# gssales/gaussian-splatting-reflection

Measured on AMD Instinct MI355X. Metric: train_step_views_per_s (fwd+bwd, 1e6 Gaussians @1080p, surfel rasterizer + reflection path), higher is better.
Workload: dtype f32

## Files before the change

gaussian-splatting-reflection_amd/csrc/gsr_cubemap.hip:

```cpp
#include <algorithm>
#include <cstring>
#include "gsr_internal.hpp"
#include <mutex>
#include <memory>
#include "gsr_sort.hpp"
#include <rocprim/iterator/counting_iterator.hpp>
#include "gsr_refl.hpp"

namespace gsr {



struct Plain {
	int f, ux0, ux1, uy0, uy1;
	float kx, ky;
};
__device__ __forceinline__ void plain_index(float vx, float vy, float vz, int L, Plain& p, bool nearest) {
	float u, v;
	cube_uv(vx, vy, vz, u, v, p.f);
	v = -v;
	u = (u * 0.5f + 0.5f) * (float)L;
	v = (v * 0.5f + 0.5f) * (float)L;
	if (nearest) {
		p.ux0 = min(max((int)u, 0), L - 1);
		p.uy0 = min(max((int)v, 0), L - 1);
		p.ux1 = p.ux0; p.uy1 = p.uy0; p.kx = 0; p.ky = 0;
		return;
	}
	const int ux_0 = (int)floorf(u - 0.5f), uy_0 = (int)floorf(v - 0.5f);
	p.kx = u - (float)ux_0 - 0.5f;
	p.ky = v - (float)uy_0 - 0.5f;
	p.ux0 = min(max(ux_0, 0), L - 1); p.ux1 = min(max(ux_0 + 1, 0), L - 1);
	p.uy0 = min(max(uy_0, 0), L - 1); p.uy1 = min(max(uy_0 + 1, 0), L - 1);
}

__global__ void __launch_bounds__(256)
cubemap_fwd_kernel(const float* __restrict__ inputs, const float* __restrict__ cubemap, const float* __restrict__ fail_value,
                   float* __restrict__ outputs, int interp, int seamless, uint32_t B, int C, int L) {
	const uint32_t n = blockIdx.x * 256 + threadIdx.x;
	if (n >= B) return;
	const float vx = inputs[(size_t)n * 3], vy = inputs[(size_t)n * 3 + 1], vz = inputs[(size_t)n * 3 + 2];
	if (vx == 0.f && vy == 0.f && vz == 0.f) {
		for (int c = 0; c < C; c++) outputs[(size_t)c * B + n] = fail_value[c];
		return;
	}
	if (interp == 0 || seamless == 0) {
		Plain p;
		plain_index(vx, vy, vz, L, p, interp == 0);
		for (int c = 0; c < C; c++) {
			if (interp == 0) {
				outputs[(size_t)c * B + n] = cubemap[texel(p.f, c, p.uy0, p.ux0, C, L)];
			} else {
				const float v00 = cubemap[texel(p.f, c, p.uy0, p.ux0, C, L)], v01 = cubemap[texel(p.f, c, p.uy0, p.ux1, C, L)];
				const float v10 = cubemap[texel(p.f, c, p.uy1, p.ux0, C, L)], v11 = cubemap[texel(p.f, c, p.uy1, p.ux1, C, L)];
				outputs[(size_t)c * B + n] = (1 - p.ky) * ((1 - p.kx) * v00 + p.kx * v01) + p.ky * ((1 - p.kx) * v10 + p.kx * v11);
			}
		}
		return;
	}
	float u, v;
	int face;
	cube_uv(vx, vy, vz, u, v, face);
	Seamless s;
	seamless_index(face, L, u, v, s);
	for (int c = 0; c < C; c++) {
		const float v00 = cubemap[texel(s.f[0], c, s.y[0], s.x[0], C, L)];
		const float v01 = cubemap[texel(s.f[1], c, s.y[1], s.x[1], C, L)];
		const float v10 = cubemap[texel(s.f[2], c, s.y[2], s.x[2], C, L)];
		const float v11 = s.is_vertex ? (v00 + v01 + v10) / 3.f : cubemap[texel(s.f[3], c, s.y[3], s.x[3], C, L)];
		outputs[(size_t)c * B + n] = (1 - s.ky) * ((1 - s.kx) * v00 + s.kx * v01) + s.ky * ((1 - s.kx) * v10 + s.kx * v11);
	}
}

__device__ __forceinline__ void seamless_bwd_channel(const Seamless& s, int c, int C, int L, const float* __restrict__ cubemap,
                                                     float* __restrict__ grad_cubemap, float g, float& gu, float& gv) {
	const size_t i00 = texel(s.f[0], c, s.y[0], s.x[0], C, L), i01 = texel(s.f[1], c, s.y[1], s.x[1], C, L);
	const size_t i10 = texel(s.f[2], c, s.y[2], s.x[2], C, L);
	const float v00 = cubemap[i00], v01 = cubemap[i01], v10 = cubemap[i10];
	float v11;
	if (s.is_vertex) {
		v11 = (v00 + v01 + v10) / 3.f;
		const float extra_g = s.ky * s.kx / 3.f;
		atomicAdd(grad_cubemap + i00, ((1 - s.ky) * (1 - s.kx) + extra_g) * g);
		atomicAdd(grad_cubemap + i01, ((1 - s.ky) * s.kx + extra_g) * g);
		atomicAdd(grad_cubemap + i10, ((s.ky * (1 - s.kx)) + extra_g) * g);
	} else {
		const size_t i11 = texel(s.f[3], c, s.y[3], s.x[3], C, L);
		v11 = cubemap[i11];
		atomicAdd(grad_cubemap + i00, (1 - s.ky) * (1 - s.kx) * g);
		atomicAdd(grad_cubemap + i01, (1 - s.ky) * s.kx * g);
		atomicAdd(grad_cubemap + i10, s.ky * (1 - s.kx) * g);
		atomicAdd(grad_cubemap + i11, s.ky * s.kx * g);
	}
	float lg0 = (1 - s.ky) * (v01 - v00) + s.ky * (v11 - v10);
	float lg1 = (1 - s.kx) * (v10 - v00) + s.kx * (v11 - v01);
	lg0 *= 0.5f * (float)L * g;
	lg1 *= 0.5f * (float)L * g;
	if (s.flag & 1) lg0 = -lg0;
	if (s.flag & 4) lg1 = -lg1;
	lg1 = -lg1;
	gu = lg0;
	gv = lg1;
}

__global__ void __launch_bounds__(256)
cubemap_bwd_kernel(const float* __restrict__ grad_outputs, const float* __restrict__ inputs, const float* __restrict__ cubemap,
                   float* __restrict__ grad_cubemap, float* __restrict__ grad_inputs, float* __restrict__ grad_fail, int interp, int seamless,
                   uint32_t B, int C, int L) {
	const uint32_t n = blockIdx.x * 256 + threadIdx.x;
	if (n >= B) return;
	const float vx = inputs[(size_t)n * 3], vy = inputs[(size_t)n * 3 + 1], vz = inputs[(size_t)n * 3 + 2];
	float gx = 0.f, gy = 0.f, gz = 0.f;
	if (vx == 0.f && vy == 0.f && vz == 0.f) {
		for (int c = 0; c < C; c++) atomicAdd(grad_fail + c, grad_outputs[(size_t)c * B + n]);
	} else if (interp == 0) {
		Plain p;
		plain_index(vx, vy, vz, L, p, true);
		for (int c = 0; c < C; c++) atomicAdd(grad_cubemap + texel(p.f, c, p.uy0, p.ux0, C, L), grad_outputs[(size_t)c * B + n]);
	} else if (seamless == 0) {
		Plain p;
		plain_index(vx, vy, vz, L, p, false);
		for (int c = 0; c < C; c++) {
			const size_t i00 = texel(p.f, c, p.uy0, p.ux0, C, L), i01 = texel(p.f, c, p.uy0, p.ux1, C, L);
			const size_t i10 = texel(p.f, c, p.uy1, p.ux0, C, L), i11 = texel(p.f, c, p.uy1, p.ux1, C, L);
			const float v00 = cubemap[i00], v01 = cubemap[i01], v10 = cubemap[i10], v11 = cubemap[i11];
			const float g = grad_outputs[(size_t)c * B + n];
			atomicAdd(grad_cubemap + i00, (1 - p.ky) * (1 - p.kx) * g);
			atomicAdd(grad_cubemap + i01, (1 - p.ky) * p.kx * g);
			atomicAdd(grad_cubemap + i10, p.ky * (1 - p.kx) * g);
			atomicAdd(grad_cubemap + i11, p.ky * p.kx * g);
			float lg0 = (1 - p.ky) * (v01 - v00) + p.ky * (v11 - v10);
			float lg1 = (1 - p.kx) * (v10 - v00) + p.kx * (v11 - v01);
			lg0 *= 0.5f * (float)L * g;
			lg1 *= 0.5f * (float)L * g;
			lg1 = -lg1;
			float a, b, cc;
			cube_uv_backward(p.f, vx, vy, vz, lg0, lg1, a, b, cc);
			gx += a; gy += b; gz += cc;
		}
	} else {
		float u, v;
		int face;
		cube_uv(vx, vy, vz, u, v, face);
		Seamless s;
		seamless_index(face, L, u, v, s);
		for (int c = 0; c < C; c++) {
			float gu, gv, a, b, cc;
			seamless_bwd_channel(s, c, C, L, cubemap, grad_cubemap, grad_outputs[(size_t)c * B + n], gu, gv);
			cube_uv_backward(face, vx, vy, vz, gu, gv, a, b, cc);
			gx += a; gy += b; gz += cc;
		}
	}
	grad_inputs[(size_t)n * 3] = gx;
	grad_inputs[(size_t)n * 3 + 1] = gy;
	grad_inputs[(size_t)n * 3 + 2] = gz;
}

__global__ void __launch_bounds__(256) cubemap_interleave_kernel(const float* __restrict__ cubemap, float4* __restrict__ rgba, int L) {
	const size_t LL = (size_t)L * L;
	const size_t t = (size_t)blockIdx.x * 256 + threadIdx.x;
	if (t >= 6 * LL) return;
	const size_t f = t / LL, r = t - f * LL;
	rgba[t] = make_float4(cubemap[(f * 3 + 0) * LL + r], cubemap[(f * 3 + 1) * LL + r], cubemap[(f * 3 + 2) * LL + r], 0.f);
}
template <bool RGBA>
__global__ void __launch_bounds__(256)
deferred_refl_fwd_kernel(const float* __restrict__ normal_view, const float* __restrict__ base, const float* __restrict__ strength,
                         const float* __restrict__ cam, const float* __restrict__ cubemap, const float4* __restrict__ rgba,
                         const float* __restrict__ fail_value, int L, int W, int H, float* __restrict__ out_final, float* __restrict__ out_refl,
                         float* __restrict__ out_nworld, uint32_t* __restrict__ sort_keys, uint32_t no_key) {
	const size_t HW = (size_t)W * H;
	const size_t pix = (size_t)blockIdx.x * 256 + threadIdx.x;
	if (pix >= HW) return;
	const int py = (int)(pix / W), px = (int)(pix - (size_t)py * W);
	const float nvx = normal_view[pix], nvy = normal_view[HW + pix], nvz = normal_view[2 * HW + pix];
	const float sv = strength[pix];
	const float b0 = base[pix], b1 = base[HW + pix], b2 = base[2 * HW + pix];
	ReflFwdOut o;
	refl_forward_pixel<RGBA>(cam, cubemap, rgba, fail_value, L, nvx, nvy, nvz, px, py, sv, b0, b1, b2, no_key, o);
	if (sort_keys) sort_keys[pix] = o.key;
#pragma unroll
	for (int ch = 0; ch < 3; ch++) {
		out_refl[ch * HW + pix] = o.refl_c[ch];
		out_final[ch * HW + pix] = o.final_c[ch];
	}
	out_nworld[pix] = o.nx;
	out_nworld[HW + pix] = o.ny;
	out_nworld[2 * HW + pix] = o.nz;
}

__device__ __forceinline__ float quad_sum(float v) {
	v += __int_as_float(__builtin_amdgcn_mov_dpp(__float_as_int(v), 0xB1, 0xF, 0xF, true));
	v += __int_as_float(__builtin_amdgcn_mov_dpp(__float_as_int(v), 0x4E, 0xF, 0xF, true));
	return v;
}
__global__ void __launch_bounds__(256)
deferred_refl_bwd_kernel(const float* __restrict__ normal_view, const float* __restrict__ base, const float* __restrict__ strength,
                         const float* __restrict__ cam, const float* __restrict__ cubemap, const float* __restrict__ fail_value, int L, int W,
                         int H, const float* __restrict__ g_final, const float* __restrict__ g_refl_color, const float* __restrict__ g_nworld,
                         float* __restrict__ g_normal_view, float* __restrict__ g_base, float* __restrict__ g_strength,
                         float* __restrict__ g_scratch, float* __restrict__ g_fail) {
	const size_t HW = (size_t)W * H;
	const size_t gid = (size_t)blockIdx.x * 256 + threadIdx.x;
	const size_t pix = gid >> 2;
	const int ch = (int)(gid & 3);
	const bool live = pix < HW;
	const size_t p = live ? pix : 0;
	const int py = (int)(p / W), px = (int)(p - (size_t)py * W);
	ReflPixel o;
	refl_pixel(cam, normal_view[p], normal_view[HW + p], normal_view[2 * HW + p], px, py, o);
	const bool fail = (o.rx == 0.f && o.ry == 0.f && o.rz == 0.f);
	const bool chan = live && ch < 3;
	const int c = ch < 3 ? ch : 0;
	Seamless s;
	int face = 0;
	float cval;
	size_t i00 = 0, i01 = 0, i10 = 0, i11 = 0;
	float v00 = 0, v01 = 0, v10 = 0, v11 = 0;
	if (fail) {
		cval = fail_value[c];
		s.kx = 0; s.ky = 0; s.flag = 0; s.is_vertex = false;
	} else {
		float u, v;
		cube_uv(o.rx, o.ry, o.rz, u, v, face);
		seamless_index(face, L, u, v, s);
		i00 = texel(s.f[0], c, s.y[0], s.x[0], 3, L); i01 = texel(s.f[1], c, s.y[1], s.x[1], 3, L);
		i10 = texel(s.f[2], c, s.y[2], s.x[2], 3, L);
		v00 = cubemap[i00]; v01 = cubemap[i01]; v10 = cubemap[i10];
		if (s.is_vertex) v11 = (v00 + v01 + v10) / 3.f;
		else { i11 = texel(s.f[3], c, s.y[3], s.x[3], 3, L); v11 = cubemap[i11]; }
		cval = (1 - s.ky) * ((1 - s.kx) * v00 + s.kx * v01) + s.ky * ((1 - s.kx) * v10 + s.kx * v11);
	}
	const float sv = strength[p];
	const float rc = sigmoidf_(cval);
	float gs = 0.f, grx = 0.f, gry = 0.f, grz = 0.f;
	int tix[4] = {-1, -1, -1, -1};
	float twg[4] = {0.f, 0.f, 0.f, 0.f};
	if (chan) {
		const float gf = g_final[c * HW + p];
		const float b = base[c * HW + p];
		g_base[c * HW + p] = (1 - sv) * gf;
		gs = gf * (rc - b);
		float gc = sv * gf;
		if (g_refl_color) gc += g_refl_color[c * HW + p];
		const float graw = gc * rc * (1 - rc);
		if (fail) {
			atomicAdd(g_fail + c, graw);
		} else {
			auto sidx = [&](int k) -> int { return (int)((((((size_t)s.f[k] * L + s.y[k]) * L + s.x[k]) << 2)) + c); };
			if (s.is_vertex) {
				const float extra_g = s.ky * s.kx / 3.f;
				tix[0] = sidx(0); twg[0] = ((1 - s.ky) * (1 - s.kx) + extra_g) * graw;
				tix[1] = sidx(1); twg[1] = ((1 - s.ky) * s.kx + extra_g) * graw;
				tix[2] = sidx(2); twg[2] = ((s.ky * (1 - s.kx)) + extra_g) * graw;
			} else {
				tix[0] = sidx(0); twg[0] = (1 - s.ky) * (1 - s.kx) * graw;
				tix[1] = sidx(1); twg[1] = (1 - s.ky) * s.kx * graw;
				tix[2] = sidx(2); twg[2] = s.ky * (1 - s.kx) * graw;
				tix[3] = sidx(3); twg[3] = s.ky * s.kx * graw;
			}
			float lg0 = (1 - s.ky) * (v01 - v00) + s.ky * (v11 - v10);
			float lg1 = (1 - s.kx) * (v10 - v00) + s.kx * (v11 - v01);
			lg0 *= 0.5f * (float)L * graw;
			lg1 *= 0.5f * (float)L * graw;
			if (s.flag & 1) lg0 = -lg0;
			if (s.flag & 4) lg1 = -lg1;
			lg1 = -lg1;
			cube_uv_backward(face, o.rx, o.ry, o.rz, lg0, lg1, grx, gry, grz);
		}
	}
	{
		const bool inA = ((threadIdx.x >> 2) & 1) == 0;
		const int XOR4 = 0x101F;
		const int s_i0 = inA ? tix[1] : tix[0], s_i1 = inA ? tix[3] : tix[2];
		const float s_w0 = inA ? twg[1] : twg[0], s_w1 = inA ? twg[3] : twg[2];
		const int r_i0 = __builtin_amdgcn_ds_swizzle(s_i0, XOR4), r_i1 = __builtin_amdgcn_ds_swizzle(s_i1, XOR4);
		const float r_w0 = __int_as_float(__builtin_amdgcn_ds_swizzle(__float_as_int(s_w0), XOR4));
		const float r_w1 = __int_as_float(__builtin_amdgcn_ds_swizzle(__float_as_int(s_w1), XOR4));
		const int i0 = inA ? tix[0] : r_i0, i1 = inA ? tix[2] : r_i1, i2 = inA ? r_i0 : tix[1], i3 = inA ? r_i1 : tix[3];
		const float w0 = inA ? twg[0] : r_w0, w1 = inA ? twg[2] : r_w1, w2 = inA ? r_w0 : twg[1], w3 = inA ? r_w1 : twg[3];
		if (i0 >= 0) atomicAdd(g_scratch + i0, w0);
		if (i1 >= 0) atomicAdd(g_scratch + i1, w1);
		if (i2 >= 0) atomicAdd(g_scratch + i2, w2);
		if (i3 >= 0) atomicAdd(g_scratch + i3, w3);
	}
	gs = quad_sum(gs); grx = quad_sum(grx); gry = quad_sum(gry); grz = quad_sum(grz);
	if (live && ch == 3) g_strength[p] = gs;
	const float grn = grx * o.nx + gry * o.ny + grz * o.nz;
	float gnx = -2.f * (o.dn * grx + grn * o.dx);
	float gny = -2.f * (o.dn * gry + grn * o.dy);
	float gnz = -2.f * (o.dn * grz + grn * o.dz);
	if (g_nworld) { gnx += g_nworld[p]; gny += g_nworld[HW + p]; gnz += g_nworld[2 * HW + p]; }
	const float inv = refl_rcp(o.len + 1e-6f);
	float gwx = gnx * inv, gwy = gny * inv, gwz = gnz * inv;
	if (o.len > 0.f) {
		const float k = (o.nwx * gnx + o.nwy * gny + o.nwz * gnz) * inv * inv * refl_rcp(o.len);
		gwx -= o.nwx * k; gwy -= o.nwy * k; gwz -= o.nwz * k;
	}
	if (chan) g_normal_view[c * HW + p] = gwx * cam[c] + gwy * cam[3 + c] + gwz * cam[6 + c];
}

#ifndef ENTRIES_BS
#define ENTRIES_BS 512
#endif
template <bool RGBA>
__global__ void __launch_bounds__(ENTRIES_BS)
deferred_refl_bwd_entries_kernel(const float* __restrict__ normal_view, const float* __restrict__ base, const float* __restrict__ strength,
                                 const float* __restrict__ cam, const float* __restrict__ cubemap, const float4* __restrict__ rgba,
                                 const float* __restrict__ fail_value, int L,
                                 int W, int H, const float* __restrict__ g_final, const float* __restrict__ g_refl_color,
                                 const float* __restrict__ g_nworld, float* __restrict__ g_normal_view, float* __restrict__ g_base,
                                 float* __restrict__ g_strength, float* __restrict__ g_fail, float* __restrict__ g_scratch,
                                 ReflFootprint* __restrict__ footprints, uint32_t* __restrict__ keys, const uint32_t* __restrict__ keys_fwd, uint32_t no_key,
                                 void* sort_clear, size_t sort_clear_bytes) {
	const size_t HW = (size_t)W * H;
	const size_t pix = (size_t)blockIdx.x * ENTRIES_BS + threadIdx.x;
	sort_clear_region(sort_clear, sort_clear_bytes, pix, (size_t)gridDim.x * ENTRIES_BS);
	const bool live = pix < HW;
	const size_t p = live ? pix : 0;
	const int py = (int)(p / W), px = (int)(p - (size_t)py * W);
	ReflBwdIn in;
	in.nvx = normal_view[p]; in.nvy = normal_view[HW + p]; in.nvz = normal_view[2 * HW + p];
	in.sv = strength[p];
	in.has_grc = g_refl_color != nullptr;
	in.has_gnw = g_nworld != nullptr;
#pragma unroll
	for (int c = 0; c < 3; c++) {
		in.gfin[c] = g_final[c * HW + p];
		in.bas[c] = base[c * HW + p];
		in.grc[c] = g_refl_color ? g_refl_color[c * HW + p] : 0.f;
		in.gnw[c] = g_nworld ? g_nworld[c * HW + p] : 0.f;
	}
	const uint32_t kf = keys_fwd ? keys_fwd[p] : no_key;
	ReflBwdOut o;
	refl_backward_pixel<RGBA>(cam, cubemap, rgba, fail_value, L, px, py, live, in, g_fail, g_scratch, footprints + p, keys_fwd != nullptr, kf,
	                          keys ? keys + p : nullptr, no_key, (int)(threadIdx.x & 63), o);
	if (!live) return;
	g_strength[p] = o.g_strength;
#pragma unroll
	for (int c = 0; c < 3; c++) {
		g_base[c * HW + p] = o.g_base[c];
		g_normal_view[c * HW + p] = o.g_nv[c];
	}
}

template <bool ACC>
__global__ void __launch_bounds__(256) unpack_cubemap_grad_kernel(const float4* __restrict__ scratch, float* __restrict__ g_cubemap,
                                                                  float* __restrict__ g_fail, int L) {
	const size_t n = (size_t)6 * L * L;
	const size_t t = (size_t)blockIdx.x * 256 + threadIdx.x;
	if (t == 0) {
		const float4 gf = scratch[n];
		g_fail[0] = (ACC ? g_fail[0] : 0.f) + gf.x; g_fail[1] = (ACC ? g_fail[1] : 0.f) + gf.y; g_fail[2] = (ACC ? g_fail[2] : 0.f) + gf.z;
	}
	if (t >= n) return;
	const size_t LL = (size_t)L * L;
	const size_t f = t / LL, r = t - f * LL;
	const float4 g = scratch[t];
	float* o = g_cubemap + f * 3 * LL + r;
	o[0] = (ACC ? o[0] : 0.f) + g.x;
	o[LL] = (ACC ? o[LL] : 0.f) + g.y;
	o[2 * LL] = (ACC ? o[2 * LL] : 0.f) + g.z;
}

#define REFL_CHUNK 8
#ifndef REFL_WIN
#define REFL_WIN 1024u
#endif
__global__ void __launch_bounds__(256) refl_run_combine_kernel(const uint32_t* __restrict__ keys_sorted, const uint32_t* __restrict__ pix_sorted,
                                                               const ReflFootprint* __restrict__ footprints, size_t n, uint32_t L, uint32_t no_key,
                                                               float* __restrict__ g_scratch) {
	__shared__ float win[3][REFL_WIN];
	__shared__ uint32_t s_hi;
	const size_t wg0 = (size_t)blockIdx.x * 256 * REFL_CHUNK;
	const uint32_t t_lo = keys_sorted[wg0];
	if (t_lo == no_key) return;
	const size_t wg_last = min(n, wg0 + (size_t)256 * REFL_CHUNK) - 1;
	const uint32_t t_hi = keys_sorted[wg_last];
	const uint32_t reach = t_hi == no_key ? REFL_WIN : min(REFL_WIN, t_hi - t_lo + L + 2u);
	for (uint32_t i = threadIdx.x; i < reach; i += 256) { win[0][i] = 0.f; win[1][i] = 0.f; win[2][i] = 0.f; }
	if (threadIdx.x == 0) s_hi = 0u;
	__syncthreads();

	const size_t i0 = wg0 + (size_t)threadIdx.x * REFL_CHUNK;
	uint32_t key[REFL_CHUNK];
	float4 ga[REFL_CHUNK];
	float gky[REFL_CHUNK];
#pragma unroll
	for (int j = 0; j < REFL_CHUNK; j++) key[j] = i0 + j < n ? keys_sorted[i0 + j] : no_key;
#pragma unroll
	for (int j = 0; j < REFL_CHUNK; j++) {
		ga[j] = make_float4(0.f, 0.f, 0.f, 0.f);
		gky[j] = 0.f;
		if (key[j] != no_key) {
			const float* f = reinterpret_cast<const float*>(footprints + pix_sorted[i0 + j]);
			ga[j] = *reinterpret_cast<const float4*>(f);
			gky[j] = f[4];
		}
	}
	float acc[4][3];
	uint32_t cur = no_key, hi = 0u;
	auto flush = [&]() {
		if (cur == no_key) return;
#pragma unroll
		for (int k = 0; k < 4; k++) {
			const uint32_t rel = cur - t_lo + (uint32_t)(k & 1) + (uint32_t)(k >> 1) * L;
			if (rel < REFL_WIN) {
				hi = max(hi, rel);
#pragma unroll
				for (int c = 0; c < 3; c++)
					if (acc[k][c] != 0.f) atomicAdd(&win[c][rel], acc[k][c]);
			} else {
				float* dst = g_scratch + (((size_t)t_lo + rel) << 2);
#pragma unroll
				for (int c = 0; c < 3; c++)
					if (acc[k][c] != 0.f) atomicAdd(dst + c, acc[k][c]);
			}
		}
	};
#pragma unroll
	for (int j = 0; j < REFL_CHUNK; j++) {
		if (key[j] != no_key) {
			if (key[j] != cur) {
				flush();
				cur = key[j];
#pragma unroll
				for (int k = 0; k < 4; k++) { acc[k][0] = 0.f; acc[k][1] = 0.f; acc[k][2] = 0.f; }
			}
			const float kx = ga[j].w, ky = gky[j];
			const float w4[4] = {(1 - ky) * (1 - kx), (1 - ky) * kx, ky * (1 - kx), ky * kx};
#pragma unroll
			for (int k = 0; k < 4; k++) {
				acc[k][0] += w4[k] * ga[j].x; acc[k][1] += w4[k] * ga[j].y; acc[k][2] += w4[k] * ga[j].z;
			}
		}
	}
	flush();
	if (hi != 0u) atomicMax(&s_hi, hi);
	__syncthreads();
	const uint32_t top = s_hi;
	for (uint32_t i = threadIdx.x; i <= top; i += 256) {
		float* dst = g_scratch + (((size_t)t_lo + i) << 2);
#pragma unroll
		for (int c = 0; c < 3; c++) {
			const float v = win[c][i];
			if (v != 0.f) atomicAdd(dst + c, v);
		}
	}
}

}

using namespace gsr;

extern "C" int gsr_cubemap_forward(const float* inputs, const float* cubemap, const float* fail_value, float* outputs, uint32_t interp,
                                   uint32_t seamless, uint32_t B, uint32_t C, uint32_t L, void* stream_) {
	hipStream_t stream = (hipStream_t)stream_;
	if (B == 0) return 0;
	if (!inputs || !cubemap || !fail_value || !outputs || C == 0 || L == 0) { set_error("gsr_cubemap_forward: invalid argument"); return GSR_E_INVALID; }
{ StageTimer st_(GSR_STAGE_CUBEMAP_FWD, stream); 	cubemap_fwd_kernel<<<(B + 255) / 256, 256, 0, stream>>>(inputs, cubemap, fail_value, outputs, (int)interp, (int)seamless, B, (int)C, (int)L); }
	GSR_LAUNCH_CHECK(0, stream);
	return 0;
}

extern "C" int gsr_cubemap_backward(const float* grad_outputs, const float* inputs, const float* cubemap, float* grad_cubemap,
                                    float* grad_inputs, float* grad_fail, uint32_t interp, uint32_t seamless, uint32_t B, uint32_t C, uint32_t L,
                                    void* stream_) {
	hipStream_t stream = (hipStream_t)stream_;
	if (B == 0) return 0;
	if (!grad_outputs || !inputs || !cubemap || !grad_cubemap || !grad_inputs || !grad_fail || C == 0 || L == 0) {
		set_error("gsr_cubemap_backward: invalid argument");
		return GSR_E_INVALID;
	}
{ StageTimer st_(GSR_STAGE_CUBEMAP_BWD, stream); 	cubemap_bwd_kernel<<<(B + 255) / 256, 256, 0, stream>>>(grad_outputs, inputs, cubemap, grad_cubemap, grad_inputs, grad_fail, (int)interp,
	                                                        (int)seamless, B, (int)C, (int)L); }
	GSR_LAUNCH_CHECK(0, stream);
	return 0;
}

extern "C" int gsr_deferred_reflection_forward_keys(const float* normal_view, const float* base_color, const float* refl_strength, const float* cam,
                                                  const float* cubemap, const float* fail_value, uint32_t L, int width, int height,
                                                  float* out_final, float* out_refl_color, float* out_normal_world, float* cubemap_rgba,
                                                  uint32_t* sort_keys, void* stream_) {
	hipStream_t stream = (hipStream_t)stream_;
	if (width <= 0 || height <= 0 || !normal_view || !base_color || !refl_strength || !cam || !cubemap || !fail_value || !out_final ||
	    !out_refl_color || !out_normal_world || L == 0 || ((uintptr_t)cubemap_rgba & 15) != 0) {
		set_error("gsr_deferred_reflection_forward: invalid argument");
		return GSR_E_INVALID;
	}
	if ((size_t)6 * L * L >= 0xFFFFFFFFull) { set_error("gsr_deferred_reflection_forward: cubemap too large"); return GSR_E_INVALID; }
	const size_t HW = (size_t)width * height;
	StageTimer st_(GSR_STAGE_REFL_FWD, stream);
	const unsigned grid = (unsigned)((HW + 255) / 256);
	if (cubemap_rgba) {
		float4* rgba = reinterpret_cast<float4*>(cubemap_rgba);
		cubemap_interleave_kernel<<<(unsigned)((6 * (size_t)L * L + 255) / 256), 256, 0, stream>>>(cubemap, rgba, (int)L);
		deferred_refl_fwd_kernel<true><<<grid, 256, 0, stream>>>(normal_view, base_color, refl_strength, cam, cubemap, rgba, fail_value, (int)L, width, height,
		                                                        out_final, out_refl_color, out_normal_world, sort_keys, (uint32_t)(6 * (size_t)L * L));
	} else {
		deferred_refl_fwd_kernel<false><<<grid, 256, 0, stream>>>(normal_view, base_color, refl_strength, cam, cubemap, nullptr, fail_value, (int)L, width, height,
		                                                         out_final, out_refl_color, out_normal_world, sort_keys, (uint32_t)(6 * (size_t)L * L));
	}
	GSR_LAUNCH_CHECK(0, stream);
	return 0;
}
extern "C" int gsr_deferred_reflection_forward_ex(const float* normal_view, const float* base_color, const float* refl_strength, const float* cam,
                                                  const float* cubemap, const float* fail_value, uint32_t L, int width, int height,
                                                  float* out_final, float* out_refl_color, float* out_normal_world, float* cubemap_rgba, void* stream_) {
	return gsr_deferred_reflection_forward_keys(normal_view, base_color, refl_strength, cam, cubemap, fail_value, L, width, height, out_final, out_refl_color,
	                                            out_normal_world, cubemap_rgba, nullptr, stream_);
}
extern "C" int gsr_deferred_reflection_forward(const float* normal_view, const float* base_color, const float* refl_strength, const float* cam,
                                               const float* cubemap, const float* fail_value, uint32_t L, int width, int height,
                                               float* out_final, float* out_refl_color, float* out_normal_world, void* stream_) {
	return gsr_deferred_reflection_forward_keys(normal_view, base_color, refl_strength, cam, cubemap, fail_value, L, width, height, out_final, out_refl_color,
	                                          out_normal_world, nullptr, nullptr, stream_);
}

struct ReflScratch {
	size_t ntex, n, sort_bytes, total_floats;
	int key_bits;
};
#ifndef REFL_SORT_BS
#define REFL_SORT_BS 512
#endif
#ifndef REFL_SORT_IPT
#define REFL_SORT_IPT 16
#endif
template <class F>
static auto with_refl_sort(int key_bits, bool small, F&& f) {
	if (small) return f(RadixSort<256, 8, 8>{});
	if (key_bits > 16 && key_bits <= 18) return f(RadixSort<REFL_SORT_BS, REFL_SORT_IPT, 9>{});
	if (key_bits > 18 && key_bits <= 20) return f(RadixSort<1024, 8, 10>{});
	return f(RadixSort<1024, 8, 8>{});
}
static ReflScratch refl_scratch(uint32_t L, int width, int height) {
	thread_local uint32_t last_L = 0;
	thread_local int last_w = 0, last_h = 0;
	thread_local ReflScratch last;
	if (last_L != 0 && L == last_L && width == last_w && height == last_h) return last;
	ReflScratch r;
	r.ntex = (size_t)6 * L * L;
	r.n = (size_t)width * height;
	r.key_bits = 1;
	while (((size_t)1 << r.key_bits) <= r.ntex) r.key_bits++;
	auto need = [&](bool small) {
		return with_refl_sort(r.key_bits, small, [&](auto sort) {
			return sort.temp_bytes((const uint32_t*)nullptr, rocprim::counting_iterator<uint32_t>(0), (uint32_t*)nullptr, r.n, (unsigned)r.key_bits);
		});
	};
	r.sort_bytes = std::max(need(false), need(true));
	r.total_floats = (r.ntex + 2) * 4 + 8 * r.n + 3 * r.n + (r.sort_bytes + 3) / 4 + 128;
	last = r; last_L = L; last_w = width; last_h = height;
	return r;
}
extern "C" size_t gsr_deferred_reflection_scratch_floats(uint32_t L, int width, int height, int binned) {
	if (L == 0 || width <= 0 || height <= 0) return 0;
	if (!binned) return ((size_t)6 * L * L + 1) * 4;
	return refl_scratch(L, width, height).total_floats;
}

namespace {
struct SideStream {
	hipStream_t stream = nullptr;
	hipEvent_t fork = nullptr, fork2 = nullptr, done = nullptr, gate = nullptr;
	bool recorded = false;
	bool gate_pending = false;
};
std::mutex g_side_mu;
SideStream g_side[64];
SideStream* side_stream(bool create) {
	int dev = 0;
	if (hipGetDevice(&dev) != hipSuccess || dev < 0 || dev >= 64) return nullptr;
	SideStream& s = g_side[dev];
	if (!s.stream && create) {
		int least = 0, greatest = 0;
		(void)hipDeviceGetStreamPriorityRange(&least, &greatest);
		if (hipStreamCreateWithPriority(&s.stream, hipStreamNonBlocking, greatest) != hipSuccess) { s.stream = nullptr; return nullptr; }
		if (hipEventCreateWithFlags(&s.fork, hipEventDisableTiming) != hipSuccess || hipEventCreateWithFlags(&s.fork2, hipEventDisableTiming) != hipSuccess ||
		    hipEventCreateWithFlags(&s.done, hipEventDisableTiming) != hipSuccess || hipEventCreateWithFlags(&s.gate, hipEventDisableTiming) != hipSuccess) {
			(void)hipStreamDestroy(s.stream);
			s.stream = nullptr;
		}
	}
	return s.stream ? &s : nullptr;
}

struct ReflTail {
	ReflScratch rs;
	float* staging = nullptr;
	float* fail_acc = nullptr;
	ReflFootprint* footprints = nullptr;
	uint32_t *keys_in = nullptr, *keys_out = nullptr, *pix_out = nullptr;
	void* sort_temp = nullptr;
	hipStream_t stream, tail;
	SideStream* side = nullptr;
	std::unique_lock<std::mutex> lock;

	ReflTail(uint32_t L, int width, int height, hipStream_t s) : rs(refl_scratch(L, width, height)), stream(s), tail(s) {}
	bool carve(float* scratch, size_t scratch_floats) {
		staging = scratch;
		fail_acc = scratch + rs.ntex * 4;
		if (scratch_floats < rs.total_floats || rs.n >= ((size_t)1 << 30) || rs.ntex >= 0xFFFFFFFFull || ((uintptr_t)scratch & 31) != 0) return false;
		footprints = reinterpret_cast<ReflFootprint*>(scratch + (rs.ntex + 1) * 4 + 4);
		keys_in = reinterpret_cast<uint32_t*>(footprints + rs.n);
		keys_out = keys_in + rs.n;
		pix_out = keys_out + rs.n;
		sort_temp = reinterpret_cast<void*>(((uintptr_t)(pix_out + rs.n) + 255) & ~(uintptr_t)255);
		return true;
	}
	void lock_side() { lock = std::unique_lock<std::mutex>(g_side_mu); }
	void use_side_stream() {
		lock_side();
		side = side_stream(true);
		if (side) tail = side->stream;
	}
	size_t sort_cleared_bytes(bool small) const {
		return with_refl_sort(rs.key_bits, small, [&](auto sort) { return sort.cleared_bytes(rs.n, (unsigned)rs.key_bits); });
	}
	hipError_t fork(hipEvent_t ev) {
		hipError_t e = hipEventRecord(ev, stream);
		return e == hipSuccess ? hipStreamWaitEvent(side->stream, ev, 0) : e;
	}
	hipError_t sort(const uint32_t* keys, bool small, bool gated) {
		hipError_t e = with_refl_sort(rs.key_bits, small, [&](auto sort) {
			return sort.pairs(sort_temp, rs.sort_bytes, keys, keys_out, rocprim::counting_iterator<uint32_t>(0), pix_out, rs.n, (unsigned)rs.key_bits, tail, true, nullptr,
			                  gated && side ? side->gate : nullptr);
		});
		if (e == hipSuccess && gated && side) side->gate_pending = true;
		return e;
	}
	hipError_t mark_done() {
		hipError_t e = hipEventRecord(side->done, side->stream);
		if (e == hipSuccess) side->recorded = true;
		return e;
	}
};
}

namespace gsr {
int side_gate_wait(hipStream_t stream) {
	std::lock_guard<std::mutex> lk(g_side_mu);
	SideStream* s = side_stream(false);
	if (s && s->gate_pending) {
		s->gate_pending = false;
		GSR_HIP_CHECK(hipStreamWaitEvent(stream, s->gate, 0));
	}
	return 0;
}

int refl_scratch_check(const char* entry, uint32_t L, int width, int height, const float* scratch, size_t scratch_floats) {
	ReflTail t(L, width, height, nullptr);
	if (!scratch || !t.carve(const_cast<float*>(scratch), scratch_floats)) {
		set_error("%s: reflection backward (sorted footprints): scratch of %zu floats, 32-byte aligned, needed (gsr_deferred_reflection_scratch_floats(L, W, H, 1))",
		          entry, t.rs.total_floats);
		return GSR_E_INVALID;
	}
	return 0;
}
int refl_sort_keys_early(uint32_t L, int width, int height, float* scratch, size_t scratch_floats, const uint32_t* sort_keys, int async, bool gated,
                         hipStream_t stream) {
	if (const int rc = refl_scratch_check("gsr_surfel_forward_refl", L, width, height, scratch, scratch_floats); rc < 0) return rc;
	ReflTail t(L, width, height, stream);
	t.carve(scratch, scratch_floats);
	if (async) t.use_side_stream();
	if (t.side) GSR_HIP_CHECK(t.fork(t.side->fork));
	{
		StageTimer tt(GSR_STAGE_REFL_BWD_TAIL, t.tail);
		GSR_HIP_CHECK(hipMemsetAsync(t.sort_temp, 0, t.sort_cleared_bytes(false), t.tail));
		GSR_HIP_CHECK(t.sort(sort_keys, false, gated));
	}
	if (t.side) GSR_HIP_CHECK(t.mark_done());
	return 0;
}
}

extern "C" int gsr_side_join(void* stream_) {
	std::lock_guard<std::mutex> lk(g_side_mu);
	const SideStream* s = side_stream(false);
	if (s && s->recorded) GSR_HIP_CHECK(hipStreamWaitEvent((hipStream_t)stream_, s->done, 0));
	return 0;
}

extern "C" int gsr_deferred_reflection_backward_keys(const float* normal_view, const float* base_color, const float* refl_strength, const float* cam,
                                                   const float* cubemap, const float* fail_value, uint32_t L, int width, int height,
                                                   const float* g_final, const float* g_refl_color, const float* g_normal_world,
                                                   float* g_normal_view, float* g_base, float* g_strength, float* g_cubemap, float* g_fail,
                                                   float* scratch, size_t scratch_floats, int accumulate, int async_tail, const float* cubemap_rgba,
                                                   const uint32_t* sort_keys, int keys_sorted, void* stream_) {
	hipStream_t stream = (hipStream_t)stream_;
	if (width <= 0 || height <= 0 || !normal_view || !base_color || !refl_strength || !cam || !cubemap || !fail_value || !g_final ||
	    !g_normal_view || !g_base || !g_strength || !g_cubemap || !g_fail || !scratch || L == 0 || (keys_sorted && !sort_keys)) {
		set_error("gsr_deferred_reflection_backward: invalid argument");
		return GSR_E_INVALID;
	}
	if ((size_t)6 * L * L >= 0xFFFFFFFFull) { set_error("gsr_deferred_reflection_backward: cubemap too large"); return GSR_E_INVALID; }
	GSR_REQUIRE_ALIGNED16_IN("gsr_deferred_reflection_backward", scratch, "scratch");
	GSR_REQUIRE_ALIGNED16_IN("gsr_deferred_reflection_backward", cubemap_rgba, "cubemap_rgba");
	const size_t HW = (size_t)width * height;
	ReflTail t(L, width, height, stream);
	const size_t ntex = t.rs.ntex;
	if (scratch_floats < (ntex + 1) * 4) { set_error("gsr_deferred_reflection_backward: scratch smaller than (6*L*L+1)*4 floats"); return GSR_E_INVALID; }
	const bool binned = t.carve(scratch, scratch_floats);
	if (keys_sorted && !binned) { set_error("gsr_deferred_reflection_backward: keys_sorted needs the scratch the forward sorted into"); return GSR_E_INVALID; }
	auto unpack = accumulate ? unpack_cubemap_grad_kernel<true> : unpack_cubemap_grad_kernel<false>;
	GSR_HIP_CHECK(hipMemsetAsync(scratch, 0, (ntex + 1) * 4 * sizeof(float), stream));
	if (!binned) {
		{
			StageTimer st_(GSR_STAGE_REFL_BWD, stream);
			const unsigned grid = (unsigned)((HW * 4 + 255) / 256);
			deferred_refl_bwd_kernel<<<grid, 256, 0, stream>>>(normal_view, base_color, refl_strength, cam, cubemap, fail_value, (int)L, width, height, g_final,
			                                                  g_refl_color, g_normal_world, g_normal_view, g_base, g_strength, t.staging, t.fail_acc);
		}
		unpack<<<(unsigned)((ntex + 255) / 256), 256, 0, stream>>>((const float4*)t.staging, g_cubemap, g_fail, (int)L);
		GSR_LAUNCH_CHECK(0, stream);
		return 0;
	}
	const bool small_sort = async_tail && !sort_keys;
	const size_t sort_cleared = t.sort_cleared_bytes(small_sort);
	if (async_tail) t.use_side_stream();
	else if (keys_sorted) t.lock_side();
	if (keys_sorted) {
		const SideStream* s = side_stream(false);
		if (s && s->recorded && t.tail != s->stream) GSR_HIP_CHECK(hipStreamWaitEvent(t.tail, s->done, 0));
	} else if (sort_keys) {
		GSR_HIP_CHECK(hipMemsetAsync(t.sort_temp, 0, sort_cleared, stream));
		if (t.side) GSR_HIP_CHECK(t.fork(t.side->fork));
		StageTimer tt(GSR_STAGE_REFL_BWD_TAIL, t.tail);
		GSR_HIP_CHECK(t.sort(sort_keys, false, true));
	}
	{
		StageTimer st_(GSR_STAGE_REFL_BWD, stream);
		const unsigned egrid = (unsigned)((HW + ENTRIES_BS - 1) / ENTRIES_BS);
		if (cubemap_rgba)
			deferred_refl_bwd_entries_kernel<true><<<egrid, ENTRIES_BS, 0, stream>>>(normal_view, base_color, refl_strength, cam, cubemap,
			                                                                 reinterpret_cast<const float4*>(cubemap_rgba), fail_value, (int)L, width, height, g_final,
			                                                                 g_refl_color, g_normal_world, g_normal_view, g_base, g_strength, t.fail_acc, t.staging,
			                                                                 t.footprints, t.keys_in, sort_keys, (uint32_t)ntex, sort_keys ? nullptr : t.sort_temp,
			                                                                 sort_keys ? 0 : sort_cleared);
		else
			deferred_refl_bwd_entries_kernel<false><<<egrid, ENTRIES_BS, 0, stream>>>(normal_view, base_color, refl_strength, cam, cubemap, nullptr, fail_value, (int)L, width,
			                                                                  height, g_final, g_refl_color, g_normal_world, g_normal_view, g_base, g_strength, t.fail_acc,
			                                                                  t.staging, t.footprints, t.keys_in, sort_keys, (uint32_t)ntex, sort_keys ? nullptr : t.sort_temp,
			                                                                  sort_keys ? 0 : sort_cleared);
	}
	if (t.side) GSR_HIP_CHECK(t.fork(sort_keys ? t.side->fork2 : t.side->fork));
	{
		StageTimer tt(GSR_STAGE_REFL_BWD_TAIL, t.tail);
		const size_t per_wg = (size_t)256 * REFL_CHUNK;
		const unsigned cgrid = (unsigned)((t.rs.n + per_wg - 1) / per_wg);
		if (!sort_keys) GSR_HIP_CHECK(t.sort(t.keys_in, small_sort, false));
		refl_run_combine_kernel<<<cgrid, 256, 0, t.tail>>>(t.keys_out, t.pix_out, t.footprints, t.rs.n, L, (uint32_t)ntex, t.staging);
		unpack<<<(unsigned)((ntex + 255) / 256), 256, 0, t.tail>>>((const float4*)t.staging, g_cubemap, g_fail, (int)L);
	}
	if (t.side) GSR_HIP_CHECK(t.mark_done());
	GSR_HIP_CHECK(hipGetLastError());
	return 0;
}

extern "C" int gsr_deferred_reflection_backward_ex(const float* normal_view, const float* base_color, const float* refl_strength, const float* cam,
                                                   const float* cubemap, const float* fail_value, uint32_t L, int width, int height,
                                                   const float* g_final, const float* g_refl_color, const float* g_normal_world,
                                                   float* g_normal_view, float* g_base, float* g_strength, float* g_cubemap, float* g_fail,
                                                   float* scratch, size_t scratch_floats, int accumulate, int async_tail, const float* cubemap_rgba,
                                                   void* stream_) {
	return gsr_deferred_reflection_backward_keys(normal_view, base_color, refl_strength, cam, cubemap, fail_value, L, width, height, g_final, g_refl_color,
	                                             g_normal_world, g_normal_view, g_base, g_strength, g_cubemap, g_fail, scratch, scratch_floats, accumulate,
	                                             async_tail, cubemap_rgba, nullptr, 0, stream_);
}

extern "C" int gsr_deferred_reflection_backward_accum(const float* normal_view, const float* base_color, const float* refl_strength, const float* cam,
                                                const float* cubemap, const float* fail_value, uint32_t L, int width, int height,
                                                const float* g_final, const float* g_refl_color, const float* g_normal_world,
                                                float* g_normal_view, float* g_base, float* g_strength, float* g_cubemap, float* g_fail,
                                                float* scratch, size_t scratch_floats, int accumulate, void* stream_) {
	return gsr_deferred_reflection_backward_keys(normal_view, base_color, refl_strength, cam, cubemap, fail_value, L, width, height, g_final, g_refl_color,
	                                             g_normal_world, g_normal_view, g_base, g_strength, g_cubemap, g_fail, scratch, scratch_floats, accumulate, 0, nullptr,
	                                             nullptr, 0, stream_);
}

extern "C" int gsr_deferred_reflection_backward(const float* normal_view, const float* base_color, const float* refl_strength, const float* cam,
                                                const float* cubemap, const float* fail_value, uint32_t L, int width, int height,
                                                const float* g_final, const float* g_refl_color, const float* g_normal_world,
                                                float* g_normal_view, float* g_base, float* g_strength, float* g_cubemap, float* g_fail,
                                                float* scratch, size_t scratch_floats, void* stream_) {
	return gsr_deferred_reflection_backward_accum(normal_view, base_color, refl_strength, cam, cubemap, fail_value, L, width, height, g_final, g_refl_color,
	                                              g_normal_world, g_normal_view, g_base, g_strength, g_cubemap, g_fail, scratch, scratch_floats, 0, stream_);
}

__global__ void __launch_bounds__(256) normal_world_fwd_kernel(const float* __restrict__ normal_view, const float* __restrict__ cam, size_t HW,
                                                               float* __restrict__ out) {
	const size_t pix = (size_t)blockIdx.x * 256 + threadIdx.x;
	if (pix >= HW) return;
	const float vx = normal_view[pix], vy = normal_view[HW + pix], vz = normal_view[2 * HW + pix];
	const float wx = vx * cam[0] + vy * cam[1] + vz * cam[2], wy = vx * cam[3] + vy * cam[4] + vz * cam[5], wz = vx * cam[6] + vy * cam[7] + vz * cam[8];
	const float inv = 1.0f / (sqrtf(wx * wx + wy * wy + wz * wz) + 1e-6f);
	out[pix] = wx * inv; out[HW + pix] = wy * inv; out[2 * HW + pix] = wz * inv;
}
__global__ void __launch_bounds__(256) normal_world_bwd_kernel(const float* __restrict__ normal_view, const float* __restrict__ cam, size_t HW,
                                                               const float* __restrict__ g_out, float* __restrict__ g_normal_view) {
	const size_t pix = (size_t)blockIdx.x * 256 + threadIdx.x;
	if (pix >= HW) return;
	const float vx = normal_view[pix], vy = normal_view[HW + pix], vz = normal_view[2 * HW + pix];
	const float wx = vx * cam[0] + vy * cam[1] + vz * cam[2], wy = vx * cam[3] + vy * cam[4] + vz * cam[5], wz = vx * cam[6] + vy * cam[7] + vz * cam[8];
	const float len = sqrtf(wx * wx + wy * wy + wz * wz);
	const float inv = 1.0f / (len + 1e-6f);
	const float gx = g_out[pix], gy = g_out[HW + pix], gz = g_out[2 * HW + pix];
	float ax = gx * inv, ay = gy * inv, az = gz * inv;
	if (len > 0.f) {
		const float k = (wx * gx + wy * gy + wz * gz) * inv * inv / len;
		ax -= wx * k; ay -= wy * k; az -= wz * k;
	}
#pragma unroll
	for (int c = 0; c < 3; c++) g_normal_view[c * HW + pix] = ax * cam[c] + ay * cam[3 + c] + az * cam[6 + c];
}
extern "C" int gsr_normal_world_forward(const float* normal_view, const float* cam, int width, int height, float* out_normal_world, void* stream_) {
	if (width <= 0 || height <= 0 || !normal_view || !cam || !out_normal_world) { set_error("gsr_normal_world_forward: invalid argument"); return GSR_E_INVALID; }
	const size_t HW = (size_t)width * height;
	normal_world_fwd_kernel<<<(unsigned)((HW + 255) / 256), 256, 0, (hipStream_t)stream_>>>(normal_view, cam, HW, out_normal_world);
	GSR_LAUNCH_CHECK(0, (hipStream_t)stream_);
	return 0;
}
extern "C" int gsr_normal_world_backward(const float* normal_view, const float* cam, int width, int height, const float* g_normal_world,
                                         float* g_normal_view, void* stream_) {
	if (width <= 0 || height <= 0 || !normal_view || !cam || !g_normal_world || !g_normal_view) { set_error("gsr_normal_world_backward: invalid argument"); return GSR_E_INVALID; }
	const size_t HW = (size_t)width * height;
	normal_world_bwd_kernel<<<(unsigned)((HW + 255) / 256), 256, 0, (hipStream_t)stream_>>>(normal_view, cam, HW, g_normal_world, g_normal_view);
	GSR_LAUNCH_CHECK(0, (hipStream_t)stream_);
	return 0;
}
```

gaussian-splatting-reflection_amd/csrc/gsr_internal.hpp:

```cpp
#pragma once
#include <cstring>
#include <cstdint>
#include <cstdio>
#include <hip/hip_runtime.h>
#include "../../include/gsr_hip.h"

#define GSR_TILE 16
#define GSR_TILE_PIX 256

namespace gsr {

void set_error(const char* fmt, ...);
#define GSR_HIP_CHECK(expr)                                                                       \
	do {                                                                                          \
		hipError_t _e = (expr);                                                                   \
		if (_e != hipSuccess) {                                                                   \
			gsr::set_error("%s failed: %s (%s:%d)", #expr, hipGetErrorString(_e), __FILE__, __LINE__); \
			return GSR_E_HIP;                                                                     \
		}                                                                                         \
	} while (0)
#define GSR_LAUNCH_CHECK(debug, stream)                                  \
	do {                                                                 \
		GSR_HIP_CHECK(hipGetLastError());                                \
		if (debug) GSR_HIP_CHECK(hipStreamSynchronize(stream));          \
	} while (0)

static inline bool misaligned16(const void* p) { return (reinterpret_cast<uintptr_t>(p) & 15u) != 0; }
#define GSR_REQUIRE_ALIGNED16_IN(func, ptr, what)                                                             \
	do {                                                                                                      \
		if ((ptr) && gsr::misaligned16(ptr)) {                                                                \
			gsr::set_error("%s: %s must be 16-byte aligned (float4 accesses); got %p", func, what, (const void*)(ptr)); \
			return GSR_E_INVALID;                                                                             \
		}                                                                                                     \
	} while (0)
#define GSR_REQUIRE_ALIGNED16(ptr, what) GSR_REQUIRE_ALIGNED16_IN(__func__, ptr, what)

struct StageTimer {
	int stage;
	hipStream_t stream;
	void* rec;
	StageTimer(int stage, hipStream_t stream);
	~StageTimer();
};

struct Carver {
	char* base;
	size_t off;
	explicit Carver(void* b) : base((char*)b), off(0) {}
	template <class T> T* take(size_t count) {
		off = (off + 255) & ~(size_t)255;
		T* p = base ? (T*)(base + off) : nullptr;
		off += count * sizeof(T);
		return p;
	}
	size_t size() const { return (off + 255) & ~(size_t)255; }
};

struct GeomState {
	float* depths;
	uint32_t* rect;
	uint32_t* tiles_touched;
	uint32_t* point_offsets;
	uint8_t* clamped;
	float4* rec;
	float4* bbox;
	float* aux;
	float* acc;
	int* flags;
	uint32_t* depth_sorted;
	unsigned long long* order;
	unsigned long long* emit_state;
	size_t emit_state_bytes;
	void* scan_temp;
	size_t scan_temp_bytes;
	void* depth_sort_temp;
	size_t depth_sort_bytes, depth_sort_clear;
};
struct ImageState {
	uint2* ranges;
	float* final_T;
	uint32_t* n_contrib;
	uint32_t* tile_order;
};
struct BinningState {
	uint32_t* point_list;
	unsigned long long* blend_mask;
	size_t mask_stride;
	uint32_t* tile_keys;
	uint32_t* tile_keys_unsorted;
	uint32_t* vals_unsorted;
	void* sort_temp;
	size_t sort_temp_bytes;
};

#define S_REC_F4 5
#define S_ACC_F 20
#define G_REC_F4 4
#define G_ACC_F 16
struct WorkspaceLayout {
	int rec_f4, aux_floats, acc_floats;
	int planes_T, planes_n;
	constexpr WorkspaceLayout inference() const { return {rec_f4, aux_floats, 0, 0, 0}; }
};
constexpr WorkspaceLayout SURFEL_LAYOUT{S_REC_F4, 0, S_ACC_F, 3, 2};
constexpr WorkspaceLayout GAUSS_LAYOUT{G_REC_F4, 0, G_ACC_F, 1, 1};

GeomState carve_geom(void* buf, size_t P, const WorkspaceLayout& layout, size_t* total);
ImageState carve_image(void* buf, size_t HW, size_t tiles, const WorkspaceLayout& layout, size_t* total);
BinningState carve_binning(void* buf, size_t R, size_t tiles, size_t sort_temp_bytes, size_t* total, bool blend_masks = true);
int forward_workspace(gsr_alloc_fn alloc, void* alloc_user, const WorkspaceLayout& layout, size_t P, size_t HW, size_t tiles, GeomState* geom,
                      ImageState* img);

static inline int check_sh_input(const char* entry, int D, int M, const float* shs) {
	if (D < 0 || D > 3 || (shs && (D + 1) * (D + 1) > M)) { set_error("%s: SH degree %d not supported with M=%d", entry, D, M); return GSR_E_INVALID; }
	if (shs && ((M * 3) & 3) == 0 && misaligned16(shs)) {
		set_error("%s: shs (rows of a multiple of 16 bytes) must be 16-byte aligned (float4 accesses); got %p", entry, (const void*)shs);
		return GSR_E_INVALID;
	}
	return 0;
}

struct RasterCam {
	const float* view;
	const float* proj;
	const float* campos;
	int W, H;
	float tan_fovx, tan_fovy, focal_x, focal_y;
};
static inline RasterCam make_cam(const float* view, const float* proj, const float* campos, int W, int H, float tan_fovx, float tan_fovy) {
	RasterCam c;
	c.view = view; c.proj = proj; c.campos = campos; c.W = W; c.H = H;
	c.tan_fovx = tan_fovx; c.tan_fovy = tan_fovy;
	c.focal_y = H / (2.0f * tan_fovy);
	c.focal_x = W / (2.0f * tan_fovx);
	return c;
}

struct BackwardWorkspace { GeomState geom; ImageState img; BinningState bin; int tiles_x, ntiles; };
static inline int backward_prologue(const char* entry, const char* func, const WorkspaceLayout& layout, int P, int M, int R, int width, int height,
                                    bool missing_pointer, const float* shs, const float* dL_dsh, const float* dL_drot, const float* also_aligned,
                                    const char* also_what, void* geom_buffer, void* binning_buffer, void* image_buffer, hipStream_t stream,
                                    BackwardWorkspace* w) {
	if (P < 0 || R < 0 || width <= 0 || height <= 0) { set_error("%s: invalid size", entry); return GSR_E_INVALID; }
	if (P == 0) return 0;
	if (missing_pointer) { set_error("%s: missing required pointer", entry); return GSR_E_INVALID; }
	if (shs && ((M * 3) & 3) == 0) GSR_REQUIRE_ALIGNED16_IN(func, dL_dsh, "dL_dsh");
	GSR_REQUIRE_ALIGNED16_IN(func, dL_drot, "dL_drot");
	GSR_REQUIRE_ALIGNED16_IN(func, also_aligned, also_what);
	w->tiles_x = (width + 15) / 16;
	w->ntiles = w->tiles_x * ((height + 15) / 16);
	w->geom = carve_geom(geom_buffer, P, layout, nullptr);
	w->img = carve_image(image_buffer, (size_t)width * height, w->ntiles, layout, nullptr);
	w->bin = carve_binning(binning_buffer, R, w->ntiles, 0, nullptr);
	GSR_HIP_CHECK(hipMemsetAsync(w->geom.acc, 0, (size_t)P * layout.acc_floats * sizeof(float), stream));
	return 1;
}

int option_cull();
int option_dev();
unsigned long long* dev_pair_counter();
size_t sort_temp_bytes(size_t R, int end_bit);
int run_tile_order(const ImageState& img, size_t tiles, hipStream_t stream);
uint32_t higher_msb(uint32_t n);

int run_binning(gsr_alloc_fn alloc, void* alloc_user, int P, int tiles_x, int tiles_y, const GeomState& geom,
                const ImageState& img, BinningState* out_binning, int prefiltered, int debug, hipStream_t stream, bool blend_masks = true);

int side_gate_wait(hipStream_t stream);
int refl_scratch_check(const char* entry, uint32_t L, int width, int height, const float* scratch, size_t scratch_floats);
int refl_sort_keys_early(uint32_t L, int width, int height, float* scratch, size_t scratch_floats, const uint32_t* sort_keys, int async, bool gated,
                         hipStream_t stream);

}

#ifdef __HIPCC__
namespace gsr {

__device__ __forceinline__ int f2i(float v) { return (int)v; }

__device__ __forceinline__ void get_rect(float px, float py, int max_radius, int gx, int gy, uint32_t& x0, uint32_t& y0,
                                         uint32_t& x1, uint32_t& y1) {
	const float r = (float)max_radius;
	x0 = (uint32_t)min(gx, max(0, f2i((px - r) / 16.0f)));
	y0 = (uint32_t)min(gy, max(0, f2i((py - r) / 16.0f)));
	x1 = (uint32_t)min(gx, max(0, f2i((px + r + 15.0f) / 16.0f)));
	y1 = (uint32_t)min(gy, max(0, f2i((py + r + 15.0f) / 16.0f)));
}

#define GSR_DPP1(CTRL, i) "v_add_f32_dpp %" #i ", %" #i ", %" #i " " CTRL "\n\t"
#define GSR_DPP4(CTRL) GSR_DPP1(CTRL, 0) GSR_DPP1(CTRL, 1) GSR_DPP1(CTRL, 2) GSR_DPP1(CTRL, 3)
#define GSR_SHR1 "row_shr:1 row_mask:0xf bank_mask:0xf bound_ctrl:0"
#define GSR_SHR2 "row_shr:2 row_mask:0xf bank_mask:0xf bound_ctrl:0"
#define GSR_SHR4 "row_shr:4 row_mask:0xf bank_mask:0xf bound_ctrl:0"
#define GSR_SHR8 "row_shr:8 row_mask:0xf bank_mask:0xf bound_ctrl:0"
#define GSR_BC15 "row_bcast:15 row_mask:0xa bank_mask:0xf"
#define GSR_BC31 "row_bcast:31 row_mask:0xc bank_mask:0xf"
__device__ __forceinline__ void wave_sum4(float* v) {
	asm volatile("s_nop 1\n\t" GSR_DPP4(GSR_SHR1) GSR_DPP4(GSR_SHR2) GSR_DPP4(GSR_SHR4) GSR_DPP4(GSR_SHR8) GSR_DPP4(GSR_BC15) GSR_DPP4(GSR_BC31)
	             : "+v"(v[0]), "+v"(v[1]), "+v"(v[2]), "+v"(v[3]));
}

#define GSR_Q1(CTRL, i) "v_add_f32_dpp %" #i ", %" #i ", %" #i " " CTRL " row_mask:0xf bank_mask:0xf\n\t"
#define GSR_DPPB(CTRL, BANK, dst, src) "v_add_f32_dpp %" #dst ", %" #src ", %" #src " " CTRL " row_mask:0xf bank_mask:" BANK "\n\t"
#define GSR_L1(CTRL, d, a, b) GSR_DPPB(CTRL, "0x3", d, a) GSR_DPPB(CTRL, "0xc", d, b)
__device__ __forceinline__ void row_reduce20(const float* v, float* z) {
	float p0, q0, p1, q1, p2, q2, p3, q3, p4, q4;
	asm volatile("s_nop 1\n\t" GSR_L1("row_mirror", 0, 6, 7) GSR_L1("row_mirror", 1, 8, 9) GSR_L1("row_mirror", 2, 10, 11)
	             GSR_L1("row_mirror", 3, 12, 13) GSR_L1("row_mirror", 4, 14, 15) GSR_L1("row_mirror", 5, 16, 17)
	             : "=&v"(p0), "=&v"(q0), "=&v"(p1), "=&v"(q1), "=&v"(p2), "=&v"(q2)
	             : "v"(v[0]), "v"(v[1]), "v"(v[2]), "v"(v[3]), "v"(v[4]), "v"(v[5]), "v"(v[6]), "v"(v[7]), "v"(v[8]), "v"(v[9]), "v"(v[10]), "v"(v[11]));
	asm volatile("s_nop 1\n\t" GSR_L1("row_mirror", 0, 4, 5) GSR_L1("row_mirror", 1, 6, 7) GSR_L1("row_mirror", 2, 8, 9) GSR_L1("row_mirror", 3, 10, 11)
	             : "=&v"(p3), "=&v"(q3), "=&v"(p4), "=&v"(q4)
	             : "v"(v[12]), "v"(v[13]), "v"(v[14]), "v"(v[15]), "v"(v[16]), "v"(v[17]), "v"(v[18]), "v"(v[19]));
#define GSR_L2(d, a, b) GSR_DPPB("row_half_mirror", "0x5", d, a) GSR_DPPB("row_half_mirror", "0xa", d, b)
#define GSR_QA(CTRL) GSR_Q1(CTRL, 0) GSR_Q1(CTRL, 1) GSR_Q1(CTRL, 2) GSR_Q1(CTRL, 3) GSR_Q1(CTRL, 4)
	asm volatile("s_nop 1\n\t" GSR_L2(0, 5, 6) GSR_L2(1, 7, 8) GSR_L2(2, 9, 10) GSR_L2(3, 11, 12) GSR_L2(4, 13, 14)
	             GSR_QA("quad_perm:[2,3,0,1]") GSR_QA("quad_perm:[1,0,3,2]")
	             : "=&v"(z[0]), "=&v"(z[1]), "=&v"(z[2]), "=&v"(z[3]), "=&v"(z[4])
	             : "v"(p0), "v"(q0), "v"(p1), "v"(q1), "v"(p2), "v"(q2), "v"(p3), "v"(q3), "v"(p4), "v"(q4));
}
__device__ __forceinline__ void row_reduce16(const float* v, float* z) {
	float p0, q0, p1, q1, p2, q2, p3, q3;
	asm volatile("s_nop 1\n\t" GSR_L1("row_mirror", 0, 8, 9) GSR_L1("row_mirror", 1, 10, 11) GSR_L1("row_mirror", 2, 12, 13) GSR_L1("row_mirror", 3, 14, 15)
	             GSR_L1("row_mirror", 4, 16, 17) GSR_L1("row_mirror", 5, 18, 19) GSR_L1("row_mirror", 6, 20, 21) GSR_L1("row_mirror", 7, 22, 23)
	             : "=&v"(p0), "=&v"(q0), "=&v"(p1), "=&v"(q1), "=&v"(p2), "=&v"(q2), "=&v"(p3), "=&v"(q3)
	             : "v"(v[0]), "v"(v[1]), "v"(v[2]), "v"(v[3]), "v"(v[4]), "v"(v[5]), "v"(v[6]), "v"(v[7]), "v"(v[8]), "v"(v[9]), "v"(v[10]), "v"(v[11]),
	               "v"(v[12]), "v"(v[13]), "v"(v[14]), "v"(v[15]));
#define GSR_QB(CTRL) GSR_Q1(CTRL, 0) GSR_Q1(CTRL, 1) GSR_Q1(CTRL, 2) GSR_Q1(CTRL, 3)
	asm volatile("s_nop 1\n\t" GSR_L2(0, 4, 5) GSR_L2(1, 6, 7) GSR_L2(2, 8, 9) GSR_L2(3, 10, 11)
	             GSR_QB("quad_perm:[2,3,0,1]") GSR_QB("quad_perm:[1,0,3,2]")
	             : "=&v"(z[0]), "=&v"(z[1]), "=&v"(z[2]), "=&v"(z[3])
	             : "v"(p0), "v"(q0), "v"(p1), "v"(q1), "v"(p2), "v"(q2), "v"(p3), "v"(q3));
}
__device__ __forceinline__ int sub_px(int lane) { return ((lane >> 4) & 1) * 4 + (lane & 3); }
__device__ __forceinline__ int sub_py(int lane) { return (lane >> 5) * 4 + ((lane >> 2) & 3); }
__device__ __forceinline__ void wave_lds_sync() {
	__builtin_amdgcn_fence(__ATOMIC_RELEASE, "wavefront");
	__builtin_amdgcn_wave_barrier();
	__builtin_amdgcn_fence(__ATOMIC_ACQUIRE, "wavefront");
}
template <int N, bool ACC>
__device__ __forceinline__ void wave_store_rows(float* lds, const float* v, float* __restrict__ out, int nrows, int lane) {
#pragma unroll
	for (int k = 0; k < N; k++) lds[k * 65 + lane] = v[k];
	wave_lds_sync();
#pragma unroll
	for (int j = 0; j < N; j++) {
		const int e = lane + 64 * j, r = e / N, k = e - r * N;
		if (r < nrows) {
			const float x = lds[k * 65 + r];
			if (ACC) {
				if (x != 0.f) out[e] += x;
			} else {
				out[e] = x;
			}
		}
	}
	wave_lds_sync();
}
template <int N, bool ACC>
__device__ __forceinline__ void wave_store_rows4(float4* lds, const float4* v, float4* __restrict__ out, int pitch, int col0, int nrows, int lane) {
#pragma unroll
	for (int k = 0; k < N; k++) lds[k * 65 + lane] = v[k];
	wave_lds_sync();
#pragma unroll
	for (int j = 0; j < N; j++) {
		const int e = lane + 64 * j, r = e / N, k = e - r * N;
		if (r < nrows) {
			const float4 x = lds[k * 65 + r];
			float4* o = out + (size_t)r * pitch + col0 + k;
			if (ACC) {
				if (x.x != 0.f || x.y != 0.f || x.z != 0.f || x.w != 0.f) {
					const float4 y = *o;
					*o = make_float4(y.x + x.x, y.y + x.y, y.z + x.z, y.w + x.w);
				}
			} else {
				*o = x;
			}
		}
	}
	wave_lds_sync();
}
template <bool ACC> __device__ __forceinline__ void put(float* p, float v) {
	if (ACC) { if (v != 0.f) *p += v; }
	else *p = v;
}
template <bool ACC> __device__ __forceinline__ void put4(float4* p, float a, float b, float c, float d) {
	if (ACC) {
		if (a != 0.f || b != 0.f || c != 0.f || d != 0.f) {
			const float4 r = *p;
			*p = make_float4(r.x + a, r.y + b, r.z + c, r.w + d);
		}
	} else {
		*p = make_float4(a, b, c, d);
	}
}
__device__ __forceinline__ uint32_t ffbl_raw(uint32_t x) {
	uint32_t r;
	asm("v_ffbl_b32 %0, %1" : "=v"(r) : "v"(x));
	return r;
}
__device__ __forceinline__ int row_reduce_slot(int lane) {
	const int q = (lane >> 2) & 3;
	return ((q & 1) << 1) | (q >> 1);
}

typedef unsigned long long lmask;
#define LMASK(cond) __builtin_amdgcn_ballot_w64(cond)
__device__ __forceinline__ float selm(lmask m, float a, float b) {
	float r;
	asm("v_cndmask_b32 %0, %1, %2, %3" : "=v"(r) : "v"(b), "v"(a), "s"(m));
	return r;
}
__device__ __forceinline__ float selm0(lmask m, float a) {
	float r;
	asm("v_cndmask_b32 %0, 0, %1, %2" : "=v"(r) : "v"(a), "s"(m));
	return r;
}
__device__ __forceinline__ uint32_t selmu(lmask m, uint32_t a, uint32_t b) {
	uint32_t r;
	asm("v_cndmask_b32 %0, %1, %2, %3" : "=v"(r) : "v"(b), "v"(a), "s"(m));
	return r;
}

__device__ __forceinline__ float min_raw(float a, float b) {
	float r;
	asm("v_min_f32 %0, %1, %2" : "=v"(r) : "v"(a), "v"(b));
	return r;
}

__device__ __forceinline__ float row_max4(float a, float b, float c, float d) {
	float p, q, z;
	asm volatile("s_nop 1\n\t"
	             "v_max_f32_dpp %0, %2, %2 row_mirror row_mask:0xf bank_mask:0x3\n\t"
	             "v_max_f32_dpp %0, %3, %3 row_mirror row_mask:0xf bank_mask:0xc\n\t"
	             "v_max_f32_dpp %1, %4, %4 row_mirror row_mask:0xf bank_mask:0x3\n\t"
	             "v_max_f32_dpp %1, %5, %5 row_mirror row_mask:0xf bank_mask:0xc\n\t"
	             : "=&v"(p), "=&v"(q) : "v"(a), "v"(b), "v"(c), "v"(d));
	asm volatile("s_nop 1\n\t"
	             "v_max_f32_dpp %0, %1, %1 row_half_mirror row_mask:0xf bank_mask:0x5\n\t"
	             "v_max_f32_dpp %0, %2, %2 row_half_mirror row_mask:0xf bank_mask:0xa\n\t"
	             "s_nop 1\n\t"
	             "v_max_f32_dpp %0, %0, %0 quad_perm:[2,3,0,1] row_mask:0xf bank_mask:0xf\n\t"
	             "s_nop 1\n\t"
	             "v_max_f32_dpp %0, %0, %0 quad_perm:[1,0,3,2] row_mask:0xf bank_mask:0xf\n\t"
	             : "=&v"(z) : "v"(p), "v"(q));
	return z;
}

__device__ __forceinline__ float exp_neg(float x) {
	const float hi = x * 1.44269504f;
	const float lo = fmaf(x, 1.44269504f, -hi) + x * 1.92596299e-8f;
	const float e = __builtin_amdgcn_exp2f(hi);
	return fmaf(e, 0.693147181f * lo, e);
}

__device__ __forceinline__ float div_nr(float a, float b) {
	const float r = __builtin_amdgcn_rcpf(b);
	const float q = a * r;
	const float e = fmaf(-b, q, a);
	return fmaf(e, r, q);
}


#ifndef GSR_CULL_RCP
#define GSR_CULL_RCP 1
#endif
__device__ __forceinline__ bool cull_hit(const float4 c0, const float4 c1, float x0, float x1, float y0, float y1) {
	if (c1.w == -2.0f) return false;
	const float a = c0.z, b = c0.w, c = c1.x;
	if (!(a > 0.0f)) return true;
	const float ex = c0.x, ey = c0.y;
	bool hit = ex >= x0 && ex <= x1 && ey >= y0 && ey <= y1;
	if (!hit) {
		float best = __int_as_float(0x7f800000);
#if GSR_CULL_RCP
		const float boc = b * __builtin_amdgcn_rcpf(c), boa = b * __builtin_amdgcn_rcpf(a);
#else
		const float boc = b / c, boa = b / a;
#endif
#pragma unroll
		for (int e = 0; e < 2; e++) {
			const float dx = (e ? x1 : x0) - ex;
			const float dy = fminf(fmaxf(-boc * dx, y0 - ey), y1 - ey);
			best = fminf(best, a * dx * dx + 2.0f * b * dx * dy + c * dy * dy);
			const float dy2 = (e ? y1 : y0) - ey;
			const float dx2 = fminf(fmaxf(-boa * dy2, x0 - ex), x1 - ex);
			best = fminf(best, a * dx2 * dx2 + 2.0f * b * dx2 * dy2 + c * dy2 * dy2);
		}
		hit = !(best > 1.0f);
	}
	if (!hit && c1.w >= 0.0f) {
		const float dx = fminf(fmaxf(c1.y, x0), x1) - c1.y;
		const float dy = fminf(fmaxf(c1.z, y0), y1) - c1.z;
		hit = !(dx * dx + dy * dy > c1.w);
	}
	return hit;
}

#define XCD_CHUNK 4
__device__ __forceinline__ uint32_t xcd_slot(uint32_t bid) {
	const uint32_t xcd = bid & 7u, j = bid >> 3;
	return ((j / XCD_CHUNK) * 8u + xcd) * XCD_CHUNK + (j % XCD_CHUNK);
}
__host__ __device__ __forceinline__ uint32_t xcd_grid(uint32_t nunits) {
	const uint32_t g = 8u * XCD_CHUNK;
	return (nunits + g - 1) / g * g;
}

}
#endif
```

gaussian-splatting-reflection_amd/csrc/gsr_refl.hpp:

```cpp
#pragma once
#include "gsr_internal.hpp"

namespace gsr {

#ifndef GSR_REFL_FAST
#define GSR_REFL_FAST 1
#endif
__device__ __forceinline__ float refl_rcp(float x) {
#if GSR_REFL_FAST
	return __builtin_amdgcn_rcpf(x);
#else
	return 1.0f / x;
#endif
}
__device__ __forceinline__ float refl_sqrt(float x) {
#if GSR_REFL_FAST
	return __builtin_amdgcn_sqrtf(x);
#else
	return sqrtf(x);
#endif
}

__device__ __forceinline__ void cube_uv(float x, float y, float z, float& u, float& v, int& index) {
	int max_dim = 0;
	const float x_ = fabsf(x), y_ = fabsf(y), z_ = fabsf(z);
	float max_v = x_;
	if (y_ > max_v) { max_v = y_; max_dim = 1; }
	if (z_ > max_v) { max_v = z_; max_dim = 2; }
#if GSR_REFL_FAST
	const float m = max_dim == 0 ? x : (max_dim == 1 ? y : z);
	const float a = max_dim == 0 ? z : x, b = max_dim == 1 ? z : y;
	const float r = refl_rcp(m);
	index = 2 * max_dim + (m >= 0.f ? 0 : 1);
	u = a * r; v = b * r;
	if (index == 0 || index == 1 || index == 3) u = -u;
	if (index == 0 || index == 3 || index == 4) v = -v;
#else
	if (max_dim == 0) {
		u = z / x; v = y / x;
		if (x >= 0.f) { index = 0; u = -u; v = -v; }
		else { index = 1; u = -u; }
	} else if (max_dim == 1) {
		u = x / y; v = z / y;
		if (y >= 0.f) { index = 2; }
		else { index = 3; u = -u; v = -v; }
	} else {
		u = x / z; v = y / z;
		if (z >= 0.f) { index = 4; v = -v; }
		else { index = 5; }
	}
#endif
}

__device__ __forceinline__ void edge_table(int L, int flag, int& face, int& x, int& y) {
	const unsigned short tbl[24] = {
	    4 | (1 << 4) | (3 << 8), 5 | (0 << 4) | (3 << 8), 3 | (1 << 4) | (2 << 8), 2 | (1 << 4) | (2 << 8),
	    5 | (1 << 4) | (3 << 8), 4 | (0 << 4) | (3 << 8), 3 | (0 << 4) | (4 << 8), 2 | (0 << 4) | (4 << 8),
	    1 | (5 << 4) | (1 << 8), 0 | (3 << 4) | (1 << 8), 4 | (2 << 4) | (1 << 8), 5 | (4 << 4) | (1 << 8),
	    1 | (5 << 4) | (0 << 8), 0 | (3 << 4) | (0 << 8), 4 | (2 << 4) | (0 << 8), 5 | (4 << 4) | (0 << 8),
	    1 | (1 << 4) | (3 << 8), 0 | (0 << 4) | (3 << 8), 3 | (2 << 4) | (0 << 8), 2 | (2 << 4) | (0 << 8),
	    0 | (1 << 4) | (3 << 8), 1 | (0 << 4) | (3 << 8), 3 | (4 << 4) | (1 << 8), 2 | (4 << 4) | (1 << 8)};
	const int fi = flag == 1 ? 0 : (flag == 2 ? 1 : (flag == 4 ? 2 : 3));
	const unsigned e = tbl[face * 4 + fi];
	const int ix = x, iy = y, Lm = L - 1;
	auto sel = [&](unsigned s) -> int {
		int r = 0;
		r = s == 1u ? Lm : r;
		r = s == 2u ? ix : r;
		r = s == 3u ? iy : r;
		r = s == 4u ? Lm - ix : r;
		r = s == 5u ? Lm - iy : r;
		return r;
	};
	face = e & 15;
	x = sel((e >> 4) & 15);
	y = sel((e >> 8) & 15);
}

struct Seamless {
	int f[4], x[4], y[4];
	float kx, ky;
	int flag;
	bool is_vertex;
};
__device__ __forceinline__ void seamless_index(int index, int L, float u, float v, Seamless& s) {
	float lu = u, lv = -v;
	lu = (lu * 0.5f + 0.5f) * (float)L;
	lv = (lv * 0.5f + 0.5f) * (float)L;
	int ux_0 = (int)floorf(lu - 0.5f), uy_0 = (int)floorf(lv - 0.5f);
	int ux_1 = ux_0 + 1, uy_1 = uy_0 + 1;
	float kx = lu - (float)ux_0 - 0.5f;
	float ky = lv - (float)uy_0 - 0.5f;
	ux_0 = min(max(ux_0, 0), L - 1); ux_1 = min(max(ux_1, 0), L - 1);
	uy_0 = min(max(uy_0, 0), L - 1); uy_1 = min(max(uy_1, 0), L - 1);
	int flag = 0;
	if (lu < 0.5f) { flag |= 1; kx = 0.5f - lu; }
	else if (lu >= (float)L - 0.5f) flag |= 2;
	if (lv < 0.5f) { flag |= 4; ky = 0.5f - lv; }
	else if (lv >= (float)L - 0.5f) flag |= 8;
	s.is_vertex = false;
#pragma unroll
	for (int i = 0; i < 4; i++) s.f[i] = index;
	s.x[0] = ux_0; s.y[0] = uy_0;
	s.x[1] = ux_1; s.y[1] = uy_0;
	s.x[2] = ux_0; s.y[2] = uy_1;
	s.x[3] = ux_1; s.y[3] = uy_1;
	if (flag != 0) {
		const int fu = flag & 3, fv = flag & 12;
		const bool hu = fu != 0, hv = fv != 0;
		s.is_vertex = hu && hv;
		int f1 = index, x1 = ux_0, y1 = uy_0;
		edge_table(L, hu ? fu : 1, f1, x1, y1);
		int f2 = index, x2 = ux_0, y2 = uy_0;
		edge_table(L, hv ? fv : 4, f2, x2, y2);
		int f3 = index, x3 = hu ? ux_0 : ux_1, y3 = hu ? uy_1 : uy_0;
		edge_table(L, hu ? fu : fv, f3, x3, y3);
		if (hu) { s.f[1] = f1; s.x[1] = x1; s.y[1] = y1; }
		if (hv) { s.f[2] = f2; s.x[2] = x2; s.y[2] = y2; }
		if (s.is_vertex) { s.f[3] = index; s.x[3] = ux_0; s.y[3] = uy_0; }
		else { s.f[3] = f3; s.x[3] = x3; s.y[3] = y3; }
	}
	s.kx = kx; s.ky = ky; s.flag = flag;
}

__device__ __forceinline__ void cube_uv_backward(int index, float x, float y, float z, float gu, float gv, float& gx, float& gy, float& gz) {
	const int face = index / 2;
#if GSR_REFL_FAST
	if (index == 0 || index == 1 || index == 3) gu = -gu;
	if (index == 0 || index == 3 || index == 4) gv = -gv;
	const float m = face == 0 ? x : (face == 1 ? y : z);
	const float a = face == 0 ? z : x, b = face == 1 ? z : y;
	const float r = refl_rcp(m);
	const float ga = r * gu, gb = r * gv, gm = -(a * gu + b * gv) * (r * r);
	gx = face == 0 ? gm : ga;
	gy = face == 1 ? gm : gb;
	gz = face == 2 ? gm : (face == 0 ? ga : gb);
#else
	if (face == 0) {
		if (index == 0) { gu = -gu; gv = -gv; }
		else { gu = -gu; }
		gx = -(z * gu + y * gv) / (x * x);
		gy = 1.f / x * gv;
		gz = 1.f / x * gu;
	} else if (face == 1) {
		if (index != 2) { gu = -gu; gv = -gv; }
		gx = 1.f / y * gu;
		gy = -(x * gu + z * gv) / (y * y);
		gz = 1.f / y * gv;
	} else {
		if (index == 4) { gv = -gv; }
		gx = 1.f / z * gu;
		gy = 1.f / z * gv;
		gz = -(x * gu + y * gv) / (z * z);
	}
#endif
}

__device__ __forceinline__ size_t texel(int f, int c, int y, int x, int C, int L) { return (((size_t)f * C + c) * L + y) * L + x; }

struct ReflPixel {
	float nwx, nwy, nwz, len;
	float nx, ny, nz;
	float dx, dy, dz;
	float dn;
	float rx, ry, rz;
};
__device__ __forceinline__ void refl_pixel(const float* __restrict__ cam, float nvx, float nvy, float nvz, int px, int py, ReflPixel& o) {
	o.nwx = nvx * cam[0] + nvy * cam[1] + nvz * cam[2];
	o.nwy = nvx * cam[3] + nvy * cam[4] + nvz * cam[5];
	o.nwz = nvx * cam[6] + nvy * cam[7] + nvz * cam[8];
	o.len = refl_sqrt(o.nwx * o.nwx + o.nwy * o.nwy + o.nwz * o.nwz);
	const float inv = refl_rcp(o.len + 1e-6f);
	o.nx = o.nwx * inv; o.ny = o.nwy * inv; o.nz = o.nwz * inv;
	const float x = (float)px, y = (float)py;
	const float pcx = cam[9] * x + cam[10] * y + cam[11] - cam[27];
	const float pcy = cam[12] * x + cam[13] * y + cam[14] - cam[28];
	const float pcz = cam[15] * x + cam[16] * y + cam[17] - cam[29];
	float wx = pcx * cam[18] + pcy * cam[21] + pcz * cam[24] - cam[30];
	float wy = pcx * cam[19] + pcy * cam[22] + pcz * cam[25] - cam[31];
	float wz = pcx * cam[20] + pcy * cam[23] + pcz * cam[26] - cam[32];
#if GSR_REFL_FAST
	const float idl = __builtin_amdgcn_rsqf(wx * wx + wy * wy + wz * wz);
	o.dx = wx * idl; o.dy = wy * idl; o.dz = wz * idl;
#else
	const float dl = sqrtf(wx * wx + wy * wy + wz * wz);
	o.dx = wx / dl; o.dy = wy / dl; o.dz = wz / dl;
#endif
	o.dn = o.dx * o.nx + o.dy * o.ny + o.dz * o.nz;
	o.rx = o.dx - 2 * o.nx * o.dn;
	o.ry = o.dy - 2 * o.ny * o.dn;
	o.rz = o.dz - 2 * o.nz * o.dn;
}
__device__ __forceinline__ float sigmoidf_(float x) { return refl_rcp(1.0f + __expf(-x)); }

template <bool RGBA>
__device__ __forceinline__ void fetch_corners(const Seamless& s, int L, const float* __restrict__ cubemap, const float4* __restrict__ rgba, float (&v)[4][3]) {
#pragma unroll
	for (int k = 0; k < 4; k++) {
		{
			if (RGBA) {
				const float4 t = rgba[(uint32_t)((s.f[k] * L + s.y[k]) * L + s.x[k])];
				v[k][0] = t.x; v[k][1] = t.y; v[k][2] = t.z;
			} else {
#pragma unroll
				for (int c = 0; c < 3; c++) v[k][c] = cubemap[texel(s.f[k], c, s.y[k], s.x[k], 3, L)];
			}
		}
	}
	if (s.is_vertex) {
#pragma unroll
		for (int c = 0; c < 3; c++) v[3][c] = GSR_REFL_FAST ? (v[0][c] + v[1][c] + v[2][c]) * 0.33333334f : (v[0][c] + v[1][c] + v[2][c]) / 3.f;
	}
}


struct alignas(32) ReflFootprint {
	float g[3], kx, ky;
	float pad[3];
};

struct ReflFwdOut {
	float final_c[3], refl_c[3], nx, ny, nz;
	uint32_t key;
};
template <bool RGBA>
__device__ __forceinline__ void refl_forward_pixel(const float* __restrict__ cam, const float* __restrict__ cubemap, const float4* __restrict__ rgba,
                                                   const float* __restrict__ fail_value, int L, float nvx, float nvy, float nvz, int px, int py, float sv,
                                                   float b0, float b1, float b2, uint32_t no_key, ReflFwdOut& out) {
	out.key = no_key;
	ReflPixel o;
	refl_pixel(cam, nvx, nvy, nvz, px, py, o);
	float c[3];
	if (o.rx == 0.f && o.ry == 0.f && o.rz == 0.f) {
		c[0] = fail_value[0]; c[1] = fail_value[1]; c[2] = fail_value[2];
	} else {
		float u, v;
		int face;
		cube_uv(o.rx, o.ry, o.rz, u, v, face);
		Seamless s;
		seamless_index(face, L, u, v, s);
		float cv[4][3];
		fetch_corners<RGBA>(s, L, cubemap, rgba, cv);
#pragma unroll
		for (int ch = 0; ch < 3; ch++)
			c[ch] = (1 - s.ky) * ((1 - s.kx) * cv[0][ch] + s.kx * cv[1][ch]) + s.ky * ((1 - s.kx) * cv[2][ch] + s.kx * cv[3][ch]);
		if (s.flag == 0 && s.x[3] == s.x[0] + 1 && s.y[3] == s.y[0] + 1) out.key = (uint32_t)(((size_t)s.f[0] * L + s.y[0]) * L + s.x[0]);
	}
	const float bs[3] = {b0, b1, b2};
#pragma unroll
	for (int ch = 0; ch < 3; ch++) {
		const float rc = sigmoidf_(c[ch]);
		out.refl_c[ch] = rc;
		out.final_c[ch] = (1 - sv) * bs[ch] + sv * rc;
	}
	out.nx = o.nx; out.ny = o.ny; out.nz = o.nz;
}

struct ReflBwdIn {
	float nvx, nvy, nvz, sv;
	float gfin[3], bas[3], grc[3], gnw[3];
	bool has_grc, has_gnw;
};
struct ReflBwdOut {
	float g_base[3], g_strength, g_nv[3];
};
template <bool RGBA>
__device__ __forceinline__ void refl_backward_pixel(const float* __restrict__ cam, const float* __restrict__ cubemap, const float4* __restrict__ rgba,
                                                    const float* __restrict__ fail_value, int L, int px, int py, bool live, const ReflBwdIn& in,
                                                    float* __restrict__ g_fail, float* __restrict__ g_scratch, ReflFootprint* __restrict__ footprint,
                                                    bool keys_fwd_valid, uint32_t kf, uint32_t* __restrict__ key_out, uint32_t no_key, int lane,
                                                    ReflBwdOut& out) {
	const float sv = in.sv;
	ReflPixel o;
	refl_pixel(cam, in.nvx, in.nvy, in.nvz, px, py, o);
	const bool fail = (o.rx == 0.f && o.ry == 0.f && o.rz == 0.f);
	Seamless s;
	int face = 0;
	s.kx = 0; s.ky = 0; s.flag = 0; s.is_vertex = false;
#pragma unroll
	for (int k = 0; k < 4; k++) { s.f[k] = 0; s.x[k] = 0; s.y[k] = 0; }
	if (!fail) {
		float u, v;
		cube_uv(o.rx, o.ry, o.rz, u, v, face);
		seamless_index(face, L, u, v, s);
	}
	float graw[3] = {0.f, 0.f, 0.f};
	float gs = 0.f, grx = 0.f, gry = 0.f, grz = 0.f;
	float cv[4][3] = {{0.f, 0.f, 0.f}, {0.f, 0.f, 0.f}, {0.f, 0.f, 0.f}, {0.f, 0.f, 0.f}};
	if (!fail) fetch_corners<RGBA>(s, L, cubemap, rgba, cv);
#pragma unroll
	for (int c = 0; c < 3; c++) {
		float cval;
		const float v00 = cv[0][c], v01 = cv[1][c], v10 = cv[2][c], v11 = cv[3][c];
		if (fail) cval = fail_value[c];
		else cval = (1 - s.ky) * ((1 - s.kx) * v00 + s.kx * v01) + s.ky * ((1 - s.kx) * v10 + s.kx * v11);
		const float rc = sigmoidf_(cval);
		const float gf = in.gfin[c];
		const float b = in.bas[c];
		out.g_base[c] = (1 - sv) * gf;
		gs += gf * (rc - b);
		float gc = sv * gf;
		if (in.has_grc) gc += in.grc[c];
		graw[c] = gc * rc * (1 - rc);
		if (fail) {
			if (live) atomicAdd(g_fail + c, graw[c]);
		} else {
			float lg0 = (1 - s.ky) * (v01 - v00) + s.ky * (v11 - v10);
			float lg1 = (1 - s.kx) * (v10 - v00) + s.kx * (v11 - v01);
			lg0 *= 0.5f * (float)L * graw[c];
			lg1 *= 0.5f * (float)L * graw[c];
			if (s.flag & 1) lg0 = -lg0;
			if (s.flag & 4) lg1 = -lg1;
			lg1 = -lg1;
			float a, bb, cc;
			cube_uv_backward(face, o.rx, o.ry, o.rz, lg0, lg1, a, bb, cc);
			grx += a; gry += bb; grz += cc;
		}
	}
	bool interior = !fail && s.flag == 0 && s.x[3] == s.x[0] + 1 && s.y[3] == s.y[0] + 1;
	const uint32_t t00 = (uint32_t)(((size_t)s.f[0] * L + s.y[0]) * L + s.x[0]);
	if (keys_fwd_valid) interior = interior && kf == t00;
	{
		const int k_of_lane = lane / 3, c_of_lane = lane - 3 * k_of_lane;
		const float extra_g = s.is_vertex ? s.ky * s.kx * 0.33333334f : 0.f;
		const float w4[4] = {(1 - s.ky) * (1 - s.kx) + extra_g, (1 - s.ky) * s.kx + extra_g, s.ky * (1 - s.kx) + extra_g, s.ky * s.kx};
		unsigned long long todo = __ballot(live && !fail && !interior);
		while (todo) {
			const int src = __ffsll((long long)todo) - 1;
			todo &= todo - 1;
			uint32_t tk[4];
			float wk[4], gk[3];
#pragma unroll
			for (int k = 0; k < 4; k++) {
				const int f = __builtin_amdgcn_readlane(s.f[k], src), y = __builtin_amdgcn_readlane(s.y[k], src), x = __builtin_amdgcn_readlane(s.x[k], src);
				tk[k] = (uint32_t)(((size_t)f * L + y) * L + x);
				wk[k] = __int_as_float(__builtin_amdgcn_readlane(__float_as_int(w4[k]), src));
			}
#pragma unroll
			for (int c = 0; c < 3; c++) gk[c] = __int_as_float(__builtin_amdgcn_readlane(__float_as_int(graw[c]), src));
			const int corners = __builtin_amdgcn_readlane((int)s.is_vertex, src) ? 3 : 4;
			if (k_of_lane < corners) {
				const uint32_t t = k_of_lane == 0 ? tk[0] : k_of_lane == 1 ? tk[1] : k_of_lane == 2 ? tk[2] : tk[3];
				const float w = k_of_lane == 0 ? wk[0] : k_of_lane == 1 ? wk[1] : k_of_lane == 2 ? wk[2] : wk[3];
				const float g = c_of_lane == 0 ? gk[0] : c_of_lane == 1 ? gk[1] : gk[2];
				atomicAdd(g_scratch + ((size_t)t << 2) + c_of_lane, w * g);
			}
		}
	}
	if (live) {
		if (interior || kf != no_key) {
			float* f = reinterpret_cast<float*>(footprint);
			*reinterpret_cast<float4*>(f) = interior ? make_float4(graw[0], graw[1], graw[2], s.kx) : make_float4(0.f, 0.f, 0.f, 0.f);
			f[4] = interior ? s.ky : 0.f;
		}
		if (!keys_fwd_valid) *key_out = interior ? t00 : no_key;
	}
	out.g_strength = gs;
	const float grn = grx * o.nx + gry * o.ny + grz * o.nz;
	float gnx = -2.f * (o.dn * grx + grn * o.dx);
	float gny = -2.f * (o.dn * gry + grn * o.dy);
	float gnz = -2.f * (o.dn * grz + grn * o.dz);
	if (in.has_gnw) { gnx += in.gnw[0]; gny += in.gnw[1]; gnz += in.gnw[2]; }
	const float inv = refl_rcp(o.len + 1e-6f);
	float gwx = gnx * inv, gwy = gny * inv, gwz = gnz * inv;
	if (o.len > 0.f) {
		const float k = (o.nwx * gnx + o.nwy * gny + o.nwz * gnz) * inv * inv * refl_rcp(o.len);
		gwx -= o.nwx * k; gwy -= o.nwy * k; gwz -= o.nwz * k;
	}
#pragma unroll
	for (int c = 0; c < 3; c++) out.g_nv[c] = gwx * cam[c] + gwy * cam[3 + c] + gwz * cam[6 + c];
}

}
```

gaussian-splatting-reflection_amd/csrc/gsr_surfel.hip:

```cpp
#include <type_traits>
#include "gsr_internal.hpp"
#include "gsr_tile_walk.hpp"
#include "gsr_sort.hpp"
#include "gsr_math.hpp"
#include "gsr_refl.hpp"

namespace gsr {

#define SA_COLOR 0
#define SA_REFL 3
#define SA_NORMAL 4
#define SA_OPAC 7
#define SA_T 8
#define SA_MEAN2D 17

#define S_NEAR 0.2f
#define S_FAR 100.0f
#define S_FILTER_INV_SQ 2.0f

__device__ __forceinline__ M3 quat_to_rotmat(const float* __restrict__ q, float& w, float& x, float& y, float& z) {
#pragma clang fp contract(off)
	const float s = 1.0f / sqrtf(q[3] * q[3] + q[0] * q[0] + q[1] * q[1] + q[2] * q[2]);
	w = q[0] * s; x = q[1] * s; y = q[2] * s; z = q[3] * s;
	return m3_make(1.f - 2.f * (y * y + z * z), 2.f * (x * y + w * z), 2.f * (x * z - w * y), 2.f * (x * y - w * z),
// ... 210 lines not shown
	__device__ __forceinline__ float refl() const { return f[3].w; }
	__device__ __forceinline__ v2f rg() const { return mk2(f[4].x, f[4].y); }
	__device__ __forceinline__ float b() const { return f[4].z; }
	__device__ __forceinline__ float mask() const { return f[4].w; }
};

#ifndef GSR_BWD_WPE
#define GSR_BWD_WPE 4
#endif
#ifndef GSR_BWD_LIST
#define GSR_BWD_LIST 1
#endif
#ifndef GSR_BWD_UNROLL
#define GSR_BWD_UNROLL 1
#endif
#ifdef GSR_FWD_WPE
#define GSR_FWD_ATTR __attribute__((amdgpu_waves_per_eu(GSR_FWD_WPE, GSR_FWD_WPE)))
#else
#define GSR_FWD_ATTR
#endif

struct SurfelFwdPix {
	float T, C2, M2, distortion, median_depth, median_contributor, maskacc;
	v2f Crg, Nxy, NzR, DM;
	uint32_t last_contributor;
};

template <bool TRAIN>
__device__ __forceinline__ lmask surfel_fwd_pair(const SurfelRec& R, const v2f pix, uint32_t contributor, bool med_live, SurfelFwdPix& st,
                                                 lmask& done, float& wq, bool& grazed) {
	float sx, sy, rho3d, depth, alpha, rho2d;
	{
#pragma clang fp contract(off)
		const v2f Tw = R.Twxy();
		const v2f X = pix * Tw.x - R.TuvX();
		const v2f Y = pix * Tw.y - R.TuvY();
		const v2f Z = pix * R.Twz() - R.TuvZ();
		const v2f a = Y * Z.yx;
		const v2f b = Z * X.yx;
		const v2f c = X * Y.yx;
		const float ppx = a.x - a.y, ppy = b.x - b.y, pz = c.x - c.y;
		const lmask unstable = LMASK(fabsf(pz) < 1e-4f);
		if (__builtin_expect(unstable == 0ull, 1)) {
			const float inv = div_nr(1.0f, pz);
			sx = ppx * inv; sy = ppy * inv;
			rho3d = sx * sx + sy * sy;
		} else {
			if constexpr (TRAIN) grazed = true;
			const float inv = div_nr(1.0f, selm(unstable, 1.0f, pz));
			sx = selm(unstable, 0.f, ppx * inv); sy = selm(unstable, 0.f, ppy * inv);
			rho3d = selm(unstable, 1e8f, sx * sx + sy * sy);
		}
		const v2f d = R.xy() - pix;
		const v2f d2 = d * d;
		rho2d = S_FILTER_INV_SQ * (d2.x + d2.y);
		const v2f st2 = mk2(sx, sy) * Tw;
		depth = (st2.x + st2.y) + R.Twz();
	}
	const float power = -0.5f * min_raw(rho3d, rho2d);
	alpha = fminf(0.99f, R.opac() * exp_neg(power));
	const lmask live = LMASK(!(depth < S_NEAR)) & LMASK(!(alpha < 1.0f / 255.0f)) & ~done;
	const float test_T = st.T * (1 - alpha);
	const lmask sat = LMASK(test_T < 0.0001f) & live;
	const lmask ok = live & ~sat;
	done |= sat;
	if constexpr (TRAIN) wq = 0.f;
	if (ok != 0ull) {
		const float w = selm0(ok, alpha * st.T);
		const v2f w2 = mk2(w, w);
		if constexpr (TRAIN) {
			const float dep = selm(ok, depth, 1.0f);
			const float A = 1 - st.T;
			const float m = S_FAR / (S_FAR - S_NEAR) * (1 - S_NEAR * __builtin_amdgcn_rcpf(dep));
			st.distortion += (m * m * A + st.M2 - 2 * m * st.DM.y) * w;
			st.M2 += m * (m * w);
			st.DM = __builtin_elementwise_fma(mk2(dep, m), w2, st.DM);
			if (med_live) {
				const lmask med = ok & LMASK(st.T > 0.5f);
				st.median_depth = selm(med, dep, st.median_depth);
				st.median_contributor = selm(med, (float)contributor, st.median_contributor);
			}
		}
		st.Nxy = __builtin_elementwise_fma(R.nxy(), w2, st.Nxy);
		st.NzR = __builtin_elementwise_fma(mk2(R.nz(), R.refl()), w2, st.NzR);
		st.Crg = __builtin_elementwise_fma(R.rg(), w2, st.Crg);
		st.C2 = fmaf(R.b(), w, st.C2);
		if constexpr (TRAIN) st.maskacc = fmaf(R.mask(), w, st.maskacc);
		st.T = selm(ok, test_T, st.T);
		if constexpr (TRAIN) {
			st.last_contributor = selmu(ok, contributor, st.last_contributor);
			wq = w;
		}
	}
	return ok;
}

struct SurfelReflFwd {
	const float* cam;
	const float* cubemap;
	const float4* rgba;
	const float* fail_value;
	int L;
	uint32_t no_key;
	float* out_final;
	float* out_refl_color;
	float* out_nworld;
	uint32_t* sort_keys;
};
struct SurfelEvalFwd {
	SurfelReflFwd refl;
	float* out_alpha;
	float* out_normal;
};
__device__ __forceinline__ const SurfelReflFwd& refl_args(const SurfelReflFwd& a) { return a; }
__device__ __forceinline__ const SurfelReflFwd& refl_args(const SurfelEvalFwd& a) { return a.refl; }
template <bool REFL, bool TRAIN, bool COUNT = false>
__global__ void __launch_bounds__(64) GSR_FWD_ATTR
surfel_render_fwd_wave_kernel(const uint2* __restrict__ ranges, const uint32_t* __restrict__ tile_order, const uint32_t* __restrict__ point_list, int W, int H, int tiles_x, int ntiles,
                              const float4* __restrict__ rec, const float4* __restrict__ bbox, int cull, const float* __restrict__ bg,
                              float* __restrict__ final_T, uint32_t* __restrict__ n_contrib, float* __restrict__ out_color,
                              float* __restrict__ out_others, float* __restrict__ out_refl, float* __restrict__ gaussian_weights,
                              unsigned long long* __restrict__ blend_mask, size_t mask_stride,
                              std::conditional_t<TRAIN, SurfelReflFwd, SurfelEvalFwd> args, PairCount<COUNT> pairs) {
	const SurfelReflFwd& rf = refl_args(args);
	const uint32_t slot = xcd_slot(blockIdx.x);
	if (slot >= (uint32_t)ntiles * 4u) return;
	const TileBlock blk = tile_block(tile_order, slot, tiles_x);
	if (blk.bx0 >= W || blk.by0 >= H) return;
	const uint32_t tile = blk.tile, quad = blk.quad;
	const int lane = threadIdx.x, bx0 = blk.bx0, by0 = blk.by0;
	const int px = bx0 + sub_px(lane), py = by0 + sub_py(lane);
	const bool inside = px < W && py < H;
	const v2f pix = mk2((float)px, (float)py);
	const uint2 range = ranges[tile];
	const int count = (int)(range.y - range.x);
	const float qx0 = (float)bx0, qy0 = (float)by0;

	__shared__ uint32_t s_hid[WBATCH];
	__shared__ uint32_t s_hc[TRAIN ? WBATCH : 1];
	__shared__ float4 s_wmax[TRAIN ? WBATCH : 1];

	lmask done = ~LMASK(px < W) | ~LMASK(py < H);
	LiveBox<true> box(qx0, qy0);
	uint32_t npairs = 0;
	SurfelFwdPix st;
	st.T = 1.0f;
	st.C2 = st.M2 = st.distortion = st.median_depth = st.maskacc = 0.f;
	st.median_contributor = -1.0f;
	st.Crg = st.Nxy = st.NzR = st.DM = mk2(0.f, 0.f);
	st.last_contributor = 0;
	bool med_live = true;
	const size_t batch0 = (size_t)(range.x / WBATCH) + tile;
	const uint32_t wmax_off = (uint32_t)row_reduce_slot(lane) * 16u + (uint32_t)(lane >> 4) * 4u;

	for (int base = 0; base < count; base += WBATCH) {
		if (done == ~0ull) break;
		const int nb = min(WBATCH, count - base);
		bool hit = lane < nb;
		uint32_t id = 0;
		if (!pairs.whole_block()) box.refresh(done, qx0, qy0);
		if (hit) {
			id = point_list[range.x + (uint32_t)(base + lane)];
			if (cull) {
				hit = cull_hit(bbox[2 * id], bbox[2 * id + 1], box.x0, box.x1, box.y0, box.y1);
			}
		}
		const unsigned long long mm = __ballot(hit);
		const int nh = __popcll(mm);
		if (nh == 0) continue;
		if constexpr (TRAIN) s_wmax[lane] = make_float4(0.f, 0.f, 0.f, 0.f);
		const int kown = __popcll(mm & ((1ull << lane) - 1ull));
		if (hit) {
			s_hid[kown] = id;
			if constexpr (TRAIN) s_hc[kown] = (uint32_t)(base + lane + 1);
		}
		__syncthreads();
		const uint32_t hid = lane < nh ? s_hid[lane] : 0u;
		const uint32_t hc = TRAIN && lane < nh ? s_hc[lane] : 0u;
		using Rec = SurfelRec;
		auto fetch = [&](int k) { return Rec{fetch_rec<S_REC_F4>(rec, hid, k)}; };
		Rec A = fetch(0), B = A;
		unsigned long long force = 0ull;
		for (int k = 0; k < nh; k += 4) {
			float w0 = 0.f, w1 = 0.f, w2 = 0.f, w3 = 0.f;
			lmask any = 0ull;
			bool stop, grazed = false;
			{
				const uint32_t c = __builtin_amdgcn_readlane(hc, k);
				if (k + 1 < nh) B = fetch(k + 1);
				any |= surfel_fwd_pair<TRAIN>(A, pix, c, med_live, st, done, w0, grazed);
				if constexpr (COUNT) npairs++;
				stop = done == ~0ull || k + 1 >= nh;
			}
			if (!stop) {
				const uint32_t c = __builtin_amdgcn_readlane(hc, k + 1);
				if (k + 2 < nh) A = fetch(k + 2);
				any |= surfel_fwd_pair<TRAIN>(B, pix, c, med_live, st, done, w1, grazed);
				if constexpr (COUNT) npairs++;
				stop = done == ~0ull || k + 2 >= nh;
			}
			if (!stop) {
				const uint32_t c = __builtin_amdgcn_readlane(hc, k + 2);
				if (k + 3 < nh) B = fetch(k + 3);
				any |= surfel_fwd_pair<TRAIN>(A, pix, c, med_live, st, done, w2, grazed);
				if constexpr (COUNT) npairs++;
				stop = done == ~0ull || k + 3 >= nh;
			}
			if (!stop) {
				const uint32_t c = __builtin_amdgcn_readlane(hc, k + 3);
				if (k + 4 < nh) A = fetch(k + 4);
				any |= surfel_fwd_pair<TRAIN>(B, pix, c, med_live, st, done, w3, grazed);
				if constexpr (COUNT) npairs++;
				stop = done == ~0ull;
			}
			if constexpr (TRAIN) {
				if (grazed) force |= 0xFull << k;
				if (any != 0ull) {
					const float z = row_max4(w0, w1, w2, w3);
					reinterpret_cast<float*>(s_wmax)[(k * 16 + wmax_off) >> 2] = z;
					med_live = med_live && LMASK(st.T > 0.5f) != 0ull;
				}
			}
			if (stop) break;
		}
		__syncthreads();
		if constexpr (!TRAIN) continue;
		float4 r = make_float4(0.f, 0.f, 0.f, 0.f);
		if (hit) {
			r = s_wmax[kown];
			const float m = fmaxf(fmaxf(r.x, r.y), fmaxf(r.z, r.w));
			if (m > 0.f) atomicMax(reinterpret_cast<int*>(gaussian_weights) + id, __float_as_int(m));
		}
		const lmask forced = __ballot(hit && ((force >> kown) & 1ull) != 0ull);
		const lmask b0 = LMASK(r.x > 0.f) | forced, b1 = LMASK(r.y > 0.f) | forced, b2 = LMASK(r.z > 0.f) | forced, b3 = LMASK(r.w > 0.f) | forced;
		if (lane < 4) {
			const lmask mine = lane == 0 ? b0 : (lane == 1 ? b1 : (lane == 2 ? b2 : b3));
			blend_mask[(batch0 + (size_t)(base / WBATCH)) * 16u + quad * 4u + (uint32_t)lane] = mine;
		}
		__syncthreads();
	}
	if constexpr (COUNT) {
		if (lane == 0) atomicAdd(pairs.word, (unsigned long long)npairs);
	}
	if (inside) {
		const size_t HW = (size_t)H * W;
		const size_t p = (size_t)W * py + px;
		const float T = st.T;
		if constexpr (TRAIN) {
			final_T[p] = T;
			final_T[HW + p] = st.DM.y;
			final_T[2 * HW + p] = st.M2;
			n_contrib[p] = st.last_contributor;
			n_contrib[HW + p] = (uint32_t)fmaxf(st.median_contributor, 0.0f);
		}
		const float c0 = st.Crg.x + T * bg[0], c1 = st.Crg.y + T * bg[1], c2 = st.C2 + T * bg[2];
		out_color[p] = c0;
		out_color[HW + p] = c1;
		out_color[2 * HW + p] = c2;
		out_refl[p] = st.NzR.y;
		if (REFL) {
			ReflFwdOut ro;
			refl_forward_pixel<true>(rf.cam, rf.cubemap, rf.rgba, rf.fail_value, rf.L, st.Nxy.x, st.Nxy.y, st.NzR.x, px, py, st.NzR.y, c0, c1, c2, rf.no_key, ro);
			if constexpr (TRAIN) {
				if (rf.sort_keys) rf.sort_keys[p] = ro.key;
			}
#pragma unroll
			for (int ch = 0; ch < 3; ch++) {
				rf.out_final[ch * HW + p] = ro.final_c[ch];
				rf.out_refl_color[ch * HW + p] = ro.refl_c[ch];
			}
			rf.out_nworld[p] = ro.nx;
			rf.out_nworld[HW + p] = ro.ny;
			rf.out_nworld[2 * HW + p] = ro.nz;
		}
		if constexpr (TRAIN) {
			out_others[0 * HW + p] = st.DM.x;
			out_others[1 * HW + p] = 1 - T;
			out_others[2 * HW + p] = st.Nxy.x;
			out_others[3 * HW + p] = st.Nxy.y;
			out_others[4 * HW + p] = st.NzR.x;
			out_others[5 * HW + p] = st.median_depth;
			out_others[6 * HW + p] = st.distortion;
			out_others[7 * HW + p] = st.maskacc > 0.f ? 1.0f : 0.f;
		} else {
			args.out_alpha[p] = 1 - T;
			if (args.out_normal) {
				args.out_normal[p] = st.Nxy.x;
				args.out_normal[HW + p] = st.Nxy.y;
				args.out_normal[2 * HW + p] = st.NzR.x;
			}
		}
	}
}

struct SurfelBwdPix {
	float T, T_final, last_dL_dT, bg_dot_dpixel;
	int last_contributor, median_contributor;
	v2f dp01, dn01, dnzr;
	v2f pixs;
	float dp2, dL_ddepth, dL_daccum, dL_dmedian_depth;
	float FD2r, FAr, FDr;
	float A, Dprev, last_alpha;
};
__device__ __forceinline__ void surfel_bwd_init(SurfelBwdPix& s, bool inside, size_t pix, size_t HW, const float* __restrict__ bg,
                                                const float* __restrict__ final_Ts, const uint32_t* __restrict__ n_contrib,
                                                const float* __restrict__ dL_dpixels, const float* __restrict__ dL_depths,
                                                const float* __restrict__ dL_drefl_map, const float* __restrict__ dL_dnormal_extra) {
	s.T_final = inside ? final_Ts[pix] : 0.f;
	s.T = s.T_final;
	s.last_contributor = inside ? (int)n_contrib[pix] : 0;
	s.median_contributor = inside ? (int)n_contrib[HW + pix] : 0;
	s.dp01 = s.dn01 = s.dnzr = mk2(0.f, 0.f);
	s.dp2 = s.dL_ddepth = s.dL_daccum = s.dL_dmedian_depth = 0.f;
	float dL_dreg = 0.f;
	if (inside) {
		s.dp01 = mk2(dL_dpixels[pix], dL_dpixels[HW + pix]);
		s.dp2 = dL_dpixels[2 * HW + pix];
		s.dL_ddepth = dL_depths[0 * HW + pix];
		s.dL_daccum = dL_depths[1 * HW + pix];
		s.dn01 = mk2(dL_depths[2 * HW + pix], dL_depths[3 * HW + pix]);
		s.dnzr = mk2(dL_depths[4 * HW + pix], dL_drefl_map[pix]);
		s.dL_dmedian_depth = dL_depths[5 * HW + pix];
		dL_dreg = dL_depths[6 * HW + pix];
		if (dL_dnormal_extra) {
			s.dn01 += mk2(dL_dnormal_extra[pix], dL_dnormal_extra[HW + pix]);
			s.dnzr.x += dL_dnormal_extra[2 * HW + pix];
		}
	}
	s.FDr = (inside ? final_Ts[HW + pix] : 0.f) * dL_dreg;
	s.FD2r = (inside ? final_Ts[2 * HW + pix] : 0.f) * dL_dreg;
	s.FAr = (1 - s.T_final) * dL_dreg;
	s.last_dL_dT = 0;
	s.A = s.Dprev = s.last_alpha = 0.f;
	s.bg_dot_dpixel = bg[0] * s.dp01.x + bg[1] * s.dp01.y + bg[2] * s.dp2;
}
__device__ __forceinline__ lmask surfel_bwd_pair(SurfelBwdPix& s, const SurfelRec& R, const v2f pix, int contributor, lmask inside_m, float* v) {
	v2f X, Y, Z, d;
	float sx, sy, rho3d, rho2d, depth, inv_pz;
	{
#pragma clang fp contract(off)
		const v2f Tw = R.Twxy();
		X = pix * Tw.x - R.TuvX();
		Y = pix * Tw.y - R.TuvY();
		Z = pix * R.Twz() - R.TuvZ();
		const v2f a = Y * Z.yx;
		const v2f b = Z * X.yx;
		const v2f c = X * Y.yx;
		const float ppx = a.x - a.y, ppy = b.x - b.y, pz = c.x - c.y;
		const lmask unstable = LMASK(fabsf(pz) < 1e-6f);
		if (__builtin_expect(unstable == 0ull, 1)) {
			inv_pz = div_nr(1.0f, pz);
			sx = ppx * inv_pz; sy = ppy * inv_pz;
			rho3d = sx * sx + sy * sy;
		} else {
			inv_pz = div_nr(1.0f, selm(unstable, 1.0f, pz));
			sx = selm(unstable, 0.f, ppx * inv_pz); sy = selm(unstable, 0.f, ppy * inv_pz);
			rho3d = selm(unstable, 1e8f, sx * sx + sy * sy);
		}
		d = R.xy() - pix;
		const v2f d2 = d * d;
		rho2d = S_FILTER_INV_SQ * (d2.x + d2.y);
		const v2f st2 = mk2(sx, sy) * Tw;
		depth = (st2.x + st2.y) + R.Twz();
	}
	const float power = -0.5f * min_raw(rho3d, rho2d);
	const float G = exp_neg(power);
	const float alpha_raw = fminf(0.99f, R.opac() * G);
	const lmask ok = LMASK(!(depth < S_NEAR)) & LMASK(!(alpha_raw < 1.0f / 255.0f)) & LMASK(contributor < s.last_contributor) & inside_m;
	const float alpha = selm0(ok, alpha_raw);
	const float c_d = selm(ok, depth, 1.0f);
	const v2f sxy = mk2(selm0(ok, sx), selm0(ok, sy));
	const float inv_1ma = div_nr(1.0f, 1.f - alpha);
	s.T *= inv_1ma;
	const float T = s.T;
	const float w = alpha * T;
	const v2f w2 = mk2(w, w);
	v2f Dv = R.rg() * s.dp01;
	Dv = __builtin_elementwise_fma(R.nxy(), s.dn01, Dv);
	Dv = __builtin_elementwise_fma(mk2(R.nz(), R.refl()), s.dnzr, Dv);
	const float D = (Dv.x + Dv.y) + R.b() * s.dp2 + c_d * s.dL_ddepth + s.dL_daccum;
	s.A = s.last_alpha * s.Dprev + (1.f - s.last_alpha) * s.A;
	s.Dprev = D;
	s.last_alpha = alpha;
	float dL_dalpha = D - s.A;
	const v2f vc = w2 * s.dp01, vn = w2 * s.dn01, vz = w2 * s.dnzr;
	v[SA_COLOR + 0] = vc.x;
	v[SA_COLOR + 1] = vc.y;
	v[SA_COLOR + 2] = w * s.dp2;
	v[SA_REFL] = vz.y;
	v[SA_NORMAL + 0] = vn.x;
	v[SA_NORMAL + 1] = vn.y;
	v[SA_NORMAL + 2] = vz.x;
	const float rc = div_nr(1.0f, c_d);
	const float m_d = S_FAR / (S_FAR - S_NEAR) * (1 - S_NEAR * rc);
	const float dmd_dd = (S_FAR * S_NEAR / (S_FAR - S_NEAR)) * rc * rc;
	const float dL_dweight = s.FD2r + m_d * (m_d * s.FAr - 2 * s.FDr);
	dL_dalpha += dL_dweight - s.last_dL_dT;
	s.last_dL_dT = dL_dweight * alpha + (1 - alpha) * s.last_dL_dT;
	const float dL_dmd = 2.0f * w * (m_d * s.FAr - s.FDr);
	float dL_dz = dL_dmd * dmd_dd + w * s.dL_ddepth;
	dL_dz += (contributor == s.median_contributor - 1) ? s.dL_dmedian_depth : 0.f;
	dL_dalpha *= T;
	dL_dalpha -= s.T_final * inv_1ma * s.bg_dot_dpixel;
	dL_dalpha = selm0(ok, dL_dalpha);
	dL_dz = selm0(ok, dL_dz);
	const float nG = -G * (R.opac() * dL_dalpha);
	const lmask use3d = LMASK(rho3d <= rho2d);
	const v2f dL_ds = __builtin_elementwise_fma(mk2(nG, nG), sxy, mk2(dL_dz, dL_dz) * R.Twxy());
	const v2f dp = mk2(selm0(use3d, dL_ds.x), selm0(use3d, dL_ds.y)) * inv_pz;
	const v2f dps = dp * sxy;
	const float dpz = -(dps.x + dps.y);
	const v2f dpx2 = mk2(dp.x, dp.x), dpy2 = mk2(dp.y, dp.y), dpz2 = mk2(dpz, dpz);
	const v2f N1 = __builtin_elementwise_fma(Z, dpy2, -(Y * dpz2));
	const v2f N2 = __builtin_elementwise_fma(X, dpz2, -(Z * dpx2));
	const v2f N3 = __builtin_elementwise_fma(Y, dpx2, -(X * dpy2));
	v[SA_T + 0] = N1.y; v[SA_T + 1] = N2.y; v[SA_T + 2] = N3.y;
	v[SA_T + 3] = N1.x; v[SA_T + 4] = N2.x; v[SA_T + 5] = N3.x;
	const v2f t1 = N1 * s.pixs, t2 = N2 * s.pixs, t3 = N3 * s.pixs;
	v[SA_T + 6] = dL_dz * sxy.x - (t1.y + t1.x);
	v[SA_T + 7] = dL_dz * sxy.y - (t2.y + t2.x);
	v[SA_T + 8] = dL_dz - (t3.y + t3.x);
	const v2f gm = d * selm(use3d, 0.f, nG * S_FILTER_INV_SQ);
	v[SA_MEAN2D + 0] = gm.x;
	v[SA_MEAN2D + 1] = gm.y;
	v[SA_OPAC] = G * dL_dalpha;
	return ok;
}

#ifndef S_CAP
#define S_CAP 48
#endif
__device__ __forceinline__ void
surfel_render_bwd_rows_body(const uint2* __restrict__ ranges, const uint32_t* __restrict__ tile_order, const uint32_t* __restrict__ point_list, int W, int H, int tiles_x, int ntiles,
                            const float* __restrict__ bg, const float4* __restrict__ rec, int dev_flags, const float* __restrict__ final_Ts,
                            const uint32_t* __restrict__ n_contrib, const float* __restrict__ dL_dpixels, const float* __restrict__ dL_depths,
                            const float* __restrict__ dL_drefl_map, const float* __restrict__ dL_dnormal_extra, float* __restrict__ acc,
                            const unsigned long long* __restrict__ blend_mask) {
	const uint32_t slot = xcd_slot(blockIdx.x);
	if (slot >= (uint32_t)ntiles * 4u) return;
	const TileBlock blk = tile_block(tile_order, slot, tiles_x);
	if (blk.bx0 >= W || blk.by0 >= H) return;
	const uint32_t tile = blk.tile, quad = blk.quad;
	const int lane = threadIdx.x, row = lane >> 4, bx0 = blk.bx0, by0 = blk.by0;
	const int px = bx0 + sub_px(lane), py = by0 + sub_py(lane);
	const bool inside = px < W && py < H;
	const lmask inside_m = LMASK(px < W) & LMASK(py < H);
	const v2f pixv = mk2((float)px, (float)py);
	const uint2 range = ranges[tile];
	const int count = (int)(range.y - range.x);
	const size_t HW = (size_t)H * W;
	const size_t pix = (size_t)W * py + px;

	__shared__ float s_slab[(S_CAP + 2) * S_ACC_F];
	__shared__ float4 s_rec[WBATCH * S_REC_F4];
	__shared__ uint32_t s_cw[WBATCH];
#if GSR_BWD_LIST
	__shared__ uint8_t s_list[64];
#endif
	static_assert(S_CAP + 1 < 64, "slab slots are packed into 6 bits");
	static_assert(S_CAP >= 32, "a chunk always takes the first 8-position group of its batch, up to 4 rows x 8 = 32 pairs");

	SurfelBwdPix st;
	surfel_bwd_init(st, inside, pix, HW, bg, final_Ts, n_contrib, dL_dpixels, dL_depths, dL_drefl_map, dL_dnormal_extra);
	st.pixs = mk2(-pixv.y, pixv.x);
	int wave_last = st.last_contributor;
#pragma unroll
	for (int off = 32; off > 0; off >>= 1) wave_last = max(wave_last, __shfl_xor(wave_last, off));
	wave_last = __builtin_amdgcn_readfirstlane(wave_last);
	if (wave_last == 0) return;
	if (lane < S_ACC_F) s_slab[(S_CAP + 1) * S_ACC_F + lane] = 0.f;
	const uint32_t slab_lane = (uint32_t)row_reduce_slot(lane) * 4u;
	const unsigned long long lt = (1ull << lane) - 1ull, gt = ~((2ull << lane) - 1ull);
	const uint32_t fl_k = (uint32_t)lane / S_ACC_F, fl_d = (uint32_t)lane - fl_k * S_ACC_F;
	const bool fl_on = lane < 3 * S_ACC_F && fl_d < S_ACC_F - 1;
	float* const fl_acc = acc + fl_d;
	const char* const slab_b = reinterpret_cast<const char*>(s_slab);

	const size_t batch0 = (size_t)(range.x / WBATCH) + tile;
	for (int b = (min(wave_last, count) - 1) / WBATCH; b >= 0; b--) {
		const unsigned long long* mp = blend_mask + ((batch0 + (size_t)b) * 16u + quad * 4u);
		const lmask m0 = mp[0], m1 = mp[1], m2 = mp[2], m3 = mp[3];
		const lmask any = (m0 | m1) | (m2 | m3);
		if (any == 0ull) continue;
		uint32_t id = 0u;
		if ((any >> lane) & 1ull) {
			id = point_list[range.x + (uint32_t)(b * WBATCH + lane)];
			const float4* q = rec + (size_t)id * S_REC_F4;
			const float4 r0 = q[0], r1 = q[1], r2 = q[2], r3 = q[3];
			float4 r4 = q[4];
			r4.w = __uint_as_float(id);
			float4* d = s_rec + lane * S_REC_F4;
			d[0] = r0; d[1] = r1; d[2] = r2; d[3] = r3; d[4] = r4;
		}
		const uint32_t jany = 63u - (uint32_t)__builtin_clzll(any);
		lmask todo = any;
		while (todo != 0ull) {
			lmask c = ~0ull;
			if (__popcll(m0 & todo) + __popcll(m1 & todo) + __popcll(m2 & todo) + __popcll(m3 & todo) > S_CAP) {
				c = 0ull;
#pragma unroll 1
				for (int e = 7; e >= 0; e--) {
					const lmask em = (0xFFull << (8 * e)) & todo;
					if (em == 0ull) continue;
					const lmask cc = c | em;
					if (c != 0ull && __popcll(m0 & cc) + __popcll(m1 & cc) + __popcll(m2 & cc) + __popcll(m3 & cc) > S_CAP) break;
					c = cc;
				}
			}
			const lmask c0 = m0 & todo & c, c1 = m1 & todo & c, c2 = m2 & todo & c, c3 = m3 & todo & c, call = any & todo & c;
			todo &= ~c;
			const int n0 = __popcll(c0), n1 = __popcll(c1), n2 = __popcll(c2), n3 = __popcll(c3);
			const int nmax = __builtin_amdgcn_readfirstlane(max(max(n0, n1), max(n2, n3)));
			const int nent = __popcll(call);
			if ((call >> lane) & 1ull) {
				const uint32_t s0 = ((c0 >> lane) & 1ull) ? (uint32_t)__popcll(c0 & gt) : (uint32_t)(S_CAP + 1);
				const uint32_t s1 = ((c1 >> lane) & 1ull) ? (uint32_t)(n0 + __popcll(c1 & gt)) : (uint32_t)(S_CAP + 1);
				const uint32_t s2 = ((c2 >> lane) & 1ull) ? (uint32_t)(n0 + n1 + __popcll(c2 & gt)) : (uint32_t)(S_CAP + 1);
				const uint32_t s3 = ((c3 >> lane) & 1ull) ? (uint32_t)(n0 + n1 + n2 + __popcll(c3 & gt)) : (uint32_t)(S_CAP + 1);
				const int k = __popcll(call & lt);
				s_cw[k] = s0 | (s1 << 6) | (s2 << 12) | (s3 << 18) | ((uint32_t)lane << 24);
#if GSR_BWD_LIST
				if ((c0 >> lane) & 1ull) s_list[s0] = (uint8_t)lane;
				if ((c1 >> lane) & 1ull) s_list[s1] = (uint8_t)lane;
				if ((c2 >> lane) & 1ull) s_list[s2] = (uint8_t)lane;
				if ((c3 >> lane) & 1ull) s_list[s3] = (uint8_t)lane;
#endif
			}
			__syncthreads();
#if !GSR_BWD_LIST
			unsigned long long left = __builtin_bitreverse64(row == 0 ? c0 : (row == 1 ? c1 : (row == 2 ? c2 : c3)));
#else
			const int nrow = row == 0 ? n0 : (row == 1 ? n1 : (row == 2 ? n2 : n3));
#endif
			const uint32_t rowbase = (uint32_t)(row == 0 ? 0 : (row == 1 ? n0 : (row == 2 ? n0 + n1 : n0 + n1 + n2)));
			uint32_t myslot = rowbase * (S_ACC_F * 4u) + slab_lane;
#pragma unroll GSR_BWD_UNROLL
			for (int t = 0; t < nmax; t++) {
#if !GSR_BWD_LIST
				const uint32_t lo = (uint32_t)left, hi = (uint32_t)(left >> 32);
				const lmask valid = LMASK((lo | hi) != 0u);
				const uint32_t tz = min(ffbl_raw(lo), ffbl_raw(hi) | 32u);
				const uint32_t j = selmu(valid, 63u - tz, jany);
				left &= left - 1ull;
#else
				const lmask valid = LMASK(t < nrow);
				const uint32_t j = selmu(valid, (uint32_t)s_list[min(rowbase + (uint32_t)t, 63u)], jany);
#endif
				const float4* q = reinterpret_cast<const float4*>(reinterpret_cast<const char*>(s_rec) + __umul24(j, S_REC_F4 * 16u));
				const SurfelRec R{q[0], q[1], q[2], q[3], q[4]};
				float v[S_ACC_F];
				v[S_ACC_F - 1] = 0.f;
				surfel_bwd_pair(st, R, pixv, b * WBATCH + (int)j, inside_m & valid, v);
				float z[5];
				row_reduce20(v, z);
				float* slab = reinterpret_cast<float*>(reinterpret_cast<char*>(s_slab) + selmu(valid, myslot, (uint32_t)(S_CAP * S_ACC_F * 4) + slab_lane));
				myslot += S_ACC_F * 4u;
#pragma unroll
				for (int g = 0; g < 5; g++) slab[4 * g] = z[g];
			}
			__syncthreads();
#pragma unroll 1
			for (int k0 = 0; k0 < nent; k0 += 3) {
				const uint32_t k = (uint32_t)k0 + fl_k;
				if (fl_on && k < (uint32_t)nent) {
					const uint32_t w = s_cw[k];
					const uint32_t eid = __float_as_uint(s_rec[(w >> 24) * S_REC_F4 + 4].w);
					const char* base = slab_b + fl_d * 4u;
					const float a0 = *reinterpret_cast<const float*>(base + (w & 0x3Fu) * (S_ACC_F * 4u));
					const float a1 = *reinterpret_cast<const float*>(base + ((w >> 6) & 0x3Fu) * (S_ACC_F * 4u));
					const float a2 = *reinterpret_cast<const float*>(base + ((w >> 12) & 0x3Fu) * (S_ACC_F * 4u));
					const float a3 = *reinterpret_cast<const float*>(base + ((w >> 18) & 0x3Fu) * (S_ACC_F * 4u));
					if (!(dev_flags & 1)) atomicAdd(fl_acc + (size_t)eid * S_ACC_F, (a0 + a1) + (a2 + a3));
				}
			}
			__syncthreads();
		}
	}
}

__global__ void __launch_bounds__(64) __attribute__((amdgpu_waves_per_eu(GSR_BWD_WPE, GSR_BWD_WPE)))
surfel_render_bwd_rows_kernel(const uint2* __restrict__ ranges, const uint32_t* __restrict__ tile_order, const uint32_t* __restrict__ point_list, int W, int H, int tiles_x, int ntiles,
                              const float* __restrict__ bg, const float4* __restrict__ rec, int dev_flags, const float* __restrict__ final_Ts,
                              const uint32_t* __restrict__ n_contrib, const float* __restrict__ dL_dpixels, const float* __restrict__ dL_depths,
                              const float* __restrict__ dL_drefl_map, const float* __restrict__ dL_dnormal_extra, float* __restrict__ acc,
                              const unsigned long long* __restrict__ blend_mask) {
	surfel_render_bwd_rows_body(ranges, tile_order, point_list, W, H, tiles_x, ntiles, bg, rec, dev_flags, final_Ts, n_contrib, dL_dpixels, dL_depths,
	                            dL_drefl_map, dL_dnormal_extra, acc, blend_mask);
}

__device__ __forceinline__ void quat_vjp(float w, float x, float y, float z, const M3& v_R, float* v_quat) {
	v_quat[0] = 2.f * (x * (v_R.m[1][2] - v_R.m[2][1]) + y * (v_R.m[2][0] - v_R.m[0][2]) + z * (v_R.m[0][1] - v_R.m[1][0]));
	v_quat[1] = 2.f * (-2.f * x * (v_R.m[1][1] + v_R.m[2][2]) + y * (v_R.m[0][1] + v_R.m[1][0]) + z * (v_R.m[0][2] + v_R.m[2][0]) + w * (v_R.m[1][2] - v_R.m[2][1]));
	v_quat[2] = 2.f * (x * (v_R.m[0][1] + v_R.m[1][0]) - 2.f * y * (v_R.m[0][0] + v_R.m[2][2]) + z * (v_R.m[1][2] + v_R.m[2][1]) + w * (v_R.m[2][0] - v_R.m[0][2]));
	v_quat[3] = 2.f * (x * (v_R.m[0][2] + v_R.m[2][0]) + y * (v_R.m[1][2] + v_R.m[2][1]) - 2.f * z * (v_R.m[0][0] + v_R.m[1][1]) + w * (v_R.m[0][1] - v_R.m[1][0]));
}

template <bool ACC>
__global__ void __launch_bounds__(256)
surfel_preprocess_bwd_kernel(int P, int D, int M, const float* __restrict__ means, const int* __restrict__ radii, const float* __restrict__ shs,
                             const uint8_t* __restrict__ clamped, const float* __restrict__ scales, const float* __restrict__ rotations,
                             const float4* __restrict__ rec, RasterCam cam, const float* __restrict__ acc, float* __restrict__ dL_dmean2D,
                             float* __restrict__ dL_dnormal, float* __restrict__ dL_dopacity, float* __restrict__ dL_dcolor,
                             float* __restrict__ dL_drefl, float* __restrict__ dL_dmean3D, float* __restrict__ dL_dtransMat,
                             float* __restrict__ dL_dsh, float* __restrict__ dL_dscale, float* __restrict__ dL_drot) {
	__shared__ __attribute__((aligned(16))) float s_tile[4][1368];
	const int lane = threadIdx.x & 63;
	float* tile = s_tile[threadIdx.x >> 6];
	const int idx_raw = blockIdx.x * 256 + threadIdx.x;
	const int g0 = idx_raw - lane, nrows = min(64, P - g0);
	if (nrows <= 0) return;
	const bool in_range = idx_raw < P;
	const int idx = in_range ? idx_raw : P - 1;
	const float4* a4 = reinterpret_cast<const float4*>(acc + (size_t)idx * S_ACC_F);
	const float4 a0 = a4[0], a1 = a4[1], a2 = a4[2], a3 = a4[3], a4v = a4[4];
	const float gcol[3] = {a0.x, a0.y, a0.z};
	const float gnrm[3] = {a1.x, a1.y, a1.z};
	float dT[9] = {a2.x, a2.y, a2.z, -a2.w, -a3.x, -a3.y, a3.z, a3.w, a4v.x};
	const float gm2x = a4v.y, gm2y = a4v.z;
	if (in_range) {
		put<ACC>(dL_drefl + idx, a0.w);
		put<ACC>(dL_dopacity + idx, a1.w);
	}

	float dmean[3] = {0.f, 0.f, 0.f}, dscale[2] = {0.f, 0.f}, drot[4] = {0.f, 0.f, 0.f, 0.f};
	float out_m2x = gm2x, out_m2y = gm2y;
	float dTout[9];
#pragma unroll
	for (int i = 0; i < 9; i++) dTout[i] = dT[i];
	const bool visible = radii[idx] > 0;
	const float mx = means[3 * idx], my = means[3 * idx + 1], mz = means[3 * idx + 2];
	if (visible) {
		const int Wb = f2i(cam.focal_x * cam.tan_fovx * 2);
		const int Hb = f2i(cam.focal_y * cam.tan_fovy * 2);
		const bool precomp = (scales == nullptr);
		M3 T;
		F3 normal = f3(0.f, 0.f, 0.f);
		P34 Pm;
		M3 R;
		float qw = 0, qx = 0, qy = 0, qz = 0, sc0 = 0, sc1 = 0;
		const float4* rc = rec + (size_t)idx * S_REC_F4;
		if (precomp) {
			const float4 r0 = rc[0], r1 = rc[1], r2 = rc[2];
			T = m3_make(r0.z, r1.x, r1.z, r0.w, r1.y, r1.w, r2.x, r2.y, r2.z);
		} else {
			R = quat_to_rotmat(rotations + 4 * idx, qw, qx, qy, qz);
			sc0 = scales[2 * idx]; sc1 = scales[2 * idx + 1];
			const float L0[3] = {R.m[0][0] * sc0, R.m[0][1] * sc0, R.m[0][2] * sc0};
			const float L1[3] = {R.m[1][0] * sc1, R.m[1][1] * sc1, R.m[1][2] * sc1};
			Pm = make_P(cam.proj, Wb, Hb);
#pragma unroll
			for (int j = 0; j < 3; j++) {
				T.m[j][0] = L0[0] * Pm.m[j][0] + L0[1] * Pm.m[j][1] + L0[2] * Pm.m[j][2];
				T.m[j][1] = L1[0] * Pm.m[j][0] + L1[1] * Pm.m[j][1] + L1[2] * Pm.m[j][2];
				T.m[j][2] = mx * Pm.m[j][0] + my * Pm.m[j][1] + mz * Pm.m[j][2] + Pm.m[j][3];
			}
			const float* vm = cam.view;
			const float nx = R.m[2][0], ny = R.m[2][1], nz = R.m[2][2];
			normal = f3(vm[0] * nx + vm[4] * ny + vm[8] * nz, vm[1] * nx + vm[5] * ny + vm[9] * nz, vm[2] * nx + vm[6] * ny + vm[10] * nz);
		}
		M3 dL_dT = m3_make(dT[0], dT[1], dT[2], dT[3], dT[4], dT[5], dT[6], dT[7], dT[8]);
		bool early = false;
		if (gm2x != 0 || gm2y != 0) {
			const float tv[3] = {9.0f, 9.0f, -1.0f};
			const float d = tv[0] * (T.m[2][0] * T.m[2][0]) + tv[1] * (T.m[2][1] * T.m[2][1]) + tv[2] * (T.m[2][2] * T.m[2][2]);
			const float invd = 1.0f / d;
			float fv[3], dL_df[3], dT3[3];
#pragma unroll
			for (int r = 0; r < 3; r++) fv[r] = tv[r] * invd;
#pragma unroll
			for (int r = 0; r < 3; r++) {
				dL_dT.m[0][r] += gm2x * fv[r] * T.m[2][r];
				dL_dT.m[1][r] += gm2y * fv[r] * T.m[2][r];
				dT3[r] = gm2x * fv[r] * T.m[0][r] + gm2y * fv[r] * T.m[1][r];
				dL_df[r] = gm2x * T.m[0][r] * T.m[2][r] + gm2y * T.m[1][r] * T.m[2][r];
			}
			const float dL_dd = (float)((double)(dL_df[0] * fv[0] + dL_df[1] * fv[1] + dL_df[2] * fv[2]) * (-1.0 / (double)d));
#pragma unroll
			for (int r = 0; r < 3; r++) dL_dT.m[2][r] += dT3[r] + dL_dd * (tv[r] * T.m[2][r] * 2.0f);
			if (precomp) {
#pragma unroll
				for (int c = 0; c < 3; c++)
#pragma unroll
					for (int r = 0; r < 3; r++) dTout[3 * c + r] = dL_dT.m[c][r];
				early = true;
			}
		}
		if (!precomp && !early) {
			float dM[3][3];
#pragma unroll
			for (int j = 0; j < 3; j++)
#pragma unroll
				for (int r = 0; r < 3; r++) dM[j][r] = Pm.m[0][r] * dL_dT.m[0][j] + Pm.m[1][r] * dL_dT.m[1][j] + Pm.m[2][r] * dL_dT.m[2][j];
			const float* vm = cam.view;
			float tnx = vm[0] * gnrm[0] + vm[1] * gnrm[1] + vm[2] * gnrm[2];
			float tny = vm[4] * gnrm[0] + vm[5] * gnrm[1] + vm[6] * gnrm[2];
			float tnz = vm[8] * gnrm[0] + vm[9] * gnrm[1] + vm[10] * gnrm[2];
			const float pvx = vm[0] * mx + vm[4] * my + vm[8] * mz + vm[12];
			const float pvy = vm[1] * mx + vm[5] * my + vm[9] * mz + vm[13];
			const float pvz = vm[2] * mx + vm[6] * my + vm[10] * mz + vm[14];
			const float cosv = -((pvx * normal.x) + (pvy * normal.y) + (pvz * normal.z));
			const float mult = cosv > 0 ? 1.f : -1.f;
			tnx *= mult; tny *= mult; tnz *= mult;
			M3 dL_dR;
#pragma unroll
			for (int r = 0; r < 3; r++) {
				dL_dR.m[0][r] = dM[0][r] * sc0;
				dL_dR.m[1][r] = dM[1][r] * sc1;
			}
			dL_dR.m[2][0] = tnx; dL_dR.m[2][1] = tny; dL_dR.m[2][2] = tnz;
			quat_vjp(qw, qx, qy, qz, dL_dR, drot);
			dscale[0] = dM[0][0] * R.m[0][0] + dM[0][1] * R.m[0][1] + dM[0][2] * R.m[0][2];
			dscale[1] = dM[1][0] * R.m[1][0] + dM[1][1] * R.m[1][1] + dM[1][2] * R.m[1][2];
			dmean[0] = dM[2][0]; dmean[1] = dM[2][1]; dmean[2] = dM[2][2];
		}
		float depth;
		{
#pragma clang fp contract(off)
			depth = precomp ? rc[2].z : ((mx * cam.proj[3] + my * cam.proj[7]) + mz * cam.proj[11]) + cam.proj[15];
		}
		out_m2x = (float)((double)(dTout[2] * depth) * 0.5 * (double)float(Wb));
		out_m2y = (float)((double)(dTout[5] * depth) * 0.5 * (double)float(Hb));
	}
	if (shs != nullptr) {
		if (M == 16) {
			float w[16];
			F3 grgb = f3(0.f, 0.f, 0.f);
#pragma unroll
			for (int k = 0; k < 16; k++) w[k] = 0.f;
			if (visible && (gcol[0] != 0.f || gcol[1] != 0.f || gcol[2] != 0.f)) {
				ShRow s;
				load_sh(shs, idx, M, (D + 1) * (D + 1), s);
				const F3 dir = f3(mx - cam.campos[0], my - cam.campos[1], mz - cam.campos[2]);
				grgb = f3(gcol[0], gcol[1], gcol[2]);
				const F3 dm = sh_backward_weights(D, s, dir, clamped[idx], grgb, w);
				dmean[0] += dm.x; dmean[1] += dm.y; dmean[2] += dm.z;
			}
			float4* sh_out = reinterpret_cast<float4*>(dL_dsh) + (size_t)g0 * 12;
#pragma unroll
			for (int t = 0; t < 3; t++) {
				const float4 q4[4] = {sh_row_f4(4 * t, w, grgb), sh_row_f4(4 * t + 1, w, grgb), sh_row_f4(4 * t + 2, w, grgb), sh_row_f4(4 * t + 3, w, grgb)};
				wave_store_rows4<4, ACC>(reinterpret_cast<float4*>(tile), q4, sh_out, 12, 4 * t, nrows, lane);
			}
		} else if (in_range) {
			if (visible) {
				ShRow s;
				load_sh(shs, idx, M, (D + 1) * (D + 1), s);
				const F3 dir = f3(mx - cam.campos[0], my - cam.campos[1], mz - cam.campos[2]);
				const F3 dm = sh_backward<ACC>(idx, D, M, s, dir, clamped[idx], f3(gcol[0], gcol[1], gcol[2]), dL_dsh);
				dmean[0] += dm.x; dmean[1] += dm.y; dmean[2] += dm.z;
			} else if (!ACC) {
				float* out = dL_dsh + (size_t)idx * M * 3;
				for (int q = 0; q < M * 3; q++) out[q] = 0.f;
			}
		}
	}
	const float m2d[3] = {out_m2x, out_m2y, 0.f};
	if (dL_dcolor != nullptr) wave_store_rows<3, false>(tile, gcol, dL_dcolor + (size_t)g0 * 3, nrows, lane);
	if (dL_dnormal != nullptr) wave_store_rows<3, false>(tile, gnrm, dL_dnormal + (size_t)g0 * 3, nrows, lane);
	wave_store_rows<3, false>(tile, m2d, dL_dmean2D + (size_t)g0 * 3, nrows, lane);
	wave_store_rows<3, ACC>(tile, dmean, dL_dmean3D + (size_t)g0 * 3, nrows, lane);
	if (dL_dtransMat != nullptr) wave_store_rows<9, false>(tile, dTout, dL_dtransMat + (size_t)g0 * 9, nrows, lane);
	if (in_range) {
		put<ACC>(dL_dscale + 2 * idx, dscale[0]); put<ACC>(dL_dscale + 2 * idx + 1, dscale[1]);
		float4* rq = reinterpret_cast<float4*>(dL_drot) + idx;
		if (ACC) {
			if (drot[0] != 0.f || drot[1] != 0.f || drot[2] != 0.f || drot[3] != 0.f) {
				const float4 r0 = *rq;
				*rq = make_float4(r0.x + drot[0], r0.y + drot[1], r0.z + drot[2], r0.w + drot[3]);
			}
		} else {
			*rq = make_float4(drot[0], drot[1], drot[2], drot[3]);
		}
	}
}

}

using namespace gsr;

static int check_refl_descriptor(const char* entry, const gsr_refl_forward* refl, int width, int height) {
	if (!refl) return 0;
	if (!refl->cam || !refl->cubemap || !refl->fail_value || refl->L == 0 || !refl->cubemap_rgba || ((uintptr_t)refl->cubemap_rgba & 15) != 0 ||
	    !refl->out_final || !refl->out_refl_color || !refl->out_normal_world) {
		set_error("%s: incomplete reflection descriptor (cam, cubemap, fail_value, L, 16-byte aligned cubemap_rgba and the three outputs are required)", entry);
		return GSR_E_INVALID;
	}
	if ((size_t)6 * refl->L * refl->L >= 0xFFFFFFFFull) { set_error("%s: cubemap too large", entry); return GSR_E_INVALID; }
	if (refl->scratch && !refl->sort_keys) { set_error("%s: refl->scratch is the place the sort keys are sorted into: it needs refl->sort_keys", entry); return GSR_E_INVALID; }
	if (refl->scratch) return refl_scratch_check(entry, refl->L, width, height, refl->scratch, refl->scratch_floats);
	return 0;
}
static int check_surfel_inputs(const char* entry, const char* missing, int P, int D, int M, const float* means3D, const float* shs,
                               const float* colors_precomp, const float* refl_strengths, const float* scales, const float* rotations,
                               const float* transMat_precomp, const float* viewmatrix, const float* projmatrix, const float* cam_pos, const int* radii) {
	if (P <= 0) return 0;
	if (!means3D || !refl_strengths || !viewmatrix || !projmatrix || !cam_pos || !radii || (!shs && !colors_precomp) ||
	    ((!scales || !rotations) && !transMat_precomp)) {
		set_error("%s: %s", entry, missing);
		return GSR_E_INVALID;
	}
	return check_sh_input(entry, D, M, shs);
}
#define SURFEL_FWD_MISSING "missing required input pointer"

static int early_key_sort(const gsr_refl_forward* refl, int width, int height, int R, hipStream_t stream) {
	if (!refl || !refl->sort_keys || !refl->scratch) return 0;
	return refl_sort_keys_early(refl->L, width, height, refl->scratch, refl->scratch_floats, refl->sort_keys, refl->async_sort, R > 0, stream);
}

template <bool TRAIN>
static int surfel_forward(gsr_alloc_fn alloc, void* alloc_user, int P, int D, int M, const float* background, int width, int height,
                          const float* means3D, const uint8_t* env_scope_mask, const float* shs, const float* colors_precomp,
                          const float* refl_strengths, const float* opacities, const float* scales, float scale_modifier,
                          const float* rotations, const float* transMat_precomp, const float* viewmatrix, const float* projmatrix,
                          const float* cam_pos, float tan_fovx, float tan_fovy, int prefiltered, float* out_color, float* out_others,
                          float* out_alpha, float* out_normal_view, float* out_refl_strength_map, int* radii, float* gaussian_weights,
                          const gsr_refl_forward* refl, int debug, hipStream_t stream) {
	const size_t HW = (size_t)width * height;
	int R = 0;
	if (P == 0) {
		float* normal = TRAIN ? out_others + 2 * HW : out_normal_view;
		if (!normal) {
			normal = static_cast<float*>(alloc(alloc_user, GSR_BUF_IMAGE, HW * 3 * 4));
			if (!normal) { set_error("workspace allocation failed (%zu bytes)", HW * 3 * 4); return GSR_E_ALLOC; }
		}
		GSR_HIP_CHECK(hipMemsetAsync(out_color, 0, HW * 3 * 4, stream));
		if (TRAIN) {
			GSR_HIP_CHECK(hipMemsetAsync(out_others, 0, HW * 8 * 4, stream));
		} else {
			GSR_HIP_CHECK(hipMemsetAsync(out_alpha, 0, HW * 4, stream));
			GSR_HIP_CHECK(hipMemsetAsync(normal, 0, HW * 3 * 4, stream));
		}
		GSR_HIP_CHECK(hipMemsetAsync(out_refl_strength_map, 0, HW * 4, stream));
		if (refl && gsr_deferred_reflection_forward_keys(normal, out_color, out_refl_strength_map, refl->cam, refl->cubemap, refl->fail_value, refl->L,
		                                                 width, height, refl->out_final, refl->out_refl_color, refl->out_normal_world, refl->cubemap_rgba,
		                                                 refl->sort_keys, stream) < 0)
			return GSR_E_HIP;
	} else {
		const int tiles_x = (width + 15) / 16, tiles_y = (height + 15) / 16;
		const int ntiles = tiles_x * tiles_y;
		GeomState geom; ImageState img;
		if (const int rc = forward_workspace(alloc, alloc_user, TRAIN ? SURFEL_LAYOUT : SURFEL_LAYOUT.inference(), P, HW, ntiles, &geom, &img); rc < 0) return rc;

		if (prefiltered) GSR_HIP_CHECK(hipMemsetAsync(geom.flags, 0, 4 * sizeof(int), stream));
		const RasterCam cam = make_cam(viewmatrix, projmatrix, cam_pos, width, height, tan_fovx, tan_fovy);
		CubemapInterleave ci{nullptr, nullptr, 0u, 1u};
		SurfelReflFwd rf{};
		if (refl) {
			ci = CubemapInterleave{refl->cubemap, reinterpret_cast<float4*>(refl->cubemap_rgba), 6u * refl->L * refl->L, refl->L * refl->L};
			rf = SurfelReflFwd{refl->cam, refl->cubemap, reinterpret_cast<const float4*>(refl->cubemap_rgba), refl->fail_value, (int)refl->L, 6u * refl->L * refl->L,
			                   refl->out_final, refl->out_refl_color, refl->out_normal_world, refl->sort_keys};
		}
	{ StageTimer st_(GSR_STAGE_PREPROCESS, stream); 	surfel_preprocess_kernel<TRAIN><<<(P + 255) / 256, 256, 0, stream>>>(P, D, M, means3D, scales, scale_modifier, rotations, opacities, shs,
		                                                                     transMat_precomp, colors_precomp, refl_strengths, env_scope_mask, cam, radii, geom,
		                                                                     tiles_x, tiles_y, prefiltered, gaussian_weights, ci); }
		GSR_LAUNCH_CHECK(debug, stream);

		BinningState bin;
		R = run_binning(alloc, alloc_user, P, tiles_x, tiles_y, geom, img, &bin, prefiltered, debug, stream, TRAIN);
		if (R < 0) return R;

	{ StageTimer st_(GSR_STAGE_RENDER_FWD, stream);
		const int nunits = (int)xcd_grid((uint32_t)ntiles * 4u);
		const auto args = [&] { if constexpr (TRAIN) return rf; else return SurfelEvalFwd{rf, out_alpha, out_normal_view}; }();
		auto launch = [&](auto render, auto pairs) {
			render<<<nunits, 64, 0, stream>>>(img.ranges, img.tile_order, bin.point_list, width, height, tiles_x, ntiles, geom.rec, geom.bbox, option_cull(),
			                                  background, TRAIN ? img.final_T : nullptr, TRAIN ? img.n_contrib : nullptr, out_color, out_others,
			                                  out_refl_strength_map, gaussian_weights, bin.blend_mask, bin.mask_stride, args, pairs);
		};
		if (option_dev() & 2) {
			unsigned long long* word = dev_pair_counter();
			if (!word) { set_error("gsr_surfel_forward: no pair counter"); return GSR_E_HIP; }
			launch(refl ? surfel_render_fwd_wave_kernel<true, TRAIN, true> : surfel_render_fwd_wave_kernel<false, TRAIN, true>, PairCount<true>{word, option_dev() & 4});
		} else {
			launch(refl ? surfel_render_fwd_wave_kernel<true, TRAIN> : surfel_render_fwd_wave_kernel<false, TRAIN>, PairCount<false>{});
		} }
		GSR_LAUNCH_CHECK(debug, stream);
	}
	if (const int rc = TRAIN ? early_key_sort(refl, width, height, R, stream) : 0; rc < 0) return rc;
	return R;
}

extern "C" int gsr_surfel_forward_refl(gsr_alloc_fn alloc, void* alloc_user, int P, int D, int M, const float* background, int width, int height,
                                  const float* means3D, const uint8_t* env_scope_mask, const float* shs, const float* colors_precomp,
                                  const float* refl_strengths, const float* opacities, const float* scales, float scale_modifier,
                                  const float* rotations, const float* transMat_precomp, const float* viewmatrix, const float* projmatrix,
                                  const float* cam_pos, float tan_fovx, float tan_fovy, int prefiltered, float* out_color, float* out_others,
                                  float* out_refl_strength_map, int* radii, float* gaussian_weights, const gsr_refl_forward* refl, int debug,
                                  void* stream_) {
	if (!alloc || P < 0 || width <= 0 || height <= 0 || !background || !out_color || !out_others || !out_refl_strength_map) {
		set_error("gsr_surfel_forward: invalid argument");
		return GSR_E_INVALID;
	}
	if (P > 0 && (!gaussian_weights || !opacities)) { set_error("gsr_surfel_forward: " SURFEL_FWD_MISSING); return GSR_E_INVALID; }
	if (const int rc = check_refl_descriptor("gsr_surfel_forward_refl", refl, width, height); rc < 0) return rc;
	if (const int rc = check_surfel_inputs("gsr_surfel_forward", SURFEL_FWD_MISSING, P, D, M, means3D, shs, colors_precomp, refl_strengths, scales, rotations,
	                                       transMat_precomp, viewmatrix, projmatrix, cam_pos, radii); rc < 0) return rc;
	return surfel_forward<true>(alloc, alloc_user, P, D, M, background, width, height, means3D, env_scope_mask, shs, colors_precomp, refl_strengths,
	                            opacities, scales, scale_modifier, rotations, transMat_precomp, viewmatrix, projmatrix, cam_pos, tan_fovx, tan_fovy,
	                            prefiltered, out_color, out_others, nullptr, nullptr, out_refl_strength_map, radii, gaussian_weights, refl, debug,
	                            (hipStream_t)stream_);
}

extern "C" int gsr_surfel_forward(gsr_alloc_fn alloc, void* alloc_user, int P, int D, int M, const float* background, int width, int height,
                                  const float* means3D, const uint8_t* env_scope_mask, const float* shs, const float* colors_precomp,
                                  const float* refl_strengths, const float* opacities, const float* scales, float scale_modifier,
                                  const float* rotations, const float* transMat_precomp, const float* viewmatrix, const float* projmatrix,
                                  const float* cam_pos, float tan_fovx, float tan_fovy, int prefiltered, float* out_color, float* out_others,
                                  float* out_refl_strength_map, int* radii, float* gaussian_weights, int debug, void* stream_) {
	return gsr_surfel_forward_refl(alloc, alloc_user, P, D, M, background, width, height, means3D, env_scope_mask, shs, colors_precomp, refl_strengths, opacities,
	                               scales, scale_modifier, rotations, transMat_precomp, viewmatrix, projmatrix, cam_pos, tan_fovx, tan_fovy, prefiltered, out_color,
	                               out_others, out_refl_strength_map, radii, gaussian_weights, nullptr, debug, stream_);
}

extern "C" int gsr_surfel_forward_eval(gsr_alloc_fn alloc, void* alloc_user, int P, int D, int M, const float* background, int width, int height,
                                       const float* means3D, const float* shs, const float* colors_precomp, const float* refl_strengths,
                                       const float* opacities, const float* scales, float scale_modifier, const float* rotations,
                                       const float* transMat_precomp, const float* viewmatrix, const float* projmatrix, const float* cam_pos,
                                       float tan_fovx, float tan_fovy, int prefiltered, float* out_color, float* out_alpha,
                                       float* out_normal_view, float* out_refl_strength_map, int* radii, const gsr_refl_forward* refl,
                                       int debug, void* stream_) {
	if (!alloc || P < 0 || width <= 0 || height <= 0 || !background || !out_color || !out_alpha || !out_refl_strength_map) {
		set_error("gsr_surfel_forward_eval: invalid argument (alloc, P >= 0, width, height, background, out_color, out_alpha, out_refl_strength_map)");
		return GSR_E_INVALID;
	}
	if (!out_normal_view && !refl) { set_error("gsr_surfel_forward_eval: out_normal_view may be NULL only with refl"); return GSR_E_INVALID; }
	if (refl && (refl->sort_keys || refl->scratch)) {
		set_error("gsr_surfel_forward_eval: refl->sort_keys and refl->scratch must be NULL (the eval forward has no backward)");
		return GSR_E_INVALID;
	}
	if (const int rc = check_refl_descriptor("gsr_surfel_forward_eval", refl, width, height); rc < 0) return rc;
	if (P > 0 && !opacities) { set_error("gsr_surfel_forward_eval: " SURFEL_FWD_MISSING); return GSR_E_INVALID; }
	if (const int rc = check_surfel_inputs("gsr_surfel_forward_eval", SURFEL_FWD_MISSING, P, D, M, means3D, shs, colors_precomp, refl_strengths, scales, rotations,
	                                       transMat_precomp, viewmatrix, projmatrix, cam_pos, radii); rc < 0) return rc;
	return surfel_forward<false>(alloc, alloc_user, P, D, M, background, width, height, means3D, nullptr, shs, colors_precomp, refl_strengths, opacities,
	                             scales, scale_modifier, rotations, transMat_precomp, viewmatrix, projmatrix, cam_pos, tan_fovx, tan_fovy, prefiltered,
	                             out_color, nullptr, out_alpha, out_normal_view, out_refl_strength_map, radii, nullptr, refl, debug, (hipStream_t)stream_);
}

extern "C" int gsr_surfel_backward_ex(int P, int D, int M, int R, const float* background, int width, int height, const float* means3D,
                                   const float* shs, const float* colors_precomp, const float* refl_strengths, const float* scales,
                                   float scale_modifier, const float* rotations, const float* transMat_precomp, const float* viewmatrix,
                                   const float* projmatrix, const float* cam_pos, float tan_fovx, float tan_fovy, const int* radii,
                                   void* geom_buffer, void* binning_buffer, void* image_buffer, const float* dL_dpix, const float* dL_dothers,
                                   const float* dL_drefl_strength_map, float* dL_dmean2D, float* dL_dnormal, float* dL_dopacity, float* dL_dcolor,
                                   float* dL_drefl_strengths, float* dL_dmean3D, float* dL_dtransMat, float* dL_dsh, float* dL_dscale,
                                   float* dL_drot, int accumulate, const float* dL_dnormal_extra, int debug, void* stream_) {
	(void)scale_modifier;
	hipStream_t stream = (hipStream_t)stream_;
	if (const int rc = check_surfel_inputs("gsr_surfel_backward", "missing required pointer", P, D, M, means3D, shs, colors_precomp, refl_strengths, scales,
	                                       rotations, transMat_precomp, viewmatrix, projmatrix, cam_pos, radii); rc < 0) return rc;
	const bool missing = !background || !geom_buffer || !image_buffer || (R > 0 && !binning_buffer) || !dL_dpix || !dL_dothers || !dL_drefl_strength_map ||
	    !dL_dmean2D || !dL_dopacity || !dL_drefl_strengths || !dL_dmean3D || !dL_dscale || !dL_drot || (!shs && !dL_dcolor) || (!scales && !dL_dtransMat) ||
	    (shs && !dL_dsh);
	BackwardWorkspace w;
	if (const int rc = backward_prologue("gsr_surfel_backward", __func__, SURFEL_LAYOUT, P, M, R, width, height, missing, shs, dL_dsh, dL_drot, nullptr, nullptr,
	                                     geom_buffer, binning_buffer, image_buffer, stream, &w); rc <= 0) return rc;
	const GeomState& geom = w.geom; const ImageState& img = w.img; const BinningState& bin = w.bin;
	const int tiles_x = w.tiles_x, ntiles = w.ntiles;
	if (R > 0) {
		{ const int rc = side_gate_wait(stream); if (rc < 0) return rc; }
{ StageTimer st_(GSR_STAGE_RENDER_BWD, stream);
		const int nunits = (int)xcd_grid((uint32_t)ntiles * 4u);
		surfel_render_bwd_rows_kernel<<<nunits, 64, 0, stream>>>(img.ranges, img.tile_order, bin.point_list, width, height, tiles_x, ntiles, background, geom.rec,
		                                                         option_dev(), img.final_T, img.n_contrib, dL_dpix, dL_dothers, dL_drefl_strength_map, dL_dnormal_extra,
		                                                         geom.acc, bin.blend_mask); }
		GSR_LAUNCH_CHECK(debug, stream);
	}
	const RasterCam cam = make_cam(viewmatrix, projmatrix, cam_pos, width, height, tan_fovx, tan_fovy);
{ StageTimer st_(GSR_STAGE_PREPROCESS_BWD, stream);
	auto kern = accumulate ? surfel_preprocess_bwd_kernel<true> : surfel_preprocess_bwd_kernel<false>;
	kern<<<(P + 255) / 256, 256, 0, stream>>>(P, D, M, means3D, radii, shs, geom.clamped, scales, rotations, geom.rec, cam, geom.acc, dL_dmean2D, dL_dnormal,
	                                          dL_dopacity, dL_dcolor, dL_drefl_strengths, dL_dmean3D, dL_dtransMat, dL_dsh, dL_dscale, dL_drot); }
	GSR_LAUNCH_CHECK(debug, stream);
	return 0;
}

extern "C" int gsr_surfel_backward(int P, int D, int M, int R, const float* background, int width, int height, const float* means3D,
                                   const float* shs, const float* colors_precomp, const float* refl_strengths, const float* scales,
                                   float scale_modifier, const float* rotations, const float* transMat_precomp, const float* viewmatrix,
                                   const float* projmatrix, const float* cam_pos, float tan_fovx, float tan_fovy, const int* radii,
                                   void* geom_buffer, void* binning_buffer, void* image_buffer, const float* dL_dpix, const float* dL_dothers,
                                   const float* dL_drefl_strength_map, float* dL_dmean2D, float* dL_dnormal, float* dL_dopacity, float* dL_dcolor,
                                   float* dL_drefl_strengths, float* dL_dmean3D, float* dL_dtransMat, float* dL_dsh, float* dL_dscale,
                                   float* dL_drot, int debug, void* stream_) {
	return gsr_surfel_backward_ex(P, D, M, R, background, width, height, means3D, shs, colors_precomp, refl_strengths, scales, scale_modifier, rotations,
	                              transMat_precomp, viewmatrix, projmatrix, cam_pos, tan_fovx, tan_fovy, radii, geom_buffer, binning_buffer, image_buffer,
	                              dL_dpix, dL_dothers, dL_drefl_strength_map, dL_dmean2D, dL_dnormal, dL_dopacity, dL_dcolor, dL_drefl_strengths, dL_dmean3D,
	                              dL_dtransMat, dL_dsh, dL_dscale, dL_drot, 0, nullptr, debug, stream_);
}

extern "C" int gsr_surfel_backward_accum(int P, int D, int M, int R, const float* background, int width, int height, const float* means3D,
                                   const float* shs, const float* colors_precomp, const float* refl_strengths, const float* scales,
                                   float scale_modifier, const float* rotations, const float* transMat_precomp, const float* viewmatrix,
                                   const float* projmatrix, const float* cam_pos, float tan_fovx, float tan_fovy, const int* radii,
                                   void* geom_buffer, void* binning_buffer, void* image_buffer, const float* dL_dpix, const float* dL_dothers,
                                   const float* dL_drefl_strength_map, float* dL_dmean2D, float* dL_dnormal, float* dL_dopacity, float* dL_dcolor,
                                   float* dL_drefl_strengths, float* dL_dmean3D, float* dL_dtransMat, float* dL_dsh, float* dL_dscale,
                                   float* dL_drot, int accumulate, int debug, void* stream_) {
	return gsr_surfel_backward_ex(P, D, M, R, background, width, height, means3D, shs, colors_precomp, refl_strengths, scales, scale_modifier, rotations,
	                              transMat_precomp, viewmatrix, projmatrix, cam_pos, tan_fovx, tan_fovy, radii, geom_buffer, binning_buffer, image_buffer,
	                              dL_dpix, dL_dothers, dL_drefl_strength_map, dL_dmean2D, dL_dnormal, dL_dopacity, dL_dcolor, dL_drefl_strengths, dL_dmean3D,
	                              dL_dtransMat, dL_dsh, dL_dscale, dL_drot, accumulate, nullptr, debug, stream_);
}
```

gaussian-splatting-reflection_amd/gaussian_renderer/__init__.py:

```python
import math
import os
import sys
import threading

import numpy as np
import torch

sys.path.insert(0, os.path.dirname(os.path.dirname(os.path.abspath(__file__))))
import _gsr
from _gsr import check, lib, ptr, stream_ptr
from _raster_api import GradSink, call_backward, call_forward, named_tensors
import diff_surfel_rasterization as _dsr
from diff_surfel_rasterization import GaussianRasterizationSettings, GaussianRasterizer


class _Block:

    def __init__(self, sources, extra, value):
        self.sources, self.versions, self.extra, self.value = sources, [t._version for t in sources], extra, value
        self.ready, self.ordered = None, set()
        if value.is_cuda:
            built_on = torch.cuda.current_stream(value.device)
            self.ready = torch.cuda.Event()
            self.ready.record(built_on)
            self.ordered.add(built_on.cuda_stream)

    def matches(self, sources, extra):
        return (len(sources) == len(self.sources) and all(a is b for a, b in zip(sources, self.sources)) and
                all(t._version == v for t, v in zip(sources, self.versions)) and extra == self.extra)

    def on_current_stream(self):
        if self.ready is not None:
            cur = torch.cuda.current_stream(self.value.device)
            if cur.cuda_stream not in self.ordered:
                cur.wait_event(self.ready)
                self.value.record_stream(cur)
                self.ordered.add(cur.cuda_stream)
        return self.value


_blocks = {}
_BLOCKS_KEPT = 64


_blocks_mu = threading.Lock()


def _cached_block(kind, sources, extra, build):
    hit = None
    with _blocks_mu:
        kept = _blocks.setdefault(kind, [])
        for k in range(len(kept) - 1, -1, -1):
            if kept[k].matches(sources, extra):
                hit = kept.pop(k)
                kept.append(hit)
                break
    if hit is not None:
        return hit.on_current_stream()
    value = build()
    block = _Block(list(sources), extra, value)
    with _blocks_mu:
        kept = _blocks.setdefault(kind, [])
        kept.append(block)
        if len(kept) > _BLOCKS_KEPT:
            del kept[0]
    return value


def _cam_block(world_view_transform, HWK, R, T):
    Kb = np.asarray(HWK[2], dtype=np.float32)

    def build():
        dev = world_view_transform.device
        Kinv = torch.tensor(np.linalg.inv(Kb), dtype=torch.float32, device=dev)
        Rw = R.T.contiguous().float()
        Tf = T.float()
        centre = (-Rw.T @ Tf.unsqueeze(-1)).flatten()
        return torch.cat([world_view_transform[:3, :3].contiguous().float().reshape(-1), Kinv.reshape(-1), Rw.reshape(-1), Tf.reshape(-1),
                          centre.reshape(-1)]).contiguous()
    return _cached_block("cam", (world_view_transform, R, T), (int(HWK[0]), int(HWK[1]), Kb.tobytes()), build)


def _ray_block(view):
    wvt, fpt = view.world_view_transform, view.full_proj_transform
    W, H = int(view.image_width), int(view.image_height)

    def build():
        wv, fp = wvt.contiguous(), fpt.contiguous()
        c2w = (wv.T).inverse()
        ndc2pix = torch.tensor([[W / 2, 0, 0, W / 2], [0, H / 2, 0, H / 2], [0, 0, 0, 1]], dtype=torch.float32, device=wvt.device).T
        intrins = ((c2w.T @ fp) @ ndc2pix)[:3, :3].T
        M = intrins.inverse().T @ c2w[:3, :3].T
        return torch.cat([M.reshape(-1), c2w[:3, 3].reshape(-1)]).float().contiguous()
    return _cached_block("ray", (wvt, fpt), (W, H), build)


REFLECTION_BACKWARD_BINNED = True
REFLECTION_FORWARD_KEYS = True


class _DeferredReflection(torch.autograd.Function):
    @staticmethod
    def forward(ctx, normal_view, base_color, refl_strength, cubemap, fail_value, cam, sink):
        nv, bc, rs = normal_view.float().contiguous(), base_color.float().contiguous(), refl_strength.float().contiguous()
        cm, fv = cubemap.float().contiguous(), fail_value.float().contiguous()
        if cm.shape[1] != 3:
            raise RuntimeError("deferred_reflection: the cubemap must have 3 channels")
        H, W = nv.shape[1], nv.shape[2]
        final = torch.empty_like(bc)
        refl_color = torch.empty_like(bc)
        normal_world = torch.empty_like(nv)
        rgba = torch.empty(6 * cm.shape[2] * cm.shape[3] * 4, dtype=torch.float32, device=cm.device)
        keys = None
        if REFLECTION_BACKWARD_BINNED and REFLECTION_FORWARD_KEYS and any(ctx.needs_input_grad[:5]):
            keys = torch.empty(H * W, dtype=torch.int32, device=cm.device)
        with torch.cuda.device(nv.device):
            check(lib.gsr_deferred_reflection_forward_keys(ptr(nv), ptr(bc), ptr(rs), ptr(cam), ptr(cm), ptr(fv), cm.shape[2], W, H, ptr(final),
                                                         ptr(refl_color), ptr(normal_world), ptr(rgba), ptr(keys), stream_ptr(nv.device)),
                  "gsr_deferred_reflection_forward")
        ctx.save_for_backward(nv, bc, rs, cm, fv, cam, rgba)
        ctx.sort_keys = keys
        ctx.sink = sink
        ctx.set_materialize_grads(False)
        return final, refl_color, normal_world

    @staticmethod
    def backward(ctx, g_final, g_refl_color, g_normal_world):
        return _reflection_backward(ctx.saved_tensors, (g_final, g_refl_color, g_normal_world), ctx.sink, ctx.sort_keys) + (None, None)


def _reflection_backward(saved, grads, sink, sort_keys, scratch=None):
    nv, bc, rs, cm, fv, cam, rgba = saved
    cont = lambda g: None if g is None else g.float().contiguous()
    g_final, g_refl_color, g_normal_world = grads
    g_final = torch.zeros_like(bc) if g_final is None else cont(g_final)
    g_refl_color, g_normal_world = cont(g_refl_color), cont(g_normal_world)
    H, W = nv.shape[1], nv.shape[2]
    tensors = sink.tensors if sink is not None else {}
    accumulate = sink is not None and sink.accumulate
    async_tail = sink is not None and sink.async_tail
    g_cm, g_fail = tensors.get("cubemap"), tensors.get("fail")
    sunk_cm, sunk_fail = g_cm is not None, g_fail is not None
    need_both = "=True needs both 'cubemap' and 'fail' tensors (accumulate / async_tail need both 'cubemap' and 'fail' tensors)"
    if accumulate and not (sunk_cm and sunk_fail):
        raise ValueError("reflection grad sink: accumulate" + need_both)
    for name, t, like in (("cubemap", g_cm, cm), ("fail", g_fail, fv)):
        if t is not None:
            _gsr.check_sink_tensor("reflection grad sink", name, t, like.shape, like.device, aligned=False)
    if async_tail and not (sunk_cm and sunk_fail):
        raise ValueError("reflection grad sink: async_tail" + need_both)
    g_cm = torch.empty_like(cm) if g_cm is None else g_cm
    g_fail = torch.empty_like(fv) if g_fail is None else g_fail
    keys_sorted = scratch is not None
    if not keys_sorted:
        scratch = torch.empty(int(lib.gsr_deferred_reflection_scratch_floats(int(cm.shape[2]), W, H, 1 if REFLECTION_BACKWARD_BINNED else 0)),
                              dtype=torch.float32, device=cm.device)
    g_nv, g_base, g_s = torch.empty_like(nv), torch.empty_like(bc), torch.empty_like(rs)
    with torch.cuda.device(nv.device):
        check(lib.gsr_deferred_reflection_backward_keys(ptr(nv), ptr(bc), ptr(rs), ptr(cam), ptr(cm), ptr(fv), cm.shape[2], W, H,
                                                        ptr(g_final), ptr(g_refl_color), ptr(g_normal_world), ptr(g_nv), ptr(g_base),
                                                        ptr(g_s), ptr(g_cm), ptr(g_fail), ptr(scratch), int(scratch.numel()), int(accumulate),
                                                        int(async_tail), ptr(rgba), ptr(sort_keys), int(keys_sorted), stream_ptr(nv.device)),
              "gsr_deferred_reflection_backward")
    if async_tail:
        _gsr.side_hold(scratch, g_cm, g_fail, sort_keys)
    return g_nv, g_base, g_s, (None if sunk_cm else g_cm), (None if sunk_fail else g_fail)


def deferred_reflection(normal_view, base_color, refl_strength_map, env_map, world_view_transform, HWK, R, T, grad_sink=None,
                        accumulate=False, async_tail=False):
    if async_tail and not grad_sink:
        raise ValueError("deferred_reflection: async_tail=True needs a grad_sink (autograd would read the gradient at once)")
    cam = _cam_block(world_view_transform, HWK, R, T)
    sink = GradSink(grad_sink, accumulate, async_tail) if grad_sink else None
    return _DeferredReflection.apply(normal_view, base_color, refl_strength_map, env_map.params['Cubemap_texture'],
                                     env_map.params['Cubemap_failv'], cam, sink)


FUSED_REFLECTION = True


class _RasterizeReflect(torch.autograd.Function):
    probe = None

    @staticmethod
    def forward(ctx, *args):
        v = GaussianRasterizer.variant
        t = named_tensors(v, args)
        cubemap, fail_value, cam, settings, raster_sink, refl_sink = args[len(v.tensors):]
        cm, fv = cubemap.float().contiguous(), fail_value.float().contiguous()
        if cm.dim() != 4 or cm.shape[1] != 3:
            raise RuntimeError("rasterize_reflect: the cubemap must be (6, 3, L, L)")
        want_keys = REFLECTION_BACKWARD_BINNED and REFLECTION_FORWARD_KEYS and any(ctx.needs_input_grad[len(v.tensors):len(v.tensors) + 2])
        early = want_keys and refl_sink is not None and refl_sink.async_tail and bool(refl_sink.tensors)
        ret = call_forward(v, t, settings, refl=dict(cam=cam, cubemap=cm, fail_value=fv, keys=want_keys, early_sort=early))
        num_rendered, (color, radii, others, refl_map, weights), buffers, _ = v.split_forward(ret[:9])
        final, refl_color, normal_world, rgba, keys, scratch = ret[9:]
        if scratch is not None:
            _gsr.side_hold(scratch, keys)
        ctx.raster_settings, ctx.num_rendered = settings, num_rendered
        ctx.raster_sink, ctx.refl_sink, ctx.sort_keys, ctx.scratch = raster_sink, refl_sink, keys, scratch
        ctx.passes = 0
        ctx.save_for_backward(*[t[k] for k in v.saved], radii, *buffers, color, others, refl_map, cm, fv, cam, rgba)
        ctx.mark_non_differentiable(radii, weights)
        ctx.set_materialize_grads(False)
        return final, refl_color, normal_world, color, radii, others, refl_map, weights

    @staticmethod
    def backward(ctx, g_final, g_refl_color, g_normal_world, g_color, _g_radii, g_others, g_refl_map, _g_weights):
        v = GaussianRasterizer.variant
        kept = ctx.saved_tensors
        ns = len(v.saved)
        saved = dict(zip(v.saved, kept[:ns]))
        radii, geom, binning, img, color, others, refl_map, cm, fv, cam, rgba = kept[ns:]
        cont = lambda g: None if g is None else g.float().contiguous()
        if ctx.scratch is not None and ctx.passes:
            with torch.cuda.device(cam.device):
                check(lib.gsr_side_join(stream_ptr(cam.device)), "gsr_side_join")
        ctx.passes += 1
        g_nv, g_base, g_s, g_cm, g_fail = _reflection_backward((others[2:5], color, refl_map, cm, fv, cam, rgba), (g_final, g_refl_color, g_normal_world),
                                                               ctx.refl_sink, ctx.sort_keys, ctx.scratch)
        g_color, g_refl_map, g_others = cont(g_color), cont(g_refl_map), cont(g_others)
        if g_color is not None:
            g_base.add_(g_color)
        if g_refl_map is not None:
            g_s.add_(g_refl_map)
        if g_others is None:
            g_others = torch.zeros_like(others)
        if _RasterizeReflect.probe is not None:
            _RasterizeReflect.probe.update(g_normal_view=g_nv.clone(), g_base=g_base.clone(), g_strength=g_s.clone())
        grads = call_backward(v, saved, ctx.raster_settings, [g_base, None, g_others, g_s, None], ctx.num_rendered, (geom, binning, img), radii,
                              ctx.raster_sink, extra_normal_grad=g_nv)
        return tuple(grads) + (g_cm, g_fail, None, None, None, None)


def rasterize_reflect(rasterizer, env_map, world_view_transform, HWK, R, T, means3D, means2D, opacities, shs=None, colors_precomp=None,
                      refl_strengths=None, scales=None, rotations=None, cov3D_precomp=None, env_scope_mask=None, refl_grad_sink=None,
                      accumulate=False, async_tail=False):
    if async_tail and not refl_grad_sink:
        raise ValueError("rasterize_reflect: async_tail=True needs a refl_grad_sink (autograd would read the gradient at once)")
    t = rasterizer._collect(means3D, means2D, opacities, shs=shs, colors_precomp=colors_precomp, refl_strengths=refl_strengths, scales=scales,
                            rotations=rotations, cov3D_precomp=cov3D_precomp, env_scope_mask=env_scope_mask)
    cam = _cam_block(world_view_transform, HWK, R, T)
    rsink = GradSink(refl_grad_sink, accumulate, async_tail) if refl_grad_sink else None
    return _RasterizeReflect.apply(*[t[name] for name in rasterizer.variant.tensors], env_map.params['Cubemap_texture'], env_map.params['Cubemap_failv'], cam,
                                   rasterizer.raster_settings, rasterizer._grad_sink, rsink)


def rasterize_eval(rasterizer, means3D, opacities, shs=None, colors_precomp=None, refl_strengths=None, scales=None, rotations=None,
                   cov3D_precomp=None, env_map=None, world_view_transform=None, HWK=None, R=None, T=None):
    inputs = (means3D, opacities, shs, colors_precomp, refl_strengths, scales, rotations, cov3D_precomp)
    if env_map is not None:
        inputs += (env_map.params['Cubemap_texture'], env_map.params['Cubemap_failv'])
    if torch.is_grad_enabled() and any(t is not None and t.requires_grad for t in inputs):
        raise RuntimeError("rasterize_eval has no backward; use rasterize_reflect / GaussianRasterizer")
    t = rasterizer._collect(means3D, None, opacities, shs=shs, colors_precomp=colors_precomp, refl_strengths=refl_strengths, scales=scales,
                            rotations=rotations, cov3D_precomp=cov3D_precomp, env_scope_mask=None)
    s = rasterizer.raster_settings
    refl = None
    if env_map is not None:
        refl = dict(cam=_cam_block(world_view_transform, HWK, R, T), cubemap=env_map.params['Cubemap_texture'].detach(),
                    fail_value=env_map.params['Cubemap_failv'].detach())
    ret = _dsr._C.rasterize_gaussians_eval(s.bg, t["means3D"], t["colors_precomp"], t["refl_strengths"], t["opacities"], t["scales"],
                                           t["rotations"], s.scale_modifier, t["cov3Ds_precomp"], s.viewmatrix, s.projmatrix, s.tanfovx, s.tanfovy,
                                           s.image_height, s.image_width, t["sh"], s.sh_degree, s.campos, s.prefiltered, s.debug, refl=refl)
    _, color, alpha, normal_view, refl_map, _ = ret[:6]
    if refl is None:
        return {"render": color, "rend_alpha": alpha, "rend_normal": normal_view, "refl_strength_map": refl_map}
    final, refl_color, normal_world = ret[6:]
    return {"render": final, "rend_alpha": alpha, "rend_normal": normal_world, "refl_strength_map": refl_map, "refl_color_map": refl_color,
            "base_color_map": color}


class _ShadingNormal(torch.autograd.Function):
    @staticmethod
    def forward(ctx, normal_view, cam):
        nv = normal_view.float().contiguous()
        out = torch.empty_like(nv)
        with torch.cuda.device(nv.device):
            check(lib.gsr_normal_world_forward(ptr(nv), ptr(cam), nv.shape[2], nv.shape[1], ptr(out), stream_ptr(nv.device)),
                  "gsr_normal_world_forward")
        ctx.save_for_backward(nv, cam)
        return out

    @staticmethod
    def backward(ctx, g):
        nv, cam = ctx.saved_tensors
        g_nv = torch.empty_like(nv)
        g = g.float().contiguous()
        with torch.cuda.device(nv.device):
            check(lib.gsr_normal_world_backward(ptr(nv), ptr(cam), nv.shape[2], nv.shape[1], ptr(g), ptr(g_nv), stream_ptr(nv.device)),
                  "gsr_normal_world_backward")
        return g_nv, None


def shading_normal(normal_view, world_view_transform, HWK, R, T):
    return _ShadingNormal.apply(normal_view, _cam_block(world_view_transform, HWK, R, T))


class _SurfacePass(torch.autograd.Function):
    @staticmethod
    def forward(ctx, allmap, raymat, depth_ratio):
        am = allmap.float().contiguous()
        if am.dim() != 3 or am.shape[0] != 8:
            raise RuntimeError("surface_pass: allmap must be (8,H,W)")
        H, W = am.shape[1], am.shape[2]
        sd = torch.empty((1, H, W), dtype=torch.float32, device=am.device)
        sn = torch.empty((3, H, W), dtype=torch.float32, device=am.device)
        with torch.cuda.device(am.device):
            check(lib.gsr_surface_forward(ptr(am), ptr(raymat), float(depth_ratio), H, W, ptr(sd), ptr(sn), stream_ptr(am.device)),
                  "gsr_surface_forward")
        ctx.save_for_backward(am, raymat, sd)
        ctx.depth_ratio = float(depth_ratio)
        ctx.set_materialize_grads(False)
        return sd, sn

    @staticmethod
    def backward(ctx, g_sd, g_sn):
        am, raymat, sd = ctx.saved_tensors
        H, W = am.shape[1], am.shape[2]
        g_am = torch.empty_like(am)
        g_sd = None if g_sd is None else g_sd.float().contiguous()
        g_sn = None if g_sn is None else g_sn.float().contiguous()
        with torch.cuda.device(am.device):
            check(lib.gsr_surface_backward(ptr(am), ptr(raymat), ctx.depth_ratio, H, W, ptr(sd), ptr(g_sd), ptr(g_sn), ptr(g_am),
                                           stream_ptr(am.device)), "gsr_surface_backward")
        return g_am, None, None


def surface_pass(allmap, view, depth_ratio):
    return _SurfacePass.apply(allmap, _ray_block(view), depth_ratio)


def _settings(viewpoint_camera, pc, bg_color, scaling_modifier):
    return GaussianRasterizationSettings(
        image_height=int(viewpoint_camera.image_height), image_width=int(viewpoint_camera.image_width),
        tanfovx=math.tan(viewpoint_camera.FoVx * 0.5), tanfovy=math.tan(viewpoint_camera.FoVy * 0.5), bg=bg_color,
        scale_modifier=scaling_modifier, viewmatrix=viewpoint_camera.world_view_transform,
        projmatrix=viewpoint_camera.full_proj_transform, sh_degree=pc.active_sh_degree, campos=viewpoint_camera.camera_center,
        prefiltered=False, debug=False)


def _precomputed_transmats(viewpoint_camera, pc, scaling_modifier, dev):
    W, H = viewpoint_camera.image_width, viewpoint_camera.image_height
    near, far = viewpoint_camera.znear, viewpoint_camera.zfar
    ndc2pix = torch.tensor([[W / 2, 0, 0, (W - 1) / 2], [0, H / 2, 0, (H - 1) / 2], [0, 0, far - near, near], [0, 0, 0, 1]],
                           dtype=torch.float32, device=dev).T
    world2pix = viewpoint_camera.full_proj_transform @ ndc2pix
    keep = [0, 1, 3]
    return (pc.get_covariance(scaling_modifier)[:, keep] @ world2pix[:, keep]).permute(0, 2, 1).reshape(-1, 9)


def _sinks(pipe):
    return (getattr(pipe, "gsr_grad_sink", None), getattr(pipe, "gsr_reflection_grad_sink", None), bool(getattr(pipe, "gsr_accumulate", False)),
            bool(getattr(pipe, "gsr_async_reflection_tail", False)))


def render(viewpoint_camera, pc, pipe, bg_color, scaling_modifier=1.0, override_color=None, initial_stage=False,
           env_scope_center=[0.0, 0.0, 0.0], env_scope_radius=0.0):
    xyz = pc.get_xyz
    dev = xyz.device
    means2D = torch.zeros_like(xyz, dtype=xyz.dtype, requires_grad=True, device=dev) + 0
    try:
        means2D.retain_grad()
    except Exception:
        pass
    raster_sink, refl_sink, accumulate, async_tail = _sinks(pipe)
    rasterizer = GaussianRasterizer(raster_settings=_settings(viewpoint_camera, pc, bg_color, scaling_modifier))
    rasterizer.set_grad_sink(raster_sink, accumulate)
    rasterizer.set_output_taps(("normal_view",))
    if env_scope_radius > 0.0:
        centre = torch.tensor([float(c) for c in env_scope_center], device=dev)
        env_scope_mask = ((xyz - centre[None]) ** 2).sum(dim=-1) < env_scope_radius ** 2
    else:
        env_scope_mask = torch.ones_like(xyz, device=dev) == 1.0
    scales = rotations = cov3D_precomp = None
    if getattr(pipe, "compute_cov3D_python", False):
        cov3D_precomp = _precomputed_transmats(viewpoint_camera, pc, scaling_modifier, dev)
    else:
        scales, rotations = pc.get_scaling, pc.get_rotation
    shs = pc.get_features if override_color is None else None
    v = viewpoint_camera
    fused = FUSED_REFLECTION and not initial_stage
    if fused:
        rasterizer.set_output_taps(())
        (final_image, refl_color, rend_normal, base_color, radii, allmap, refl_strength_map, gaussian_weights) = rasterize_reflect(
            rasterizer, pc.get_envmap, v.world_view_transform, v.HWK, v.R, v.T, means3D=xyz, means2D=means2D, shs=shs,
            colors_precomp=override_color, refl_strengths=pc.get_refl, opacities=pc.get_opacity, scales=scales, rotations=rotations,
            cov3D_precomp=cov3D_precomp, env_scope_mask=env_scope_mask, refl_grad_sink=refl_sink, accumulate=accumulate,
            async_tail=async_tail and bool(refl_sink))
    else:
        base_color, radii, allmap, refl_strength_map, gaussian_weights, normal_view = rasterizer(
            means3D=xyz, means2D=means2D, shs=shs, colors_precomp=override_color, refl_strengths=pc.get_refl, opacities=pc.get_opacity,
            scales=scales, rotations=rotations, cov3D_precomp=cov3D_precomp, env_scope_mask=env_scope_mask)

    surf_depth, surf_normal = surface_pass(allmap, viewpoint_camera, pipe.depth_ratio)
    out = {"viewspace_points": means2D, "visibility_filter": radii > 0, "radii": radii, "rend_alpha": allmap[1:2],
           "rend_dist": allmap[6:7], "surf_depth": surf_depth, "surf_normal": surf_normal, "gaussian_weights": gaussian_weights,
           "env_scope_mask": allmap[7:8]}
    if initial_stage:
        out["rend_normal"] = shading_normal(normal_view, v.world_view_transform, v.HWK, v.R, v.T)
        out["render"] = base_color
        return out
    if not fused:
        final_image, refl_color, rend_normal = deferred_reflection(normal_view, base_color, refl_strength_map, pc.get_envmap,
                                                                   v.world_view_transform, v.HWK, v.R, v.T, grad_sink=refl_sink,
                                                                   accumulate=accumulate, async_tail=async_tail and bool(refl_sink))
    out.update({"rend_normal": rend_normal, "render": final_image, "refl_strength_map": refl_strength_map, "refl_color_map": refl_color,
                "base_color_map": base_color})
    return out


def render_fast(viewpoint_camera, pc, pipe, bg_color, scaling_modifier=1.0, initial_stage=False):
    xyz = pc.get_xyz
    if not torch.is_grad_enabled():
        return _render_fast_eval(viewpoint_camera, pc, bg_color, scaling_modifier, initial_stage)
    means2D = torch.zeros_like(xyz, dtype=xyz.dtype, requires_grad=True, device=xyz.device) + 0
    rasterizer = GaussianRasterizer(raster_settings=_settings(viewpoint_camera, pc, bg_color, scaling_modifier))
    v = viewpoint_camera
    if FUSED_REFLECTION and not initial_stage:
        final_image, refl_color, rend_normal, base_color, _, allmap, refl_strength_map, _ = rasterize_reflect(
            rasterizer, pc.get_envmap, v.world_view_transform, v.HWK, v.R, v.T, means3D=xyz, means2D=means2D, shs=pc.get_features,
            refl_strengths=pc.get_refl, opacities=pc.get_opacity, scales=pc.get_scaling, rotations=pc.get_rotation,
            env_scope_mask=torch.ones_like(xyz).bool())
        return {"render": final_image, "rend_alpha": allmap[1:2], "rend_normal": rend_normal, "refl_strength_map": refl_strength_map,
                "refl_color_map": refl_color, "base_color_map": base_color}
    base_color, _, allmap, refl_strength_map, _ = rasterizer(
        means3D=xyz, means2D=means2D, shs=pc.get_features, colors_precomp=None, refl_strengths=pc.get_refl, opacities=pc.get_opacity,
        scales=pc.get_scaling, rotations=pc.get_rotation, cov3D_precomp=None, env_scope_mask=torch.ones_like(xyz).bool())
    return _render_fast_tail(v, pc, base_color, allmap[1:2], allmap[2:5], refl_strength_map, initial_stage)


def _render_fast_eval(viewpoint_camera, pc, bg_color, scaling_modifier, initial_stage):
    rasterizer = GaussianRasterizer(raster_settings=_settings(viewpoint_camera, pc, bg_color, scaling_modifier))
    v = viewpoint_camera
    fused = FUSED_REFLECTION and not initial_stage
    out = rasterize_eval(rasterizer, pc.get_xyz, pc.get_opacity, shs=pc.get_features, refl_strengths=pc.get_refl, scales=pc.get_scaling,
                         rotations=pc.get_rotation, env_map=pc.get_envmap if fused else None, world_view_transform=v.world_view_transform,
                         HWK=v.HWK, R=v.R, T=v.T)
    if fused:
        return out
    return _render_fast_tail(v, pc, out["render"], out["rend_alpha"], out["rend_normal"], out["refl_strength_map"], initial_stage)


def _render_fast_tail(v, pc, base_color, alpha, normal_view, refl_strength_map, initial_stage):
    if initial_stage:
        return {"render": base_color, "rend_alpha": alpha, "refl_strength_map": refl_strength_map,
                "rend_normal": shading_normal(normal_view, v.world_view_transform, v.HWK, v.R, v.T)}
    final_image, refl_color, rend_normal = deferred_reflection(normal_view, base_color, refl_strength_map, pc.get_envmap,
                                                               v.world_view_transform, v.HWK, v.R, v.T)
    return {"render": final_image, "rend_alpha": alpha, "rend_normal": rend_normal, "refl_strength_map": refl_strength_map,
            "refl_color_map": refl_color, "base_color_map": base_color}


def _panorama_dirs(H, W, device):
    az = torch.linspace(-math.pi, math.pi, W, dtype=torch.float32, device=device)[None, :]
    po = torch.linspace(0.0, math.pi, H, dtype=torch.float32, device=device)[:, None]
    grid1 = torch.stack([torch.sin(po) * torch.cos(az), torch.sin(po) * torch.sin(az), torch.cos(po).expand(H, W)], dim=-1)
    th = math.pi * torch.linspace(1.0 / H, 1.0 - 1.0 / H, H, dtype=torch.float32, device=device)[:, None]
    ph = math.pi * torch.linspace(-1.0 + 1.0 / W, 1.0 - 1.0 / W, W, dtype=torch.float32, device=device)[None, :]
    grid2 = torch.stack([torch.sin(th) * torch.sin(ph), torch.cos(th).expand(H, W), -torch.sin(th) * torch.cos(ph)], dim=-1)
    return grid1, grid2


def render_env_map(pc, height=512, width=1024):
    env = pc.get_envmap
    dev = env.params['Cubemap_texture'].device
    out = {}
    for name, dirs in zip(("env_cood1", "env_cood2"), _panorama_dirs(height, width, dev)):
        rgb = torch.sigmoid(env(dirs.reshape(-1, 3)))
        out[name] = rgb.reshape(height, width, 3).permute(2, 0, 1)
    return out
```

Measured before the change: 549.4.

## Fuse per-pixel reflection backward into surfel render backward prologue

The deferred reflection backward now gets a records-only path: it runs the cubemap footprint records, combine and unpack on the side stream, and skips writing the per-pixel g_base/g_strength/g_normal gradients. A pending-prologue table hands the reflection inputs to the surfel backward, whose render kernel recomputes those per-pixel gradients in registers as a prologue. This drops a full-image kernel and the write and re-read of seven HW-sized gradient planes. In exchange the reflection maths runs twice, the render backward kernel uses more registers, and correctness depends on host-side pointer matching between the two calls.

```diff
diff --git a/gaussian-splatting-reflection_amd/csrc/gsr_cubemap.hip b/gaussian-splatting-reflection_amd/csrc/gsr_cubemap.hip
--- a/gaussian-splatting-reflection_amd/csrc/gsr_cubemap.hip
+++ b/gaussian-splatting-reflection_amd/csrc/gsr_cubemap.hip
@@ -1,6 +1,7 @@
 #include <algorithm>
 #include <cstring>
 #include "gsr_internal.hpp"
+#include <atomic>
 #include <mutex>
 #include <memory>
 #include "gsr_sort.hpp"
@@ -344,6 +345,35 @@
 	}
 }
 
+__global__ void __launch_bounds__(256) __attribute__((amdgpu_num_vgpr(96)))
+deferred_refl_bwd_records_kernel(const float* __restrict__ normal_view, const float* __restrict__ strength, const float* __restrict__ cam,
+                                 const float4* __restrict__ rgba, const float* __restrict__ fail_value, int L, int W, int H,
+                                 const float* __restrict__ g_final, const float* __restrict__ g_refl_color, float* __restrict__ g_fail,
+                                 float* __restrict__ g_scratch, ReflFootprint* __restrict__ footprints, const uint32_t* __restrict__ keys_fwd,
+                                 uint32_t no_key) {
+	const size_t HW = (size_t)W * H;
+	const size_t pix = (size_t)blockIdx.x * 256 + threadIdx.x;
+	const bool live = pix < HW;
+	const size_t p = live ? pix : 0;
+	const int py = (int)(p / W), px = (int)(p - (size_t)py * W);
+	ReflBwdIn in;
+	in.nvx = normal_view[p]; in.nvy = normal_view[HW + p]; in.nvz = normal_view[2 * HW + p];
+	in.sv = strength[p];
+	in.has_grc = g_refl_color != nullptr;
+	in.has_gnw = false;
+#pragma unroll
+	for (int c = 0; c < 3; c++) {
+		in.gfin[c] = g_final[c * HW + p];
+		in.bas[c] = 0.f;
+		in.grc[c] = g_refl_color ? g_refl_color[c * HW + p] : 0.f;
+		in.gnw[c] = 0.f;
+	}
+	const uint32_t kf = keys_fwd[p];
+	ReflBwdOut o;
+	refl_backward_pixel<true, false, true>(cam, nullptr, rgba, fail_value, L, px, py, live, in, g_fail, g_scratch, footprints + p, true, kf, nullptr, no_key,
+	                                       (int)(threadIdx.x & 63), o);
+}
+
 template <bool ACC>
 __global__ void __launch_bounds__(256) unpack_cubemap_grad_kernel(const float4* __restrict__ scratch, float* __restrict__ g_cubemap,
                                                                   float* __restrict__ g_fail, int L) {
@@ -561,14 +591,31 @@
 }
 
 namespace {
+struct PendingPrologue {
+	bool used = false;
+	const float *g_nv = nullptr, *g_base = nullptr, *g_strength = nullptr;
+	hipStream_t stream = nullptr;
+	ReflPrologue p;
+};
+constexpr int PENDING_PROLOGUES = 8;
 struct SideStream {
 	hipStream_t stream = nullptr;
 	hipEvent_t fork = nullptr, fork2 = nullptr, done = nullptr, gate = nullptr;
 	bool recorded = false;
 	bool gate_pending = false;
+	PendingPrologue pending[PENDING_PROLOGUES];
+	PendingPrologue* find(const float* g_nv, const float* g_base, const float* g_strength, bool or_free) {
+		PendingPrologue* free_slot = nullptr;
+		for (PendingPrologue& e : pending) {
+			if (e.used && e.g_nv == g_nv && e.g_base == g_base && e.g_strength == g_strength) return &e;
+			if (!e.used && !free_slot) free_slot = &e;
+		}
+		return or_free ? free_slot : nullptr;
+	}
 };
 std::mutex g_side_mu;
 SideStream g_side[64];
+std::atomic<int> g_pending_prologues{0};
 SideStream* side_stream(bool create) {
 	int dev = 0;
 	if (hipGetDevice(&dev) != hipSuccess || dev < 0 || dev >= 64) return nullptr;
@@ -649,6 +696,19 @@
 	return 0;
 }
 
+bool refl_prologue_take(const float* g_normal_view, const float* g_base, const float* g_strength, hipStream_t stream, ReflPrologue* out) {
+	if (g_pending_prologues.load(std::memory_order_relaxed) == 0) return false;
+	std::lock_guard<std::mutex> lk(g_side_mu);
+	SideStream* s = side_stream(false);
+	PendingPrologue* e = s ? s->find(g_normal_view, g_base, g_strength, false) : nullptr;
+	if (!e) return false;
+	e->used = false;
+	g_pending_prologues--;
+	if (e->stream != stream) return false;
+	*out = e->p;
+	return true;
+}
+
 int refl_scratch_check(const char* entry, uint32_t L, int width, int height, const float* scratch, size_t scratch_floats) {
 	ReflTail t(L, width, height, nullptr);
 	if (!scratch || !t.carve(const_cast<float*>(scratch), scratch_floats)) {
@@ -704,6 +764,38 @@
 	const bool binned = t.carve(scratch, scratch_floats);
 	if (keys_sorted && !binned) { set_error("gsr_deferred_reflection_backward: keys_sorted needs the scratch the forward sorted into"); return GSR_E_INVALID; }
 	auto unpack = accumulate ? unpack_cubemap_grad_kernel<true> : unpack_cubemap_grad_kernel<false>;
+	if (g_pending_prologues.load(std::memory_order_relaxed) != 0) {
+		std::lock_guard<std::mutex> lk(g_side_mu);
+		SideStream* s = side_stream(false);
+		if (PendingPrologue* e = s ? s->find(g_normal_view, g_base, g_strength, false) : nullptr) { e->used = false; g_pending_prologues--; }
+	}
+	const size_t per_wg = (size_t)256 * REFL_CHUNK;
+	const unsigned cgrid = (unsigned)((t.rs.n + per_wg - 1) / per_wg);
+	if ((async_tail & 2) && binned && keys_sorted && cubemap_rgba) {
+		t.use_side_stream();
+		PendingPrologue* e = t.side ? t.side->find(g_normal_view, g_base, g_strength, true) : nullptr;
+		if (e) {
+			GSR_HIP_CHECK(t.fork(t.side->fork));
+			{
+				StageTimer tt(GSR_STAGE_REFL_BWD_TAIL, t.tail);
+				GSR_HIP_CHECK(hipMemsetAsync(scratch, 0, (ntex + 1) * 4 * sizeof(float), t.tail));
+				deferred_refl_bwd_records_kernel<<<(unsigned)((HW + 255) / 256), 256, 0, t.tail>>>(normal_view, refl_strength, cam, reinterpret_cast<const float4*>(cubemap_rgba),
+				                                                                                  fail_value, (int)L, width, height, g_final, g_refl_color, t.fail_acc,
+				                                                                                  t.staging, t.footprints, sort_keys, (uint32_t)ntex);
+				refl_run_combine_kernel<<<cgrid, 256, 0, t.tail>>>(t.keys_out, t.pix_out, t.footprints, t.rs.n, L, (uint32_t)ntex, t.staging);
+				unpack<<<(unsigned)((ntex + 255) / 256), 256, 0, t.tail>>>((const float4*)t.staging, g_cubemap, g_fail, (int)L);
+			}
+			GSR_HIP_CHECK(t.mark_done());
+			GSR_HIP_CHECK(hipGetLastError());
+			e->used = true;
+			g_pending_prologues++;
+			e->g_nv = g_normal_view; e->g_base = g_base; e->g_strength = g_strength; e->stream = stream;
+			e->p = ReflPrologue{normal_view, base_color, refl_strength, cam, fail_value, g_final, g_refl_color, g_normal_world, cubemap_rgba, (int)L, width, height};
+			return 1;
+		}
+		t.lock.unlock();
+		t.side = nullptr; t.tail = stream;
+	}
 	GSR_HIP_CHECK(hipMemsetAsync(scratch, 0, (ntex + 1) * 4 * sizeof(float), stream));
 	if (!binned) {
 		{
@@ -747,8 +839,6 @@
 	if (t.side) GSR_HIP_CHECK(t.fork(sort_keys ? t.side->fork2 : t.side->fork));
 	{
 		StageTimer tt(GSR_STAGE_REFL_BWD_TAIL, t.tail);
-		const size_t per_wg = (size_t)256 * REFL_CHUNK;
-		const unsigned cgrid = (unsigned)((t.rs.n + per_wg - 1) / per_wg);
 		if (!sort_keys) GSR_HIP_CHECK(t.sort(t.keys_in, small_sort, false));
 		refl_run_combine_kernel<<<cgrid, 256, 0, t.tail>>>(t.keys_out, t.pix_out, t.footprints, t.rs.n, L, (uint32_t)ntex, t.staging);
 		unpack<<<(unsigned)((ntex + 255) / 256), 256, 0, t.tail>>>((const float4*)t.staging, g_cubemap, g_fail, (int)L);
diff --git a/gaussian-splatting-reflection_amd/csrc/gsr_internal.hpp b/gaussian-splatting-reflection_amd/csrc/gsr_internal.hpp
--- a/gaussian-splatting-reflection_amd/csrc/gsr_internal.hpp
+++ b/gaussian-splatting-reflection_amd/csrc/gsr_internal.hpp
@@ -167,6 +167,12 @@
                 const ImageState& img, BinningState* out_binning, int prefiltered, int debug, hipStream_t stream, bool blend_masks = true);
 
 int side_gate_wait(hipStream_t stream);
+struct ReflPrologue {
+	const float *normal_view, *base, *strength, *cam, *fail_value, *g_final, *g_refl_color, *g_nworld;
+	const float* rgba;
+	int L, width, height;
+};
+bool refl_prologue_take(const float* g_normal_view, const float* g_base, const float* g_strength, hipStream_t stream, ReflPrologue* out);
 int refl_scratch_check(const char* entry, uint32_t L, int width, int height, const float* scratch, size_t scratch_floats);
 int refl_sort_keys_early(uint32_t L, int width, int height, float* scratch, size_t scratch_floats, const uint32_t* sort_keys, int async, bool gated,
                          hipStream_t stream);
diff --git a/gaussian-splatting-reflection_amd/csrc/gsr_refl.hpp b/gaussian-splatting-reflection_amd/csrc/gsr_refl.hpp
--- a/gaussian-splatting-reflection_amd/csrc/gsr_refl.hpp
+++ b/gaussian-splatting-reflection_amd/csrc/gsr_refl.hpp
@@ -264,7 +264,7 @@
 struct ReflBwdOut {
 	float g_base[3], g_strength, g_nv[3];
 };
-template <bool RGBA>
+template <bool RGBA, bool GRADS = true, bool RECORDS = true>
 __device__ __forceinline__ void refl_backward_pixel(const float* __restrict__ cam, const float* __restrict__ cubemap, const float4* __restrict__ rgba,
                                                     const float* __restrict__ fail_value, int L, int px, int py, bool live, const ReflBwdIn& in,
                                                     float* __restrict__ g_fail, float* __restrict__ g_scratch, ReflFootprint* __restrict__ footprint,
@@ -297,14 +297,18 @@
 		const float rc = sigmoidf_(cval);
 		const float gf = in.gfin[c];
 		const float b = in.bas[c];
-		out.g_base[c] = (1 - sv) * gf;
-		gs += gf * (rc - b);
+		if constexpr (GRADS) {
+			out.g_base[c] = (1 - sv) * gf;
+			gs += gf * (rc - b);
+		}
 		float gc = sv * gf;
 		if (in.has_grc) gc += in.grc[c];
 		graw[c] = gc * rc * (1 - rc);
 		if (fail) {
-			if (live) atomicAdd(g_fail + c, graw[c]);
-		} else {
+			if constexpr (RECORDS) {
+				if (live) atomicAdd(g_fail + c, graw[c]);
+			}
+		} else if constexpr (GRADS) {
 			float lg0 = (1 - s.ky) * (v01 - v00) + s.ky * (v11 - v10);
 			float lg1 = (1 - s.kx) * (v10 - v00) + s.kx * (v11 - v01);
 			lg0 *= 0.5f * (float)L * graw[c];
@@ -317,6 +321,7 @@
 			grx += a; gry += bb; grz += cc;
 		}
 	}
+	if constexpr (RECORDS) {
 	bool interior = !fail && s.flag == 0 && s.x[3] == s.x[0] + 1 && s.y[3] == s.y[0] + 1;
 	const uint32_t t00 = (uint32_t)(((size_t)s.f[0] * L + s.y[0]) * L + s.x[0]);
 	if (keys_fwd_valid) interior = interior && kf == t00;
@@ -355,6 +360,8 @@
 		}
 		if (!keys_fwd_valid) *key_out = interior ? t00 : no_key;
 	}
+	}
+	if constexpr (!GRADS) return;
 	out.g_strength = gs;
 	const float grn = grx * o.nx + gry * o.ny + grz * o.nz;
 	float gnx = -2.f * (o.dn * grx + grn * o.dx);
diff --git a/gaussian-splatting-reflection_amd/csrc/gsr_surfel.hip b/gaussian-splatting-reflection_amd/csrc/gsr_surfel.hip
--- a/gaussian-splatting-reflection_amd/csrc/gsr_surfel.hip
+++ b/gaussian-splatting-reflection_amd/csrc/gsr_surfel.hip
@@ -536,6 +536,7 @@
 	float FD2r, FAr, FDr;
 	float A, Dprev, last_alpha;
 };
+template <bool REFL>
 __device__ __forceinline__ void surfel_bwd_init(SurfelBwdPix& s, bool inside, size_t pix, size_t HW, const float* __restrict__ bg,
                                                 const float* __restrict__ final_Ts, const uint32_t* __restrict__ n_contrib,
                                                 const float* __restrict__ dL_dpixels, const float* __restrict__ dL_depths,
@@ -548,15 +549,17 @@
 	s.dp2 = s.dL_ddepth = s.dL_daccum = s.dL_dmedian_depth = 0.f;
 	float dL_dreg = 0.f;
 	if (inside) {
-		s.dp01 = mk2(dL_dpixels[pix], dL_dpixels[HW + pix]);
-		s.dp2 = dL_dpixels[2 * HW + pix];
+		if constexpr (!REFL) {
+			s.dp01 = mk2(dL_dpixels[pix], dL_dpixels[HW + pix]);
+			s.dp2 = dL_dpixels[2 * HW + pix];
+		}
 		s.dL_ddepth = dL_depths[0 * HW + pix];
 		s.dL_daccum = dL_depths[1 * HW + pix];
 		s.dn01 = mk2(dL_depths[2 * HW + pix], dL_depths[3 * HW + pix]);
-		s.dnzr = mk2(dL_depths[4 * HW + pix], dL_drefl_map[pix]);
+		s.dnzr = mk2(dL_depths[4 * HW + pix], REFL ? 0.f : dL_drefl_map[pix]);
 		s.dL_dmedian_depth = dL_depths[5 * HW + pix];
 		dL_dreg = dL_depths[6 * HW + pix];
-		if (dL_dnormal_extra) {
+		if (!REFL && dL_dnormal_extra) {
 			s.dn01 += mk2(dL_dnormal_extra[pix], dL_dnormal_extra[HW + pix]);
 			s.dnzr.x += dL_dnormal_extra[2 * HW + pix];
 		}
@@ -566,6 +569,37 @@
 	s.FAr = (1 - s.T_final) * dL_dreg;
 	s.last_dL_dT = 0;
 	s.A = s.Dprev = s.last_alpha = 0.f;
+	s.bg_dot_dpixel = bg[0] * s.dp01.x + bg[1] * s.dp01.y + bg[2] * s.dp2;
+}
+struct ReflBwdArgs {
+	const float *normal_view, *base, *strength, *cam, *fail_value, *g_final, *g_refl_color, *g_nworld;
+	const float4* rgba;
+	int L;
+};
+__device__ __forceinline__ void surfel_bwd_refl_prologue(SurfelBwdPix& s, const ReflBwdArgs& rb, bool inside, size_t pix, size_t HW, int px, int py, int lane,
+                                                         const float* __restrict__ bg) {
+	if (inside) {
+		ReflBwdIn in;
+		in.nvx = rb.normal_view[pix]; in.nvy = rb.normal_view[HW + pix]; in.nvz = rb.normal_view[2 * HW + pix];
+		in.sv = rb.strength[pix];
+		in.has_grc = rb.g_refl_color != nullptr;
+		in.has_gnw = rb.g_nworld != nullptr;
+#pragma unroll
+		for (int c = 0; c < 3; c++) {
+			in.gfin[c] = rb.g_final[c * HW + pix];
+			in.bas[c] = rb.base[c * HW + pix];
+			in.grc[c] = rb.g_refl_color ? rb.g_refl_color[c * HW + pix] : 0.f;
+			in.gnw[c] = rb.g_nworld ? rb.g_nworld[c * HW + pix] : 0.f;
+		}
+		ReflBwdOut o;
+		refl_backward_pixel<true, true, false>(rb.cam, nullptr, rb.rgba, rb.fail_value, rb.L, px, py, true, in, nullptr, nullptr, nullptr, false, 0u, nullptr, 0u,
+		                                       lane, o);
+		s.dp01 = mk2(o.g_base[0], o.g_base[1]);
+		s.dp2 = o.g_base[2];
+		s.dnzr.y = o.g_strength;
+		s.dn01 += mk2(o.g_nv[0], o.g_nv[1]);
+		s.dnzr.x += o.g_nv[2];
+	}
 	s.bg_dot_dpixel = bg[0] * s.dp01.x + bg[1] * s.dp01.y + bg[2] * s.dp2;
 }
 __device__ __forceinline__ lmask surfel_bwd_pair(SurfelBwdPix& s, const SurfelRec& R, const v2f pix, int contributor, lmask inside_m, float* v) {
@@ -664,12 +698,13 @@
 #ifndef S_CAP
 #define S_CAP 48
 #endif
+template <bool REFL>
 __device__ __forceinline__ void
 surfel_render_bwd_rows_body(const uint2* __restrict__ ranges, const uint32_t* __restrict__ tile_order, const uint32_t* __restrict__ point_list, int W, int H, int tiles_x, int ntiles,
                             const float* __restrict__ bg, const float4* __restrict__ rec, int dev_flags, const float* __restrict__ final_Ts,
                             const uint32_t* __restrict__ n_contrib, const float* __restrict__ dL_dpixels, const float* __restrict__ dL_depths,
                             const float* __restrict__ dL_drefl_map, const float* __restrict__ dL_dnormal_extra, float* __restrict__ acc,
-                            const unsigned long long* __restrict__ blend_mask) {
+                            const unsigned long long* __restrict__ blend_mask, const ReflBwdArgs& rb) {
 	const uint32_t slot = xcd_slot(blockIdx.x);
 	if (slot >= (uint32_t)ntiles * 4u) return;
 	const TileBlock blk = tile_block(tile_order, slot, tiles_x);
@@ -695,13 +730,14 @@
 	static_assert(S_CAP >= 32, "a chunk always takes the first 8-position group of its batch, up to 4 rows x 8 = 32 pairs");
 
 	SurfelBwdPix st;
-	surfel_bwd_init(st, inside, pix, HW, bg, final_Ts, n_contrib, dL_dpixels, dL_depths, dL_drefl_map, dL_dnormal_extra);
+	surfel_bwd_init<REFL>(st, inside, pix, HW, bg, final_Ts, n_contrib, dL_dpixels, dL_depths, dL_drefl_map, dL_dnormal_extra);
 	st.pixs = mk2(-pixv.y, pixv.x);
 	int wave_last = st.last_contributor;
 #pragma unroll
 	for (int off = 32; off > 0; off >>= 1) wave_last = max(wave_last, __shfl_xor(wave_last, off));
 	wave_last = __builtin_amdgcn_readfirstlane(wave_last);
 	if (wave_last == 0) return;
+	if constexpr (REFL) surfel_bwd_refl_prologue(st, rb, inside, pix, HW, px, py, lane, bg);
 	if (lane < S_ACC_F) s_slab[(S_CAP + 1) * S_ACC_F + lane] = 0.f;
 	const uint32_t slab_lane = (uint32_t)row_reduce_slot(lane) * 4u;
 	const unsigned long long lt = (1ull << lane) - 1ull, gt = ~((2ull << lane) - 1ull);
@@ -818,8 +854,16 @@
                               const uint32_t* __restrict__ n_contrib, const float* __restrict__ dL_dpixels, const float* __restrict__ dL_depths,
                               const float* __restrict__ dL_drefl_map, const float* __restrict__ dL_dnormal_extra, float* __restrict__ acc,
                               const unsigned long long* __restrict__ blend_mask) {
-	surfel_render_bwd_rows_body(ranges, tile_order, point_list, W, H, tiles_x, ntiles, bg, rec, dev_flags, final_Ts, n_contrib, dL_dpixels, dL_depths,
-	                            dL_drefl_map, dL_dnormal_extra, acc, blend_mask);
+	surfel_render_bwd_rows_body<false>(ranges, tile_order, point_list, W, H, tiles_x, ntiles, bg, rec, dev_flags, final_Ts, n_contrib, dL_dpixels, dL_depths,
+	                                   dL_drefl_map, dL_dnormal_extra, acc, blend_mask, ReflBwdArgs{});
+}
+__global__ void __launch_bounds__(64) __attribute__((amdgpu_waves_per_eu(GSR_BWD_WPE, GSR_BWD_WPE)))
+surfel_render_bwd_rows_kernel(const uint2* __restrict__ ranges, const uint32_t* __restrict__ tile_order, const uint32_t* __restrict__ point_list, int W, int H, int tiles_x, int ntiles,
+                              const float* __restrict__ bg, const float4* __restrict__ rec, int dev_flags, const float* __restrict__ final_Ts,
+                              const uint32_t* __restrict__ n_contrib, const float* __restrict__ dL_depths, float* __restrict__ acc,
+                              const unsigned long long* __restrict__ blend_mask, const ReflBwdArgs rb) {
+	surfel_render_bwd_rows_body<true>(ranges, tile_order, point_list, W, H, tiles_x, ntiles, bg, rec, dev_flags, final_Ts, n_contrib, nullptr, dL_depths,
+	                                  nullptr, nullptr, acc, blend_mask, rb);
 }
 
 __device__ __forceinline__ void quat_vjp(float w, float x, float y, float z, const M3& v_R, float* v_quat) {
@@ -1182,6 +1226,12 @@
                                    float* dL_drot, int accumulate, const float* dL_dnormal_extra, int debug, void* stream_) {
 	(void)scale_modifier;
 	hipStream_t stream = (hipStream_t)stream_;
+	ReflPrologue rp;
+	const bool deferred = dL_dnormal_extra && dL_dpix && dL_drefl_strength_map && refl_prologue_take(dL_dnormal_extra, dL_dpix, dL_drefl_strength_map, stream, &rp);
+	if (deferred && (rp.width != width || rp.height != height)) {
+		set_error("gsr_surfel_backward: the deferred reflection backward was made for %d x %d pixels, this call has %d x %d", rp.width, rp.height, width, height);
+		return GSR_E_INVALID;
+	}
 	if (const int rc = check_surfel_inputs("gsr_surfel_backward", "missing required pointer", P, D, M, means3D, shs, colors_precomp, refl_strengths, scales,
 	                                       rotations, transMat_precomp, viewmatrix, projmatrix, cam_pos, radii); rc < 0) return rc;
 	const bool missing = !background || !geom_buffer || !image_buffer || (R > 0 && !binning_buffer) || !dL_dpix || !dL_dothers || !dL_drefl_strength_map ||
@@ -1196,9 +1246,15 @@
 		{ const int rc = side_gate_wait(stream); if (rc < 0) return rc; }
 { StageTimer st_(GSR_STAGE_RENDER_BWD, stream);
 		const int nunits = (int)xcd_grid((uint32_t)ntiles * 4u);
-		surfel_render_bwd_rows_kernel<<<nunits, 64, 0, stream>>>(img.ranges, img.tile_order, bin.point_list, width, height, tiles_x, ntiles, background, geom.rec,
-		                                                         option_dev(), img.final_T, img.n_contrib, dL_dpix, dL_dothers, dL_drefl_strength_map, dL_dnormal_extra,
-		                                                         geom.acc, bin.blend_mask); }
+		if (deferred)
+			surfel_render_bwd_rows_kernel<<<nunits, 64, 0, stream>>>(img.ranges, img.tile_order, bin.point_list, width, height, tiles_x, ntiles, background, geom.rec,
+			                                                         option_dev(), img.final_T, img.n_contrib, dL_dothers, geom.acc, bin.blend_mask,
+			                                                         ReflBwdArgs{rp.normal_view, rp.base, rp.strength, rp.cam, rp.fail_value, rp.g_final, rp.g_refl_color,
+			                                                                     rp.g_nworld, reinterpret_cast<const float4*>(rp.rgba), rp.L});
+		else
+			surfel_render_bwd_rows_kernel<<<nunits, 64, 0, stream>>>(img.ranges, img.tile_order, bin.point_list, width, height, tiles_x, ntiles, background, geom.rec,
+			                                                         option_dev(), img.final_T, img.n_contrib, dL_dpix, dL_dothers, dL_drefl_strength_map, dL_dnormal_extra,
+			                                                         geom.acc, bin.blend_mask); }
 		GSR_LAUNCH_CHECK(debug, stream);
 	}
 	const RasterCam cam = make_cam(viewmatrix, projmatrix, cam_pos, width, height, tan_fovx, tan_fovy);
diff --git a/gaussian-splatting-reflection_amd/gaussian_renderer/__init__.py b/gaussian-splatting-reflection_amd/gaussian_renderer/__init__.py
--- a/gaussian-splatting-reflection_amd/gaussian_renderer/__init__.py
+++ b/gaussian-splatting-reflection_amd/gaussian_renderer/__init__.py
@@ -129,7 +129,7 @@
         return _reflection_backward(ctx.saved_tensors, (g_final, g_refl_color, g_normal_world), ctx.sink, ctx.sort_keys) + (None, None)
 
 
-def _reflection_backward(saved, grads, sink, sort_keys, scratch=None):
+def _reflection_backward(saved, grads, sink, sort_keys, scratch=None, defer=False):
     nv, bc, rs, cm, fv, cam, rgba = saved
     cont = lambda g: None if g is None else g.float().contiguous()
     g_final, g_refl_color, g_normal_world = grads
@@ -157,14 +157,19 @@
                               dtype=torch.float32, device=cm.device)
     g_nv, g_base, g_s = torch.empty_like(nv), torch.empty_like(bc), torch.empty_like(rs)
     with torch.cuda.device(nv.device):
-        check(lib.gsr_deferred_reflection_backward_keys(ptr(nv), ptr(bc), ptr(rs), ptr(cam), ptr(cm), ptr(fv), cm.shape[2], W, H,
+        rc = check(lib.gsr_deferred_reflection_backward_keys(ptr(nv), ptr(bc), ptr(rs), ptr(cam), ptr(cm), ptr(fv), cm.shape[2], W, H,
                                                         ptr(g_final), ptr(g_refl_color), ptr(g_normal_world), ptr(g_nv), ptr(g_base),
                                                         ptr(g_s), ptr(g_cm), ptr(g_fail), ptr(scratch), int(scratch.numel()), int(accumulate),
-                                                        int(async_tail), ptr(rgba), ptr(sort_keys), int(keys_sorted), stream_ptr(nv.device)),
+                                                        int(async_tail) | (2 if defer and async_tail else 0), ptr(rgba), ptr(sort_keys),
+                                                        int(keys_sorted), stream_ptr(nv.device)),
               "gsr_deferred_reflection_backward")
     if async_tail:
         _gsr.side_hold(scratch, g_cm, g_fail, sort_keys)
-    return g_nv, g_base, g_s, (None if sunk_cm else g_cm), (None if sunk_fail else g_fail)
+    if not defer:
+        return g_nv, g_base, g_s, (None if sunk_cm else g_cm), (None if sunk_fail else g_fail)
+    if rc == 1:
+        _gsr.side_hold(g_final, g_refl_color, nv, bc, rs, rgba, cam, fv)
+    return g_nv, g_base, g_s, (None if sunk_cm else g_cm), (None if sunk_fail else g_fail), rc == 1
 
 
 def deferred_reflection(normal_view, base_color, refl_strength_map, env_map, world_view_transform, HWK, R, T, grad_sink=None,
@@ -178,10 +183,12 @@
 
 
 FUSED_REFLECTION = True
+FUSED_REFLECTION_BACKWARD = True
 
 
 class _RasterizeReflect(torch.autograd.Function):
     probe = None
+    deferred_passes = 0
 
     @staticmethod
     def forward(ctx, *args):
@@ -217,9 +224,15 @@
         if ctx.scratch is not None and ctx.passes:
             with torch.cuda.device(cam.device):
                 check(lib.gsr_side_join(stream_ptr(cam.device)), "gsr_side_join")
+        first = ctx.passes == 0
         ctx.passes += 1
-        g_nv, g_base, g_s, g_cm, g_fail = _reflection_backward((others[2:5], color, refl_map, cm, fv, cam, rgba), (g_final, g_refl_color, g_normal_world),
-                                                               ctx.refl_sink, ctx.sort_keys, ctx.scratch)
+        defer = (FUSED_REFLECTION_BACKWARD and ctx.refl_sink is not None and ctx.refl_sink.async_tail and ctx.scratch is not None
+                 and ctx.num_rendered > 0 and _RasterizeReflect.probe is None and first and g_color is None and g_refl_map is None)
+        g_nv, g_base, g_s, g_cm, g_fail, deferred = _reflection_backward((others[2:5], color, refl_map, cm, fv, cam, rgba),
+                                                                         (g_final, g_refl_color, g_normal_world), ctx.refl_sink, ctx.sort_keys, ctx.scratch,
+                                                                         defer=defer) + ((False,) if not defer else ())
+        if deferred:
+            _RasterizeReflect.deferred_passes += 1
         g_color, g_refl_map, g_others = cont(g_color), cont(g_refl_map), cont(g_others)
         if g_color is not None:
             g_base.add_(g_color)
```

Result: no change. 554.2 (median of 6 runs) (+0.9%).
